# wells-wood-research/timed-design

Measured on AMD Instinct MI355X. Metric: residue_frames_per_sec, higher is better.
Workload: dtype f32

## Files before the change

include/timed_hip.h:

```cpp
#ifndef TIMED_HIP_H
#define TIMED_HIP_H

#include <stddef.h>
#include <stdint.h>

#ifdef __cplusplus
extern "C" {
#endif

#define TH_OK 0
#define TH_EINVAL (-1)
#define TH_EIO (-2)
#define TH_EHIP (-3)
#define TH_EUNSUP (-4)
#define TH_ENOMEM (-5)
#define TH_ECOMM (-6)
#define TH_EBUSY (-7)

#define TH_F32 0
#define TH_F64 1
#define TH_U8 2
#define TH_BOOL 3
#define TH_F16 4

#define TH_LOAD_DEFAULT 0u
#define TH_LOAD_NO_FUSE 1u
#define TH_LOAD_NO_MFMA 2u
#define TH_LOAD_KEEP_ALL 4u

#define TH_PREDICT_DEFAULT 0u
#define TH_PREDICT_LOGITS 1u
#define TH_PREDICT_OUT_DEVICE 2u
#define TH_PREDICT_IN_DEVICE 4u

typedef struct th_model th_model;
typedef struct th_comm th_comm;

int th_version(void);
const char* th_last_error(void);
int th_device_count(int* n_out);
int th_host_cpus(void);
int th_device_info(int device, char* name, size_t name_len, char* arch, size_t arch_len, int* cus);

int th_model_load(const char* pack_path, int device, unsigned flags, th_model** out);
int th_model_load_mem(const void* pack, size_t nbytes, int device, unsigned flags, th_model** out);
void th_model_free(th_model* m);
int th_model_info(const th_model* m, int dims[4], int* n_classes);
int th_model_cost(const th_model* m, double* algo_flops, double* exec_flops, int* n_steps);
int th_model_set_chunk(th_model* m, int frames_per_chunk);

int th_predict(th_model* m, const void* frames, int dtype, int64_t n, float* probs_out, unsigned flags);
int th_predict_async(th_model* m, const void* frames, int dtype, int64_t n, float* probs_out, unsigned flags, int* ticket);
int th_predict_wait(th_model* m, int ticket);
#define TH_SPARSE_MAGIC "THSPF001"
int th_predict_sparse_async(th_model* m, const void* blob, size_t blob_bytes, float* probs_out, unsigned flags, int* ticket);
int th_host_alloc(size_t bytes, void** out);
int th_host_free(void* p);
int th_host_register(void* p, size_t bytes);
int th_host_unregister(void* p);
int th_predict_device(th_model* m, const void* d_frames, int dtype, int64_t n, float* d_probs, unsigned flags);
int th_model_fetch(th_model* m, const char* layer_name, int64_t n, float* out, int64_t out_floats);

int th_model_profile(th_model* m, int enable);
int th_model_step_info(const th_model* m, int i, char* label, size_t label_len, double* ms, int64_t* launches,
                       double* flops_per_frame, double* exec_flops_per_frame, double* bytes_per_frame);
int th_model_step_direct_flops(const th_model* m, int i, double* direct_flops_per_frame);

int th_model_guard_info(const th_model* m, int* state, double* max_dlogit, double* logit_scale, char* note, size_t note_len);

int th_model_knobs(const th_model* m, char* buf, size_t buf_len);

int th_dev_alloc(int device, size_t bytes, void** d_out);
int th_dev_free(int device, void* d);
int th_dev_upload(int device, void* d_dst, const void* h_src, size_t bytes);
int th_dev_download(int device, void* h_dst, const void* d_src, size_t bytes);
int th_dev_sync(int device);
int th_dev_synth_frames(int device, float* d_frames, int64_t n, int side, int channels, int atoms, uint64_t seed);

int th_apply_temp(const double* probs, int64_t n_res, int n_cls, double t, double* out);
int th_apply_temp_on(int device, const double* probs, int64_t n_res, int n_cls, double t, double* out);
#define TH_RNG_HOST 0
#define TH_RNG_PHILOX 1
#define TH_RNG_MT19937 2
#define TH_RNG_MT_WORDS 3
int th_sample(const double* probs, int64_t n_res, int n_cls, int64_t n_samples, double temperature,
              int rng_mode, uint64_t seed, const double* uniforms, int32_t* idx_out);
int th_sample_ex(const double* probs, int64_t n_res, int n_cls, int64_t n_samples, double temperature,
                 int rng_mode, uint64_t seed, uint64_t rng_offset, const double* uniforms, int32_t* idx_out,
                 double* r_out, const char* cat_letters, char* letters_out, double* q_out, int device);

typedef struct th_sampler th_sampler;
int th_sampler_create(int device, th_sampler** out);
void th_sampler_free(th_sampler* s);
#define TH_TEMPER_NONE 0
#define TH_TEMPER_POW 1
#define TH_TEMPER_PREPOWERED 2
int th_sampler_load(th_sampler* s, const double* probs, int64_t n_rows, int n_cls, double temperature, int temper_mode,
                    int cum_dtype, double* q_out);
int th_sampler_draw(th_sampler* s, int64_t n_keys, const int64_t* row_off, int64_t n_samples, int rng_mode, uint64_t seed,
                    uint64_t rng_offset, const double* uniforms, const char* cat_letters, int32_t* idx_out, double* r_out,
                    char* letters_out, double* metrics_out);

int th_sampler_uniform_buffer(th_sampler* s, size_t bytes, void** out);
int th_sampler_run(th_sampler* s, const double* probs, int64_t n_rows, int n_cls, int cum_dtype, int64_t n_keys, const int64_t* row_off,
                   int64_t n_samples, int rng_mode, uint64_t seed, uint64_t rng_offset, const double* uniforms, const char* cat_letters,
                   unsigned want, const void** block_out, int64_t* offsets_out);

int th_mt19937_rand(uint32_t* key, int* pos, int64_t n, double* out);
int th_mt19937_words(uint32_t* key, int* pos, int64_t n, uint32_t* out);

int64_t th_format_csv(const void* data, int dtype, int64_t n, int64_t k, char* out, int64_t cap);
int64_t th_format_csv_device(int device, const float* rows, int64_t n, int64_t k, char* out, int64_t cap);
int th_format_csv_device_release(void);
int th_csv_shape(const char* text, int64_t len, char delim, int64_t* rows_out, int* cols_out, int* width_out);
int th_csv_fill(const char* text, int64_t len, char delim, int64_t rows, int cols, int width, uint32_t* out);
int th_argmax_letters(const void* matrix, int dtype, int64_t n, int64_t k, const char* col_letters, char* letters_out,
                      int32_t* idx_out);

typedef struct th_analysis_totals {
    int64_t confusion[20][20];
    int64_t rank_hist[21];
    int64_t n_labelled, n_nonfinite, n_similar;
} th_analysis_totals;
int th_analyse_probs(int device, const void* matrix, int dtype, int64_t n, int64_t k, const int8_t* col_res, const int8_t* true_res,
                     int8_t* pred_out, int8_t* rank_out, double* entropy_out, th_analysis_totals* totals);

int th_h5_read_chunked(const void* file, int64_t file_len, int64_t base, int64_t n_datasets, const int64_t* btree_addrs,
                       void* const* dests, int rank, const int64_t* shape, const int64_t* chunk, int esz, int n_filters,
                       const int* filter_ids, int nthreads);

int th_h5_read_chunked_as(const void* file, int64_t file_len, int64_t base, int64_t n_datasets, const int64_t* btree_addrs,
                          void* const* dests, int rank, const int64_t* shape, const int64_t* chunk, int esz, int n_filters,
                          const int* filter_ids, int nthreads, int conv);
int th_h5_read_contiguous_as(const void* file, int64_t file_len, int64_t base, int64_t n_datasets, const int64_t* data_addrs,
                             void* const* dests, int64_t count, int esz, int conv);
int th_h5_decode_device(const void* file, int64_t file_len, int64_t base, int64_t n_datasets, const int64_t* btree_addrs, int rank,
                        const int64_t* shape, const int64_t* chunk, int esz, int n_filters, const int* filter_ids, int conv, int device,
                        void* d_out);
int th_dev_trim(int device);
int th_dev_cache_info(int device, uint64_t* cached_bytes, uint64_t* cap_bytes, int* blocks);
int th_h5_release_scratch(int device);
int th_inflate_many(int device, const void* comp, int64_t comp_len, int64_t n, const int64_t* src_off, const int64_t* src_len,
                    const int64_t* dst_off, const int64_t* dst_len, void* out, int64_t out_len, int wrapped, int* status_out);

int th_h5_resolve(const void* file, int64_t file_len, int64_t base, int64_t n, const int64_t* ohdr_addrs, const char* num_attr,
                  double* num_out, int num_len, const char* str_attr, char* str_out, int str_len, int64_t* btree_out,
                  int64_t* geom_out, int* status_out, int nthreads);

int th_h5_group_links(const void* file, int64_t file_len, int64_t base, int64_t btree_addr, int64_t heap_data, int64_t heap_size,
                      char* names, int64_t names_cap, int64_t* addrs, int64_t addrs_cap, int64_t* n_out, int64_t* names_len);

int th_voxelise(int device, const float* atoms_xyz, const int32_t* atom_channel, const float* atom_sigma, int64_t n_atoms,
                const float* frames_rt, int64_t n_res, int voxels_per_side, float frame_edge_length, int n_channels, int gaussian,
                void* out, int out_on_device);

#define TH_COMM_ID_BYTES 128
int th_comm_unique_id(char id[TH_COMM_ID_BYTES]);
int th_comm_init(const char id[TH_COMM_ID_BYTES], int n_ranks, int rank, int device, th_comm** out);
void th_comm_free(th_comm* c);
int th_comm_gather_rows(th_comm* c, const float* d_local, const int64_t* counts, int width, int root,
                        float* d_out);
int th_comm_barrier(th_comm* c);
int th_comm_stats(th_comm* c, int64_t out[5]);

#ifdef __cplusplus
}
#endif
#endif
```

timed-design_amd/csrc/common.h:

```cpp
#pragma once
#include <hip/hip_runtime.h>
#include <stdint.h>
#include <string>
#include <vector>

#include "../../include/timed_hip.h"

enum : int {
    OP_INPUT = 0, OP_CONV3D, OP_DENSE, OP_BN, OP_ACT, OP_MAXPOOL, OP_AVGPOOL, OP_GAP, OP_GMP,
    OP_FLATTEN, OP_CONCAT, OP_ADD, OP_IDENTITY
};
enum : int { ACT_LINEAR = 0, ACT_RELU, ACT_ELU, ACT_SOFTMAX, ACT_SIGMOID, ACT_TANH, ACT_LEAKY };

void th_set_error(const char* fmt, ...);
#define TH_FAIL(code, ...)          \
    do {                            \
        th_set_error(__VA_ARGS__);  \
        return (code);              \
    } while (0)
#define HIP_TRY(expr)                                                                            \
    do {                                                                                         \
        hipError_t _e = (expr);                                                                  \
        if (_e != hipSuccess) {                                                                  \
            th_set_error("%s failed: %s (%s:%d)", #expr, hipGetErrorString(_e), __FILE__, __LINE__); \
            return TH_EHIP;                                                                      \
        }                                                                                        \
    } while (0)

struct ThKnobs {
    int winograd = 1;
    int wino_split = 1;
    int wfused = 1;
    int wf_split = 1;
    int lanes = 1, lane_lag = 1;
    int guard = 1;
    int first_wino = 1;
    int first_split = 1;
    int conv_gl = 1;
    int dense_gemm = 1;
    int first_int = 1;
    int first_zb = 0;
    int first_dbg = 0;
    int no_pool_first = 0;
    int no_tail_fuse = 0;
    int conv_nogeo = 0, n16_nogeo = 0, conv_noxc = 0, conv_notail = 0, conv_nozmajor = 0, conv_nocompact = 0, conv_nopw = 0;
    int conv_bmode = 0;
    int conv_dbg = 0, conv_ldspad = 0, n16_resident = 0;
    int pw_nopipe = 0, pw_noepi = 0, pw_dbg = 0;
    int wf_resident = 0, wf_dbg = 0, wf_noblk = 0;
    long long wino_piece = 0;
    int wino_dbg = 0, wino_var = 3, wino_b3var = 2, wino_nomid = 0;
    std::string nondefault;
};
void th_knobs_read(ThKnobs* k);
inline const ThKnobs& th_knobs_of(const ThKnobs* k) { static const ThKnobs dflt; return k ? *k : dflt; }

hipError_t th_malloc_retry_impl(void** p, size_t bytes);
template <class T> inline hipError_t th_malloc_retry(T** p, size_t bytes) { return th_malloc_retry_impl(reinterpret_cast<void**>(p), bytes); }

int th_usable_cpus();

struct TView {
    float* p = nullptr;
    int D = 1, H = 1, W = 1, C = 0;
    int cs = 0;
    int coff = 0;
    int64_t fs = 0;
    int blk = 0;
    int V() const { return D * H * W; }
};

#define TH_MAX_POST 4
enum : int { POP_ACT = 1, POP_AFFINE = 2 };
struct PostOps {
    int n = 0;
    int type[TH_MAX_POST] = {0, 0, 0, 0};
    int act[TH_MAX_POST] = {0, 0, 0, 0};
    float alpha[TH_MAX_POST] = {0, 0, 0, 0};
    const float* scale[TH_MAX_POST] = {nullptr, nullptr, nullptr, nullptr};
    const float* shift[TH_MAX_POST] = {nullptr, nullptr, nullptr, nullptr};
    int monotone = 0;
};
struct PreOp {
    const float* scale = nullptr;
    const float* shift = nullptr;
    int act = ACT_LINEAR;
    float alpha = 0.f;
};

struct ConvGeom {
    int kd, kh, kw, sd, sh, sw, dd, dh, dw;
    int pz, py, px;
};
int launch_convert_frames(hipStream_t s, const void* src, int dtype, int64_t n, int V, int C, TView dst);
int launch_conv3d_direct(hipStream_t s, int64_t n, TView in, TView out, ConvGeom g, const float* w, const float* bias,
                         PreOp pre, PostOps post);
int launch_pool3d(hipStream_t s, int64_t n, TView in, TView out, ConvGeom g, int is_max);
int launch_eltwise(hipStream_t s, int64_t n, TView in, TView out, PostOps ops);
int launch_global_pool(hipStream_t s, int64_t n, TView in, TView out, int is_max);
int launch_dense(hipStream_t s, int64_t n, TView in, TView out, const float* w, const float* bias, PostOps post);
inline bool conv_gl_wanted(int knob, const ConvGeom& g, int Vo) { return knob == 2 || (knob == 1 && (g.sd > 1 || g.sh > 1 || g.sw > 1 || Vo <= 64)); }
bool conv_gl_ok(int Cin, int Cout, int in_cs, int in_coff, int64_t in_fs);
size_t conv_gl_wpk_floats(const ConvGeom& g, int Cin, int Cout);
double conv_gl_exec_flops(const ConvGeom& g, int Cin, int Cout, int Vo);
std::string conv_gl_label(int Cout);
void conv_gl_pack_weights(const ConvGeom& g, int Cin, int Cout, const float* w, float* dst);
int launch_conv_gl(hipStream_t s, int64_t n, TView in, TView out, ConvGeom g, int Cin, int Cout, const float* wpk, const float* bias, PreOp pre, PostOps post);
bool dense_gemm_ok(int F, int O, int64_t xfs);
int launch_dense_gemm(hipStream_t s, int64_t n, TView in, TView out, const float* w, const float* bias, PostOps post);
int launch_softmax(hipStream_t s, int64_t n, TView in, TView out);
int launch_gap_softmax(hipStream_t s, int64_t n, TView in, TView logits, TView probs);
int launch_tail_dense(hipStream_t s, int64_t n, TView in, PostOps pre, TView pooled, TView logits, TView probs, const float* w,
                      const float* bias, PostOps post, int softmax);
int launch_copy(hipStream_t s, int64_t n, TView in, TView out);
int launch_add(hipStream_t s, int64_t n, TView a, TView b, TView out);
int launch_synth_frames(hipStream_t s, float* d, int64_t n, int side, int channels, int atoms, uint64_t seed);

struct ConvMfmaPlan {
    int cfg = -1;
    int CI = 0, CS = 0;
    int BN = 0;
    int nnb = 0;
    int nchunks = 0;
    int pool = 0;
    int Dc = 0, Hc = 0, Wc = 0;
    int FB = 1, ZB = 0, nzb = 1;
    int Zp = 0, Hp = 0, Wp = 0;
    int rows_pf = 0;
    int bres = 0;
    int ncu = 0;
    size_t lds_bytes = 0;
    size_t tab_off = 0;
    size_t wpk_floats = 0;
    double exec_flops = 0;
    int first_wino = 0;
    double own_flops = 0;
    int geo = 0;
    const ThKnobs* knobs = nullptr;
    std::string label;
};
bool conv_mfma_plan(const TView& in, const TView& out_conv, const ConvGeom& g, int Cin, int Cout, int pool,
                    const ThKnobs& kn, ConvMfmaPlan* plan);
bool conv_mfma_plan_tail(const TView& in, const TView& out_conv, const ConvGeom& g, int Cin, int Cout, int pool,
                         const ConvMfmaPlan& main, const ThKnobs& kn, ConvMfmaPlan* tail, int* cout_main);
void conv_mfma_pack_weights(const ConvMfmaPlan& p, const ConvGeom& g, int Cin, int Cout, const float* w_keras,
                            float* dst);
int launch_conv_mfma(hipStream_t s, int64_t n, const ConvMfmaPlan& p, TView in, TView out, ConvGeom g, int Cin,
                     int Cout, const float* wpk, const float* bias, PreOp pre, PostOps post);

struct ConvWinoPlan {
    int P = 9;
    int Cin = 0, Cout = 0, Coutp = 0, ncb = 0;
    int Cinp = 0;
    size_t wpk_floats = 0;
    int64_t v_fpf = 0, m_fpf = 0;
    double gemm_flops = 0;
    double exec_flops = 0;
    int split = 0;
    int narrow = 0;
    int b3var = 0;
    const ThKnobs* knobs = nullptr;
    std::string label;
};
bool conv_wino_plan(const TView& in, const TView& out_conv, const ConvGeom& g, int Cin, int Cout, int scheme, int split, const ThKnobs& kn,
                    ConvWinoPlan* plan);
void conv_wino_pack_weights(const ConvWinoPlan& p, const float* w_keras, float* dst);
int launch_wino_in(hipStream_t s, int64_t n, const ConvWinoPlan& p, TView in, float* V, PreOp pre);
int launch_wino_gemm(hipStream_t s, int64_t n, const ConvWinoPlan& p, const float* V, float* M, const float* wpk);
int launch_wino_out(hipStream_t s, int64_t n, const ConvWinoPlan& p, const float* M, TView out, const float* bias, PostOps post, bool gap = false);
int launch_wino_mid(hipStream_t s, int64_t n, const ConvWinoPlan& p, const float* M, float* V_next, const float* bias, PostOps post);

struct ConvWfPlan {
    int geo = -1;
    int pool = 0;
    int Cin = 0, Cout = 0, ncb = 0, nchunks = 0;
    size_t wpk_floats = 0, lds_bytes = 0;
    double own_flops = 0;
    double exec_flops = 0;
    int ncu = 0;
    const ThKnobs* knobs = nullptr;
    std::string label;
};
bool conv_wf_plan(const TView& in, const TView& out_conv, const ConvGeom& g, int Cin, int Cout, int pool, const ThKnobs& kn, ConvWfPlan* plan);
bool conv_wf_view_ok(const TView& in);
int conv_wf_pre_kind(const PreOp& pre);
std::string conv_wf_label(const ConvWfPlan& p, const PreOp& pre);
void conv_wf_pack_weights(const ConvWfPlan& p, const float* w_keras, float* dst);
int launch_conv_wf(hipStream_t s, int64_t n, const ConvWfPlan& p, TView in, TView out, const float* wpk, const float* bias, PreOp pre,
                   PostOps post);

struct ConvWfsPlan {
    int geo = -1, pool = 0;
    int Cin = 0, Cout = 0, nkh = 0, ncp = 0;
    size_t wpk_floats = 0, lds_bytes = 0;
    double own_flops = 0, exec_flops = 0;
    int ncu = 0;
    const ThKnobs* knobs = nullptr;
    std::string label;
};
bool conv_wfs_plan(const ConvWfPlan& base, const TView& in, const PreOp& pre, const ThKnobs& kn, ConvWfsPlan* plan);
void conv_wfs_pack_weights(const ConvWfsPlan& p, const float* w_keras, float* dst);
int launch_conv_wfs(hipStream_t s, int64_t n, const ConvWfsPlan& p, TView in, TView out, const float* wpk, const float* bias, PostOps post);

int launch_sparse_expand(hipStream_t s, int64_t n, const uint32_t* bits, const uint64_t* vidx, const float* values, float* out, int E, int W);

std::string conv_first_label(const ConvMfmaPlan& p, int Cin, const PostOps& post);
bool conv_first_plan(int Din, int Hin, int Win, int Cin, const TView& out_conv, const ConvGeom& g, int Cout, int pool,
                     const ThKnobs& kn, ConvMfmaPlan* plan);
void conv_first_pack_weights(int Cin, int Cout, const float* w_keras, float* dst);
void conv_first_w_pack_weights(int Cin, int Cout, const float* w_keras, float* dst);
int launch_conv_first(hipStream_t s, int64_t n, const ConvMfmaPlan& p, const void* frames, int dtype, int Din, int Hin,
                      int Win, int Cin, TView out, ConvGeom g, int Cout, const float* wpk, const float* bias, PostOps post);
bool conv_first_b3_ok(const ConvMfmaPlan& p, int Din, int Hin, int Win, int Cin, int Cout, const ConvGeom& g, const PostOps& post);
size_t conv_first_b3_wpk_floats();
double conv_first_b3_exec_flops();
std::string conv_first_b3_label(int nnb);
void conv_first_b3_pack_weights(int Cin, int Cout, const float* w_keras, float* dst);
int launch_conv_first_b3(hipStream_t s, int64_t n, const ConvMfmaPlan& p, const void* frames, int dtype, int Cin, TView out, int Cout,
                         const float* wpk, const float* bias, PostOps post);

bool conv_first5_ok(int Din, int Hin, int Win, int Cin, int Cout, const ConvGeom& g, int pool, const ThKnobs& kn);
size_t conv_first5_wpk_floats();
double conv_first5_exec_flops();
std::string conv_first5_label();
void conv_first5_pack_weights(int Cin, int Cout, const float* w_keras, float* dst);
int launch_conv_first5(hipStream_t s, int64_t n, const ThKnobs* knobs, int ncu, const void* frames, int dtype, int Cin, TView out, int Cout,
                       const float* wpk, const float* bias, PostOps post);

bool conv_pw_plan(const TView& in, const TView& out_conv, const ConvGeom& g, int Cin, int Cout, int pool, const ThKnobs& kn, ConvMfmaPlan* plan);
void conv_pw_pack_weights(const ConvMfmaPlan& p, int Cin, int Cout, const float* w_keras, float* dst);
std::string conv_pw_label(const ConvMfmaPlan& p, bool out_blk, const PostOps& post);
int launch_conv_pw(hipStream_t s, int64_t n, const ConvMfmaPlan& p, TView in, TView out, int Cin, int Cout, const float* wpk,
                   const float* bias, PreOp pre, PostOps post);

int sampler_run(int device, const double* h_probs, int64_t n_res, int n_cls, int64_t n_samples, double temperature,
                int rng_mode, uint64_t seed, uint64_t rng_offset, const double* h_uniforms, int32_t* h_idx, double* h_r_out,
                const char* cat_letters, char* h_letters, double* h_q_out);
```

timed-design_amd/csrc/conv_wino.hip:

```cpp
#include "common.h"
#include "device_math.h"
#include "wino_tables.h"

#include <algorithm>
#include <cstdlib>
#include <cstring>
#include <thread>
#include <vector>

typedef float f32x16 __attribute__((ext_vector_type(16)));

namespace {

constexpr int kZ = WINO_N;
constexpr int kNF = 64;
constexpr int kKC = 32;
constexpr int kCB = 128;

template <int R, int C>
__device__ __forceinline__ void wino_apply(const float (&T)[R][C], const float (&in)[C], float (&out)[R]) {
#pragma unroll
    for (int r = 0; r < R; ++r) {
        float acc = 0.f;
        bool first = true;
#pragma unroll
        for (int c = 0; c < C; ++c) {
            const float t = T[r][c];
            if (t == 0.f) continue;
            if (first) acc = t == 1.f ? in[c] : (t == -1.f ? -in[c] : t * in[c]);
            else acc = t == 1.f ? acc + in[c] : (t == -1.f ? acc - in[c] : fmaf(t, in[c], acc));
            first = false;
        }
        out[r] = acc;
    }
}

template <int P> struct WinoTab;
template <> struct WinoTab<9> {
    static __device__ __forceinline__ void fwd(const float (&in)[kZ], float (&out)[9]) { wino_apply<9, kZ>(kWinoBT9, in, out); }
    static __device__ __forceinline__ void inv(const float (&in)[9], float (&out)[kZ]) { wino_apply<kZ, 9>(kWinoAT9, in, out); }
};
template <> struct WinoTab<7> {
    static __device__ __forceinline__ void fwd(const float (&in)[kZ], float (&out)[7]) { wino_apply<7, kZ>(kWinoBT7, in, out); }
    static __device__ __forceinline__ void inv(const float (&in)[7], float (&out)[kZ]) { wino_apply<kZ, 7>(kWinoAT7, in, out); }
};

struct WinoInArgs {
    const float* in; int64_t in_fs; int in_cs, in_coff;
    int Cin;
    int Creal;
    PreOp pre;
    float* V; int64_t Ns;
    int64_t n;
};

template <bool PRE, int kP>
__global__ void __launch_bounds__(256) k_wino_in(const WinoInArgs a) {
    constexpr int kPos = kP * kP;
    const unsigned idx = blockIdx.x * 256u + threadIdx.x;
    const unsigned c = idx % (unsigned)a.Cin, f = idx / (unsigned)a.Cin;
    if (f >= (unsigned)a.n) return;
    const unsigned ooff = f * (unsigned)a.Cin + c;
    const int64_t pstride = a.Ns * a.Cin;
    if (c >= (unsigned)a.Creal) {
        for (int z = 0; z < kZ; ++z) {
            float* __restrict__ pos = a.V + (int64_t)z * kPos * pstride;
            for (int q = 0; q < kPos; ++q) (pos + (int64_t)q * pstride)[ooff] = 0.f;
        }
        return;
    }
    const unsigned ioff = f * (unsigned)a.in_fs + c;
    const float* __restrict__ in0 = a.in + a.in_coff;
    const bool affine = PRE && a.pre.scale != nullptr;
    const float sc = affine ? a.pre.scale[c] : 1.f, sh = affine ? a.pre.shift[c] : 0.f;
#pragma unroll 1
    for (int z = 0; z < kZ; ++z) {
        float x[kZ][kZ];
        const float* __restrict__ vox = in0 + (int64_t)z * kZ * kZ * a.in_cs;
#pragma unroll
        for (int i = 0; i < kZ * kZ; ++i) x[i / kZ][i % kZ] = (vox + (int64_t)i * a.in_cs)[ioff];
        if (PRE) {
            float flat[kZ * kZ];
#pragma unroll
            for (int i = 0; i < kZ * kZ; ++i) flat[i] = affine ? fmaf(x[i / kZ][i % kZ], sc, sh) : x[i / kZ][i % kZ];
            th_act_vec<kZ * kZ>(flat, a.pre.act, a.pre.alpha);
#pragma unroll
            for (int i = 0; i < kZ * kZ; ++i) x[i / kZ][i % kZ] = flat[i];
        }
        float t[kP][kZ];
#pragma unroll
        for (int k = 0; k < kZ; ++k) {
            float col[kZ], o[kP];
#pragma unroll
            for (int y = 0; y < kZ; ++y) col[y] = x[y][k];
            WinoTab<kP>::fwd(col, o);
#pragma unroll
            for (int aa = 0; aa < kP; ++aa) t[aa][k] = o[aa];
        }
        float* __restrict__ pos = a.V + (int64_t)z * kPos * pstride;
#pragma unroll
        for (int aa = 0; aa < kP; ++aa) {
            float o[kP];
            WinoTab<kP>::fwd(t[aa], o);
#pragma unroll
            for (int b = 0; b < kP; ++b) (pos + (int64_t)(aa * kP + b) * pstride)[ooff] = o[b];
        }
    }
}

struct WinoOutArgs {
    const float* M; int64_t Ns; int Coutp;
    int Cout;
    const float* bias;
    PostOps post;
    float* out; int64_t out_fs; int out_cs, out_coff;
    int64_t n;
};

template <int kP, bool GAP = false>
__global__ void __launch_bounds__(256) k_wino_out(const WinoOutArgs a) {
    constexpr int kPos = kP * kP;
    const unsigned idx = blockIdx.x * 256u + threadIdx.x;
    const unsigned co = idx % (unsigned)a.Cout, f = idx / (unsigned)a.Cout;
    if (f >= (unsigned)a.n) return;
    const unsigned ioff = f * (unsigned)a.Coutp + co;
    const unsigned ooff = f * (unsigned)a.out_fs + co;
    const int64_t pstride = a.Ns * a.Coutp;
    const float bv = a.bias ? a.bias[co] : 0.f;
    const bool elu_bn = a.post.n == 2 && a.post.type[0] == POP_ACT && a.post.act[0] == ACT_ELU && a.post.type[1] == POP_AFFINE;
    const float ealpha = a.post.alpha[0], esc = elu_bn ? a.post.scale[1][co] : 1.f, esh = elu_bn ? a.post.shift[1][co] : 0.f;
    float* __restrict__ out0 = a.out + a.out_coff;
    float gsum = 0.f;
#pragma unroll 1
    for (int z = 0; z < kZ; ++z) {
        float t[kP][kZ];
        const float* __restrict__ pos = a.M + (int64_t)z * kPos * pstride;
#pragma unroll
        for (int aa = 0; aa < kP; ++aa) {
            float m[kP];
#pragma unroll
            for (int b = 0; b < kP; ++b) m[b] = (pos + (int64_t)(aa * kP + b) * pstride)[ioff];
            WinoTab<kP>::inv(m, t[aa]);
        }
        float y[kZ * kZ];
#pragma unroll
        for (int k = 0; k < kZ; ++k) {
            float col[kP], o[kZ];
#pragma unroll
            for (int aa = 0; aa < kP; ++aa) col[aa] = t[aa][k];
            WinoTab<kP>::inv(col, o);
#pragma unroll
            for (int j = 0; j < kZ; ++j) y[j * kZ + k] = o[j] + bv;
        }
        if (elu_bn) {
#pragma unroll
            for (int k = 0; k < kZ * kZ; ++k) y[k] = fmaf(y[k] > 0.f ? y[k] : ealpha * (__expf(y[k]) - 1.f), esc, esh);
        } else
        for (int i = 0; i < a.post.n; ++i) {
            if (a.post.type[i] == POP_AFFINE) {
                const float sc = a.post.scale[i][co], sh = a.post.shift[i][co];
#pragma unroll
                for (int k = 0; k < kZ * kZ; ++k) y[k] = fmaf(y[k], sc, sh);
            } else {
                th_act_vec<kZ * kZ>(y, a.post.act[i], a.post.alpha[i]);
            }
        }
        if (GAP) {
#pragma unroll
            for (int v = 0; v < kZ * kZ; ++v) gsum += y[v];
            continue;
        }
        float* __restrict__ vox = out0 + (int64_t)z * kZ * kZ * a.out_cs;
#pragma unroll
        for (int v = 0; v < kZ * kZ; ++v) (vox + (int64_t)v * a.out_cs)[ooff] = y[v];
    }
    if (GAP) out0[ooff] = gsum / (float)(kZ * kZ * kZ);
}

struct WinoMidArgs {
    const float* M; int64_t Ns; int Coutp;
    int C;
    const float* bias;
    PostOps post;
    float* V;
    int Cn;
    int64_t n;
};

template <int kP>
__global__ void __launch_bounds__(256) k_wino_mid(const WinoMidArgs a) {
    constexpr int kPos = kP * kP;
    const unsigned idx = blockIdx.x * 256u + threadIdx.x;
    const unsigned c = idx % (unsigned)a.Cn, f = idx / (unsigned)a.Cn;
    if (f >= (unsigned)a.n) return;
    const unsigned ioff = f * (unsigned)a.Coutp + c;
    const unsigned ooff = f * (unsigned)a.Cn + c;
    const int64_t ipstride = a.Ns * a.Coutp, opstride = a.Ns * a.Cn;
    if (c >= (unsigned)a.C) {
        for (int z = 0; z < kZ; ++z) {
            float* __restrict__ opos = a.V + (int64_t)z * kPos * opstride;
            for (int q = 0; q < kPos; ++q) (opos + (int64_t)q * opstride)[ooff] = 0.f;
        }
        return;
    }
    const float bv = a.bias ? a.bias[c] : 0.f;
    const bool elu_bn = a.post.n == 2 && a.post.type[0] == POP_ACT && a.post.act[0] == ACT_ELU && a.post.type[1] == POP_AFFINE;
    const float ealpha = a.post.alpha[0], esc = elu_bn ? a.post.scale[1][c] : 1.f, esh = elu_bn ? a.post.shift[1][c] : 0.f;
#pragma unroll 1
    for (int z = 0; z < kZ; ++z) {
        float t[kP][kZ];
        const float* __restrict__ ipos = a.M + (int64_t)z * kPos * ipstride;
#pragma unroll
        for (int aa = 0; aa < kP; ++aa) {
            float m[kP];
#pragma unroll
            for (int b = 0; b < kP; ++b) m[b] = (ipos + (int64_t)(aa * kP + b) * ipstride)[ioff];
            WinoTab<kP>::inv(m, t[aa]);
        }
        float y[kZ * kZ];
#pragma unroll
        for (int k = 0; k < kZ; ++k) {
            float col[kP], o[kZ];
#pragma unroll
            for (int aa = 0; aa < kP; ++aa) col[aa] = t[aa][k];
            WinoTab<kP>::inv(col, o);
#pragma unroll
            for (int j = 0; j < kZ; ++j) y[j * kZ + k] = o[j] + bv;
        }
        if (elu_bn) {
#pragma unroll
            for (int k = 0; k < kZ * kZ; ++k) y[k] = fmaf(y[k] > 0.f ? y[k] : ealpha * (__expf(y[k]) - 1.f), esc, esh);
        } else
        for (int i = 0; i < a.post.n; ++i) {
            if (a.post.type[i] == POP_AFFINE) {
                const float sc = a.post.scale[i][c], sh = a.post.shift[i][c];
#pragma unroll
                for (int k = 0; k < kZ * kZ; ++k) y[k] = fmaf(y[k], sc, sh);
            } else {
                th_act_vec<kZ * kZ>(y, a.post.act[i], a.post.alpha[i]);
            }
        }
        float u[kP][kZ];
#pragma unroll
        for (int k = 0; k < kZ; ++k) {
            float col[kZ], o[kP];
#pragma unroll
            for (int j = 0; j < kZ; ++j) col[j] = y[j * kZ + k];
            WinoTab<kP>::fwd(col, o);
#pragma unroll
            for (int aa = 0; aa < kP; ++aa) u[aa][k] = o[aa];
        }
        float* __restrict__ opos = a.V + (int64_t)z * kPos * opstride;
#pragma unroll
        for (int aa = 0; aa < kP; ++aa) {
            float o[kP];
            WinoTab<kP>::fwd(u[aa], o);
#pragma unroll
            for (int b = 0; b < kP; ++b) (opos + (int64_t)(aa * kP + b) * opstride)[ooff] = o[b];
        }
    }
}

struct WinoGemmArgs {
    const float* V; const float* U; float* M;
    int64_t Ns;
    int Cin, Coutp;
    int Cout;
    int nfb, ncb;
    int npos;
    unsigned total;
    unsigned per_xcd;
    int dbg;
};

__device__ __forceinline__ constexpr bool wino_tap_ok(int zi, int dz) { return zi - dz + 1 >= 0 && zi - dz + 1 < kZ; }

template <int VAR>
__global__ void __launch_bounds__(256, 2) k_wino_gemm(const WinoGemmArgs a) {
    __shared__ __attribute__((aligned(16))) float lds[kZ * kNF * kKC];
    const unsigned xcd = blockIdx.x & 7u, slot = blockIdx.x >> 3;
    const unsigned L = xcd * a.per_xcd + slot;
    if (slot >= a.per_xcd || L >= a.total) return;
    const unsigned cb = L % (unsigned)a.ncb;
    const unsigned fb = (L / (unsigned)a.ncb) % (unsigned)a.nfb;
    const unsigned p = L / (unsigned)(a.ncb * a.nfb);
    const int tid = threadIdx.x, lane = tid & 63;
    const int wave = __builtin_amdgcn_readfirstlane(tid >> 6);
    const int j = lane & 31, h = lane >> 5;
    const int nchunks = a.Cin / kKC;
    const bool active = (int)(cb * kCB) + wave * 32 < a.Cout;
    const int S = a.Cin / 8;
    const float4* wq = reinterpret_cast<const float4*>(a.U) + ((size_t)((p * a.ncb + cb) * 4 + wave) * S * 3) * 64 + lane;
    const float* vbase = a.V + ((int64_t)p * a.Ns + (int64_t)fb * kNF) * a.Cin;
    const int64_t zstride = (int64_t)a.npos * a.Ns * a.Cin;

    f32x16 acc[kZ][2];
#pragma unroll
    for (int z = 0; z < kZ; ++z)
#pragma unroll
        for (int rt = 0; rt < 2; ++rt)
#pragma unroll
            for (int r = 0; r < 16; ++r) acc[z][rt][r] = 0.f;

    float4 bw[2][3];
#pragma unroll
    for (int dz = 0; dz < 3; ++dz) bw[0][dz] = wq[dz * 64];
    const int r0 = 8 * wave + (lane >> 3);
    const float* gsrc = vbase + (int64_t)r0 * a.Cin + (((lane & 7) ^ (lane >> 3)) << 2);
    const int64_t rstride32 = (int64_t)32 * a.Cin;
    unsigned aoff[kKC / 8];
#pragma unroll
    for (int s = 0; s < kKC / 8; ++s) aoff[s] = (unsigned)(j * kKC + (((2 * s + h) ^ (j & 7)) << 2));
    constexpr int kSlots = kKC / 8;
    static_assert(kSlots % 2 == 0, "the weight register sets alternate per k-slot");

    for (int ch = 0; ch < nchunks; ++ch) {
        __syncthreads();
        if (!(a.dbg & 1))
#pragma unroll
        for (int i = 0; i < 10; ++i)
            __builtin_amdgcn_global_load_lds(gsrc + (i >> 1) * zstride + (i & 1) * rstride32 + ch * kKC,
                                             lds + (size_t)(i * 4 + wave) * 256, 16, 0, 0);
        __syncthreads();
        if (!active) continue;
        float4 af[2][2];
        af[0][0] = *reinterpret_cast<const float4*>(lds + aoff[0]);
        af[0][1] = *reinterpret_cast<const float4*>(lds + aoff[0] + 32 * kKC);
#pragma unroll
        for (int s = 0; s < kSlots; ++s) {
            {
                const int sg = ch * kSlots + s;
                const int nx = sg + 1 < S ? sg + 1 : sg;
                if (a.dbg & 4) {
#pragma unroll
                    for (int dz = 0; dz < 3; ++dz) bw[(s + 1) & 1][dz] = bw[s & 1][dz];
                } else
#pragma unroll
                for (int dz = 0; dz < 3; ++dz) bw[(s + 1) & 1][dz] = wq[(size_t)(nx * 3 + dz) * 64];
            }
#pragma unroll
            for (int zi = 0; zi < kZ; ++zi) {
                const int ph = s * kZ + zi, cur = ph & 1;
                if (ph + 1 < kSlots * kZ) {
                    const int ns = (ph + 1) / kZ, nz = (ph + 1) % kZ;
                    af[cur ^ 1][0] = *reinterpret_cast<const float4*>(lds + aoff[ns] + (nz * kNF) * kKC);
                    af[cur ^ 1][1] = *reinterpret_cast<const float4*>(lds + aoff[ns] + (nz * kNF + 32) * kKC);
                }
                if (VAR == 1) __builtin_amdgcn_sched_barrier(0);
                const float av0[4] = {af[cur][0].x, af[cur][0].y, af[cur][0].z, af[cur][0].w};
                const float av1[4] = {af[cur][1].x, af[cur][1].y, af[cur][1].z, af[cur][1].w};
#pragma unroll
                for (int dz = 0; dz < 3; ++dz) {
                    if (!wino_tap_ok(zi, dz)) continue;
                    const int zo = zi - dz + 1;
                    const float4 b4 = bw[s & 1][dz];
                    const float bv[4] = {b4.x, b4.y, b4.z, b4.w};
#pragma unroll
                    for (int t = 0; t < 4; ++t) {
                        acc[zo][0] = __builtin_amdgcn_mfma_f32_32x32x2f32(av0[t], bv[t], acc[zo][0], 0, 0, 0);
                        acc[zo][1] = __builtin_amdgcn_mfma_f32_32x32x2f32(av1[t], bv[t], acc[zo][1], 0, 0, 0);
                    }
                }
                if (VAR == 1) __builtin_amdgcn_sched_barrier(0);
            }
        }
    }
    if (!active) return;
    float* mbase = a.M + ((int64_t)p * a.Ns + (int64_t)fb * kNF) * a.Coutp + cb * kCB + wave * 32 + j;
    const int64_t mz = (int64_t)a.npos * a.Ns * a.Coutp;
    if (a.dbg & 2) {
        float sum = 0.f;
#pragma unroll
        for (int z = 0; z < kZ; ++z)
#pragma unroll
            for (int rt = 0; rt < 2; ++rt)
#pragma unroll
                for (int r = 0; r < 16; ++r) sum += acc[z][rt][r];
        if (sum == 12345.678f) mbase[0] = sum;
        return;
    }
    if (VAR == 3) {
        __syncthreads();
        float* T = lds + wave * (32 * 36);
        const int rr = lane >> 3, c4 = (lane & 7) * 4;
        float* mb = a.M + ((int64_t)p * a.Ns + (int64_t)fb * kNF) * a.Coutp + cb * kCB + wave * 32 + c4;
#pragma unroll
        for (int z = 0; z < kZ; ++z)
#pragma unroll
            for (int rt = 0; rt < 2; ++rt) {
#pragma unroll
                for (int r = 0; r < 16; ++r) T[((r & 3) + 8 * (r >> 2) + 4 * h) * 36 + j] = acc[z][rt][r];
#pragma unroll
                for (int k = 0; k < 4; ++k) {
                    const int row = rr + 8 * k;
                    *reinterpret_cast<float4*>(mb + z * mz + (int64_t)(rt * 32 + row) * a.Coutp) = *reinterpret_cast<const float4*>(T + row * 36 + c4);
                }
            }
        return;
    }
#pragma unroll
    for (int z = 0; z < kZ; ++z)
#pragma unroll
        for (int rt = 0; rt < 2; ++rt)
#pragma unroll
            for (int r = 0; r < 16; ++r) {
                const int row = rt * 32 + (r & 3) + 8 * (r >> 2) + 4 * h;
                if (VAR == 2) __builtin_nontemporal_store(acc[z][rt][r], mbase + z * mz + (int64_t)row * a.Coutp);
                else mbase[z * mz + (int64_t)row * a.Coutp] = acc[z][rt][r];
            }
}


typedef __bf16 bf16x8 __attribute__((ext_vector_type(8)));
typedef __bf16 bf16x2 __attribute__((ext_vector_type(2)));
typedef float f32x2v __attribute__((ext_vector_type(2)));
typedef unsigned u32x4v __attribute__((ext_vector_type(4)));

__device__ __forceinline__ unsigned wino_pk_bf16(float lo, float hi) {
    return __builtin_bit_cast(unsigned, __builtin_convertvector((f32x2v){lo, hi}, bf16x2));
}
__device__ __forceinline__ float wino_bf16_lo(unsigned w) { return __builtin_bit_cast(float, w << 16); }
__device__ __forceinline__ float wino_bf16_hi(unsigned w) { return __builtin_bit_cast(float, w & 0xffff0000u); }

constexpr int kB3Slab = kZ * kNF * kKC * 2;

__device__ __forceinline__ constexpr int wino_b3_sw16(int R) { return ((R >> 2) & 3) ^ (((R >> 2) & 1) << 1); }

typedef float f32x4 __attribute__((ext_vector_type(4)));

__device__ __forceinline__ void wino_gemm_b3_16(const WinoGemmArgs& a, unsigned char* lds) {
    const unsigned xcd = blockIdx.x & 7u, slot = blockIdx.x >> 3;
    const unsigned L = xcd * a.per_xcd + slot;
    if (slot >= a.per_xcd || L >= a.total) return;
    const unsigned cb = L % (unsigned)a.ncb;
    const unsigned fb = (L / (unsigned)a.ncb) % (unsigned)a.nfb;
    const unsigned p = L / (unsigned)(a.ncb * a.nfb);
    const int tid = threadIdx.x, lane = tid & 63;
    const int wave = __builtin_amdgcn_readfirstlane(tid >> 6);
    const int r16 = lane & 15, g16 = lane >> 4;
    const int nchunks = a.Cin / kKC;
    const bool active = (int)(cb * kCB) + wave * 32 < a.Cout;
    const __amdgpu_buffer_rsrc_t wrsrc = __builtin_amdgcn_make_buffer_rsrc(
        const_cast<float*>(a.U + ((size_t)((p * a.ncb + cb) * 4 + wave) * nchunks * 18) * 256), 0, 0xffffffffu, 0x00020000);
    const unsigned woff = (unsigned)lane * 16u;
    const float* vbase = a.V + ((int64_t)p * a.Ns + (int64_t)fb * kNF) * a.Cin;
    const int64_t zstride = (int64_t)a.npos * a.Ns * a.Cin;

    f32x4 acc[kZ][4][2];
#pragma unroll
    for (int z = 0; z < kZ; ++z)
#pragma unroll
        for (int rt = 0; rt < 4; ++rt)
#pragma unroll
            for (int ct = 0; ct < 2; ++ct) acc[z][rt][ct] = (f32x4){0.f, 0.f, 0.f, 0.f};

    const int r0 = 8 * wave + (lane >> 3), g4 = lane & 7;
    __amdgpu_buffer_rsrc_t vrsrc[kZ];
#pragma unroll
    for (int z = 0; z < kZ; ++z) vrsrc[z] = __builtin_amdgcn_make_buffer_rsrc(const_cast<float*>(vbase + z * zstride), 0, 0xffffffffu, 0x00020000);
    const unsigned goff = (unsigned)(r0 * a.Cin + 4 * g4) * 4u;
    const unsigned rstride32_b = (unsigned)(32 * a.Cin * 4);
    unsigned char* const sdst = lds + r0 * 64 + (((g4 >> 1) ^ wino_b3_sw16(r0)) << 4) + ((g4 & 1) << 3);
    const unsigned char* const aptr = lds + r16 * 64 + ((g16 ^ wino_b3_sw16(r16)) << 4);

    uint4 bw[2][3][3];
    auto load_b = [&](int ch, int ct) {
        if (a.dbg & 4) {
            const unsigned k = woff ^ ((unsigned)(ch * 2 + ct) << 4);
#pragma unroll
            for (int dz = 0; dz < 3; ++dz)
#pragma unroll
                for (int pc = 0; pc < 3; ++pc)
                    bw[ct][dz][pc] = make_uint4(0x3f813f82u ^ (k << (dz + pc)), 0x3e833e84u ^ k, 0x3d853d86u + (k << pc), 0x3c873c88u ^ (k << dz));
            return;
        }
#pragma unroll
        for (int dz = 0; dz < 3; ++dz)
#pragma unroll
            for (int pc = 0; pc < 3; ++pc)
                bw[ct][dz][pc] = __builtin_bit_cast(uint4, __builtin_amdgcn_raw_buffer_load_b128(wrsrc, woff, (((ch * 2 + ct) * 3 + dz) * 3 + pc) * 1024, 0));
    };

    for (int ch = 0; ch < nchunks; ++ch) {
        __syncthreads();
        {
            float4 x[10];
#pragma unroll
            for (int i = 0; i < 10; ++i)
                x[i] = (a.dbg & 1) ? make_float4(1.f, 2.f, 3.f, 4.f) :
                       __builtin_bit_cast(float4, __builtin_amdgcn_raw_buffer_load_b128(vrsrc[i >> 1], goff, (i & 1) * rstride32_b + ch * (kKC * 4), 0));
            __builtin_amdgcn_sched_barrier(0);
#pragma unroll
            for (int i = 0; i < 10; ++i) {
                const unsigned h01 = wino_pk_bf16(x[i].x, x[i].y), h23 = wino_pk_bf16(x[i].z, x[i].w);
                const float rx = x[i].x - wino_bf16_lo(h01), ry = x[i].y - wino_bf16_hi(h01);
                const float rz = x[i].z - wino_bf16_lo(h23), rw = x[i].w - wino_bf16_hi(h23);
                const unsigned m01 = wino_pk_bf16(rx, ry), m23 = wino_pk_bf16(rz, rw);
                const float sx = rx - wino_bf16_lo(m01), sy = ry - wino_bf16_hi(m01);
                const float sz = rz - wino_bf16_lo(m23), sw = rw - wino_bf16_hi(m23);
                const unsigned l01 = wino_pk_bf16(sx, sy), l23 = wino_pk_bf16(sz, sw);
                *reinterpret_cast<uint2*>(sdst + i * 2048) = make_uint2(h01, h23);
                *reinterpret_cast<uint2*>(sdst + i * 2048 + kB3Slab) = make_uint2(m01, m23);
                *reinterpret_cast<uint2*>(sdst + i * 2048 + 2 * kB3Slab) = make_uint2(l01, l23);
            }
        }
        load_b(ch, 0);
        load_b(ch, 1);
        __syncthreads();
        if (!active) continue;
#pragma unroll
        for (int zi = 0; zi < kZ; ++zi)
#pragma unroll
            for (int rt = 0; rt < 4; ++rt) {
                bf16x8 af[3];
#pragma unroll
                for (int pc = 0; pc < 3; ++pc)
                    af[pc] = __builtin_bit_cast(bf16x8, *reinterpret_cast<const uint4*>(aptr + pc * kB3Slab + (zi * kNF + rt * 16) * 64));
#pragma unroll
                for (int dz = 0; dz < 3; ++dz) {
                    if (!wino_tap_ok(zi, dz)) continue;
                    const int zo = zi - dz + 1;
                    constexpr int PA[6] = {2, 0, 1, 1, 0, 0}, PB[6] = {0, 2, 1, 0, 1, 0};
#pragma unroll
                    for (int c = 0; c < 6; ++c)
#pragma unroll
                        for (int ct = 0; ct < 2; ++ct)
                            acc[zo][rt][ct] = __builtin_amdgcn_mfma_f32_16x16x32_bf16(af[PA[c]], __builtin_bit_cast(bf16x8, bw[ct][dz][PB[c]]),
                                                                                     acc[zo][rt][ct], 0, 0, 0);
                }
                __builtin_amdgcn_sched_barrier(0);
            }
    }
    if (!active) return;
    if (a.dbg & 2) {
        float sum = 0.f;
#pragma unroll
        for (int z = 0; z < kZ; ++z)
#pragma unroll
            for (int rt = 0; rt < 4; ++rt)
#pragma unroll
                for (int ct = 0; ct < 2; ++ct)
#pragma unroll
                    for (int r = 0; r < 4; ++r) sum += acc[z][rt][ct][r];
        if (sum == 12345.678f) a.M[0] = sum;
        return;
    }
    __syncthreads();
    float* T = reinterpret_cast<float*>(lds) + wave * (16 * 36);
    const int rr = lane >> 3, c4 = (lane & 7) * 4;
    float* mb = a.M + ((int64_t)p * a.Ns + (int64_t)fb * kNF) * a.Coutp + cb * kCB + wave * 32 + c4;
    const int64_t mz = (int64_t)a.npos * a.Ns * a.Coutp;
#pragma unroll
    for (int z = 0; z < kZ; ++z)
#pragma unroll
        for (int rt = 0; rt < 4; ++rt) {
#pragma unroll
            for (int ct = 0; ct < 2; ++ct)
#pragma unroll
                for (int r = 0; r < 4; ++r) T[(4 * g16 + r) * 36 + ct * 16 + r16] = acc[z][rt][ct][r];
#pragma unroll
            for (int k = 0; k < 2; ++k) {
                const int row = rr + 8 * k;
                *reinterpret_cast<float4*>(mb + z * mz + (int64_t)(rt * 16 + row) * a.Coutp) = *reinterpret_cast<const float4*>(T + row * 36 + c4);
            }
        }
}

template <int VAR>
__global__ void __launch_bounds__(256, 2) k_wino_gemm_b3(const WinoGemmArgs a) {
    __shared__ __attribute__((aligned(16))) unsigned char lds[3 * kB3Slab];
    if constexpr (VAR == 2) {
        wino_gemm_b3_16(a, lds);
        return;
    }
    const unsigned xcd = blockIdx.x & 7u, slot = blockIdx.x >> 3;
    const unsigned L = xcd * a.per_xcd + slot;
    if (slot >= a.per_xcd || L >= a.total) return;
    const unsigned cb = L % (unsigned)a.ncb;
    const unsigned fb = (L / (unsigned)a.ncb) % (unsigned)a.nfb;
    const unsigned p = L / (unsigned)(a.ncb * a.nfb);
    const int tid = threadIdx.x, lane = tid & 63;
    const int wave = __builtin_amdgcn_readfirstlane(tid >> 6);
    const int j = lane & 31, h = lane >> 5;
    const int nchunks = a.Cin / kKC;
    const bool active = (int)(cb * kCB) + wave * 32 < a.Cout;
    const int S = nchunks * 6;
    const uint4* wq = reinterpret_cast<const uint4*>(a.U) + ((size_t)((p * a.ncb + cb) * 4 + wave) * S * 3) * 64 + lane;
    const float* vbase = a.V + ((int64_t)p * a.Ns + (int64_t)fb * kNF) * a.Cin;
    const int64_t zstride = (int64_t)a.npos * a.Ns * a.Cin;

    f32x16 acc[kZ][2];
#pragma unroll
    for (int z = 0; z < kZ; ++z)
#pragma unroll
        for (int rt = 0; rt < 2; ++rt)
#pragma unroll
            for (int r = 0; r < 16; ++r) acc[z][rt][r] = 0.f;

    uint4 bw[2][3];
#pragma unroll
    for (int pc = 0; pc < 3; ++pc) bw[0][pc] = wq[pc * 64];
    const int r0 = 8 * wave + (lane >> 3), g4 = lane & 7;
    __amdgpu_buffer_rsrc_t vrsrc[kZ];
#pragma unroll
    for (int z = 0; z < kZ; ++z) vrsrc[z] = __builtin_amdgcn_make_buffer_rsrc(const_cast<float*>(vbase + z * zstride), 0, 0xffffffffu, 0x00020000);
    const unsigned goff = (unsigned)(r0 * a.Cin + 4 * g4) * 4u;
    const unsigned rstride32_b = (unsigned)(32 * a.Cin * 4);
    unsigned char* const sdst = lds + r0 * 64 + (((g4 >> 1) ^ ((r0 >> 2) & 3)) << 4) + ((g4 & 1) << 3);
    const unsigned char* aptr[2];
#pragma unroll
    for (int ks = 0; ks < 2; ++ks) aptr[ks] = lds + j * 64 + (((2 * ks + h) ^ ((j >> 2) & 3)) << 4);

    for (int ch = 0; ch < nchunks; ++ch) {
        __syncthreads();
        {
            float4 x[10];
#pragma unroll
            for (int i = 0; i < 10; ++i)
                x[i] = (a.dbg & 1) ? make_float4(1.f, 2.f, 3.f, 4.f) :
                       __builtin_bit_cast(float4, __builtin_amdgcn_raw_buffer_load_b128(vrsrc[i >> 1], goff, (i & 1) * rstride32_b + ch * (kKC * 4), 0));
            __builtin_amdgcn_sched_barrier(0);
#pragma unroll
            for (int i = 0; i < 10; ++i) {
                const unsigned h01 = wino_pk_bf16(x[i].x, x[i].y), h23 = wino_pk_bf16(x[i].z, x[i].w);
                const float rx = x[i].x - wino_bf16_lo(h01), ry = x[i].y - wino_bf16_hi(h01);
                const float rz = x[i].z - wino_bf16_lo(h23), rw = x[i].w - wino_bf16_hi(h23);
                const unsigned m01 = wino_pk_bf16(rx, ry), m23 = wino_pk_bf16(rz, rw);
                const float sx = rx - wino_bf16_lo(m01), sy = ry - wino_bf16_hi(m01);
                const float sz = rz - wino_bf16_lo(m23), sw = rw - wino_bf16_hi(m23);
                const unsigned l01 = wino_pk_bf16(sx, sy), l23 = wino_pk_bf16(sz, sw);
                *reinterpret_cast<uint2*>(sdst + i * 2048) = make_uint2(h01, h23);
                *reinterpret_cast<uint2*>(sdst + i * 2048 + kB3Slab) = make_uint2(m01, m23);
                *reinterpret_cast<uint2*>(sdst + i * 2048 + 2 * kB3Slab) = make_uint2(l01, l23);
            }
        }
        __syncthreads();
        if (!active) continue;
#pragma unroll
        for (int st = 0; st < 6; ++st) {
            const int ks = st / 3, dz = st % 3, cur = st & 1;
            {
                const int sg = ch * 6 + st;
                const int nx = sg + 1 < S ? sg + 1 : sg;
                if (a.dbg & 4) {
#pragma unroll
                    for (int pc = 0; pc < 3; ++pc) bw[cur ^ 1][pc] = bw[cur][pc];
                } else
#pragma unroll
                for (int pc = 0; pc < 3; ++pc) bw[cur ^ 1][pc] = wq[(size_t)(nx * 3 + pc) * 64];
            }
            bf16x8 bf[3];
#pragma unroll
            for (int pc = 0; pc < 3; ++pc) bf[pc] = __builtin_bit_cast(bf16x8, bw[cur][pc]);
            const int nzi = 5 - (dz != 1), z0 = dz == 2 ? 1 : 0;
            bf16x8 af[2][2][3];
            auto read_a = [&](int set, int zi) {
#pragma unroll
                for (int rt = 0; rt < 2; ++rt)
#pragma unroll
                    for (int pc = 0; pc < 3; ++pc)
                        af[set][rt][pc] = __builtin_bit_cast(bf16x8, *reinterpret_cast<const uint4*>(aptr[ks] + pc * kB3Slab + (zi * kNF + rt * 32) * 64));
            };
            if (VAR == 1) read_a(0, z0);
#pragma unroll
            for (int k = 0; k < kZ; ++k) {
                if (k >= nzi) continue;
                const int zi = z0 + k, zo = zi - dz + 1;
                const int set = VAR == 1 ? (k & 1) : 0;
                if (VAR == 1) { if (k + 1 < nzi) read_a(set ^ 1, zi + 1); }
                else read_a(0, zi);
                if (VAR == 1) __builtin_amdgcn_sched_barrier(0);
                constexpr int PA[6] = {2, 0, 1, 1, 0, 0}, PB[6] = {0, 2, 1, 0, 1, 0};
#pragma unroll
                for (int c = 0; c < 6; ++c)
#pragma unroll
                    for (int rt = 0; rt < 2; ++rt)
                        acc[zo][rt] = __builtin_amdgcn_mfma_f32_32x32x16_bf16(af[set][rt][PA[c]], bf[PB[c]], acc[zo][rt], 0, 0, 0);
                __builtin_amdgcn_sched_barrier(0);
            }
        }
    }
    if (!active) return;
    if (a.dbg & 2) {
        float sum = 0.f;
#pragma unroll
        for (int z = 0; z < kZ; ++z)
#pragma unroll
            for (int rt = 0; rt < 2; ++rt)
#pragma unroll
                for (int r = 0; r < 16; ++r) sum += acc[z][rt][r];
        if (sum == 12345.678f) a.M[0] = sum;
        return;
    }
    __syncthreads();
    float* T = reinterpret_cast<float*>(lds) + wave * (32 * 36);
    const int rr = lane >> 3, c4 = (lane & 7) * 4;
    float* mb = a.M + ((int64_t)p * a.Ns + (int64_t)fb * kNF) * a.Coutp + cb * kCB + wave * 32 + c4;
    const int64_t mz = (int64_t)a.npos * a.Ns * a.Coutp;
#pragma unroll
    for (int z = 0; z < kZ; ++z)
#pragma unroll
        for (int rt = 0; rt < 2; ++rt) {
#pragma unroll
            for (int r = 0; r < 16; ++r) T[((r & 3) + 8 * (r >> 2) + 4 * h) * 36 + j] = acc[z][rt][r];
#pragma unroll
            for (int k = 0; k < 4; ++k) {
                const int row = rr + 8 * k;
                *reinterpret_cast<float4*>(mb + z * mz + (int64_t)(rt * 32 + row) * a.Coutp) = *reinterpret_cast<const float4*>(T + row * 36 + c4);
            }
        }
}



__global__ void __launch_bounds__(256, 2) k_wino_gemm_n32(const WinoGemmArgs a) {
    __shared__ __attribute__((aligned(16))) float4 tile[4][32 * 8];
    const int tid = threadIdx.x, lane = tid & 63;
    const int wave = __builtin_amdgcn_readfirstlane(tid >> 6);
    const int j = lane & 31, h = lane >> 5;
    const int nfb32 = (int)(a.Ns / 32);
    const int groups = (nfb32 + 3) / 4;
    const unsigned p = blockIdx.x / (unsigned)groups;
    const int fb = (int)(blockIdx.x % (unsigned)groups) * 4 + wave;
    if (fb >= nfb32) return;
    const int nchunks = a.Cin / kKC;
    const uint4* wq = reinterpret_cast<const uint4*>(a.U) + (size_t)p * nchunks * 18 * 64 + lane;
    const float* vbase = a.V + ((int64_t)p * a.Ns + (int64_t)fb * 32) * a.Cin;
    const int64_t zstride = (int64_t)a.npos * a.Ns * a.Cin;
    __amdgpu_buffer_rsrc_t vrsrc[kZ];
#pragma unroll
    for (int z = 0; z < kZ; ++z) vrsrc[z] = __builtin_amdgcn_make_buffer_rsrc(const_cast<float*>(vbase + z * zstride), 0, 0xffffffffu, 0x00020000);
    const int lr = lane >> 3, lg = lane & 7;
    const unsigned goff = (unsigned)(lr * a.Cin + 4 * lg) * 4u;
    const unsigned row8_b = (unsigned)(8 * a.Cin * 4);
    float4* const T = tile[wave];

    f32x16 acc[kZ];
#pragma unroll
    for (int z = 0; z < kZ; ++z)
#pragma unroll
        for (int r = 0; r < 16; ++r) acc[z][r] = 0.f;

    auto load_plane = [&](float4 (&x)[4], int ch, int zi) {
#pragma unroll
        for (int k = 0; k < 4; ++k)
            x[k] = __builtin_bit_cast(float4, __builtin_amdgcn_raw_buffer_load_b128(vrsrc[zi], goff, k * row8_b + ch * (kKC * 4), 0));
    };
    auto transpose = [&](const float4 (&x)[4], float4 (&f)[4]) {
#pragma unroll
        for (int k = 0; k < 4; ++k) { const int r = 8 * k + lr; T[r * 8 + (lg ^ ((r >> 1) & 7))] = x[k]; }
#pragma unroll
        for (int g = 0; g < 4; ++g) f[g] = T[j * 8 + ((4 * h + g) ^ ((j >> 1) & 7))];
    };
    auto split8 = [&](const float4& lo, const float4& hi, bf16x8 (&f)[3]) {
        const float v[8] = {lo.x, lo.y, lo.z, lo.w, hi.x, hi.y, hi.z, hi.w};
        unsigned hw[4], mw[4], lw[4];
#pragma unroll
        for (int q = 0; q < 4; ++q) {
            hw[q] = wino_pk_bf16(v[2 * q], v[2 * q + 1]);
            const float r0 = v[2 * q] - wino_bf16_lo(hw[q]), r1 = v[2 * q + 1] - wino_bf16_hi(hw[q]);
            mw[q] = wino_pk_bf16(r0, r1);
            const float s0 = r0 - wino_bf16_lo(mw[q]), s1 = r1 - wino_bf16_hi(mw[q]);
            lw[q] = wino_pk_bf16(s0, s1);
        }
        f[0] = __builtin_bit_cast(bf16x8, make_uint4(hw[0], hw[1], hw[2], hw[3]));
        f[1] = __builtin_bit_cast(bf16x8, make_uint4(mw[0], mw[1], mw[2], mw[3]));
        f[2] = __builtin_bit_cast(bf16x8, make_uint4(lw[0], lw[1], lw[2], lw[3]));
    };

    float4 xs[3][4];
    auto load_step = [&](float4 (&x)[4], int step_ch, int zi) {
        load_plane(x, step_ch < nchunks ? step_ch : nchunks - 1, zi);
    };
    load_step(xs[0], 0, 0);
    load_step(xs[1], 0, 1);
    for (int ch0 = 0; ch0 < nchunks; ch0 += 3) {
#pragma unroll
        for (int cc = 0; cc < 3; ++cc) {
            const int ch = ch0 + cc;
            if (ch >= nchunks) break;
            uint4 bw[2][3][3];
#pragma unroll
            for (int ks = 0; ks < 2; ++ks)
#pragma unroll
                for (int dz = 0; dz < 3; ++dz)
#pragma unroll
                    for (int pc = 0; pc < 3; ++pc) bw[ks][dz][pc] = wq[(size_t)(((ch * 2 + ks) * 3 + dz) * 3 + pc) * 64];
#pragma unroll
            for (int zi = 0; zi < kZ; ++zi) {
                const int t = cc * kZ + zi;
                float4 fr[4];
                transpose(xs[t % 3], fr);
                {
                    const int t2 = t + 2, c2 = ch0 + t2 / kZ, z2 = t2 % kZ;
                    load_step(xs[t2 % 3], c2, z2);
                }
                bf16x8 af[2][3];
                split8(fr[0], fr[1], af[0]);
                split8(fr[2], fr[3], af[1]);
                constexpr int PA[6] = {2, 0, 1, 1, 0, 0}, PB[6] = {0, 2, 1, 0, 1, 0};
#pragma unroll
                for (int q = 0; q < 6; ++q)
#pragma unroll
                    for (int ks = 0; ks < 2; ++ks)
#pragma unroll
                        for (int dz = 0; dz < 3; ++dz) {
                            if (!wino_tap_ok(zi, dz)) continue;
                            acc[zi - dz + 1] = __builtin_amdgcn_mfma_f32_32x32x16_bf16(af[ks][PA[q]], __builtin_bit_cast(bf16x8, bw[ks][dz][PB[q]]),
                                                                                       acc[zi - dz + 1], 0, 0, 0);
                        }
                __builtin_amdgcn_sched_barrier(0);
            }
        }
    }
    float* mb = a.M + ((int64_t)p * a.Ns + (int64_t)fb * 32) * a.Coutp + j;
    const int64_t mz = (int64_t)a.npos * a.Ns * a.Coutp;
#pragma unroll
    for (int z = 0; z < kZ; ++z)
#pragma unroll
        for (int r = 0; r < 16; ++r) mb[z * mz + (int64_t)((r & 3) + 8 * (r >> 2) + 4 * h) * a.Coutp] = acc[z][r];
}

}

bool conv_wino_plan(const TView& in, const TView& out, const ConvGeom& g, int Cin, int Cout, int scheme, int split, const ThKnobs& kn, ConvWinoPlan* p) {
    if (g.kd != 3 || g.kh != 3 || g.kw != 3 || g.sd != 1 || g.sh != 1 || g.sw != 1 || g.dd != 1 || g.dh != 1 || g.dw != 1) return false;
    if (g.pz != 1 || g.py != 1 || g.px != 1) return false;
    if (in.D != kZ || in.H != kZ || in.W != kZ || out.D != kZ || out.H != kZ || out.W != kZ) return false;
    const bool narrow = split && Cout <= 32 && Cin >= 128;
    if (Cin < kKC || (Cout < 64 && !narrow)) return false;
    if (scheme != 9 && scheme != 7) return false;
    const int kPos = scheme * scheme;
    p->P = scheme;
    p->Cin = Cin; p->Cout = Cout;
    p->Cinp = (Cin + kKC - 1) / kKC * kKC;
    const int Cinp = p->Cinp;
    p->narrow = narrow ? 1 : 0;
    p->Coutp = narrow ? 32 : (Cout + kCB - 1) / kCB * kCB;
    p->ncb = narrow ? 1 : p->Coutp / kCB;
    p->split = split ? 1 : 0;
    p->b3var = split && !narrow ? kn.wino_b3var : 0;
    p->knobs = &kn;
    p->wpk_floats = (size_t)kPos * 3 * Cinp * p->Coutp * (p->split ? 3 : 2) / 2;
    p->v_fpf = (int64_t)kZ * kPos * Cinp;
    p->m_fpf = (int64_t)kZ * kPos * p->Coutp;
    p->gemm_flops = 2.0 * kPos * 13 * Cin * (double)Cout;
    p->exec_flops = 2.0 * kPos * 13 * Cinp * (double)((Cout + 31) / 32 * 32);
    p->label = std::string("conv_wino<") + (scheme == 9 ? "F(3,3)+F(2,3)" : "F(5,3)") + " in-plane, z direct; gemm " + (narrow ? "32f x 32" : "64f x " + std::to_string(kCB)) + "c, K" + std::to_string(Cinp) + (Cinp != Cin ? " (" + std::to_string(Cin) + " real)" : "") +
               (p->split ? "; bf16x3 split operands, 6 products, fp32 accumulate" : "") + ">";
    return true;
}

static inline uint16_t wino_bf16_rne(float f) {
    uint32_t u;
    std::memcpy(&u, &f, 4);
    if ((u & 0x7f800000u) == 0x7f800000u) return (uint16_t)(u >> 16);
    u += 0x7fffu + ((u >> 16) & 1u);
    return (uint16_t)(u >> 16);
}
static inline double wino_bf16_val(uint16_t b) {
    const uint32_t u = (uint32_t)b << 16;
    float f;
    std::memcpy(&f, &u, 4);
    return (double)f;
}
static inline void wino_split3(double x, uint16_t (&pc)[3]) {
    pc[0] = wino_bf16_rne((float)x);
    const double r1 = x - wino_bf16_val(pc[0]);
    pc[1] = wino_bf16_rne((float)r1);
    const double r2 = r1 - wino_bf16_val(pc[1]);
    pc[2] = wino_bf16_rne((float)r2);
}

void conv_wino_pack_weights(const ConvWinoPlan& p, const float* w, float* dst) {
    const int Cin = p.Cin, Cinp = p.Cinp, Cout = p.Cout, S = Cinp / 8, ncb = p.ncb, kP = p.P;
    auto G = [kP](int a, int j) { return kP == 9 ? kWinoG9[a][j] : kWinoG7[a][j]; };
    std::memset(dst, 0, p.wpk_floats * sizeof(float));
    auto work = [&](int ci_lo, int ci_hi) {
        std::vector<double> t((size_t)kP * 3 * Cout), u((size_t)Cout);
        for (int ci = ci_lo; ci < ci_hi; ++ci) {
            const int s = ci / 8, hh = (ci % 8) / 4, tt = ci % 4;
            for (int dz = 0; dz < 3; ++dz) {
                for (int a = 0; a < kP; ++a)
                    for (int k = 0; k < 3; ++k) {
                        double* tr = &t[((size_t)a * 3 + k) * Cout];
                        std::fill(tr, tr + Cout, 0.0);
                        for (int jj = 0; jj < 3; ++jj) {
                            const double g = G(a, jj);
                            if (g == 0.0) continue;
                            const float* wr = w + ((((size_t)dz * 3 + jj) * 3 + k) * Cin + ci) * Cout;
                            for (int co = 0; co < Cout; ++co) tr[co] += g * (double)wr[co];
                        }
                    }
                for (int a = 0; a < kP; ++a)
                    for (int b = 0; b < kP; ++b) {
                        std::fill(u.begin(), u.end(), 0.0);
                        for (int k = 0; k < 3; ++k) {
                            const double g = G(b, k);
                            if (g == 0.0) continue;
                            const double* tr = &t[((size_t)a * 3 + k) * Cout];
                            for (int co = 0; co < Cout; ++co) u[co] += g * tr[co];
                        }
                        const int pos = a * kP + b;
                        if (p.narrow) {
                            uint16_t* d16 = reinterpret_cast<uint16_t*>(dst);
                            const int chunk = ci / kKC, h16 = (ci % kKC) / 16, ks = (ci % 16) / 8, e = ci % 8, nch = Cinp / kKC;
                            for (int co = 0; co < Cout; ++co) {
                                uint16_t pc[3];
                                wino_split3(u[co], pc);
                                const size_t frag = ((size_t)(pos * nch + chunk) * 2 + ks) * 3 + dz;
                                for (int q = 0; q < 3; ++q) d16[((frag * 3 + q) * 64 + (h16 * 32 + co)) * 8 + e] = pc[q];
                            }
                            continue;
                        }
                        if (p.split && p.b3var == 2) {
                            uint16_t* d16 = reinterpret_cast<uint16_t*>(dst);
                            const int chunk = ci / kKC, g8 = (ci % kKC) / 8, e = ci % 8, nch = Cinp / kKC;
                            for (int co = 0; co < Cout; ++co) {
                                const int cb = co / kCB, wv = (co % kCB) / 32, ct = (co % 32) / 16, c = co % 16;
                                uint16_t pc[3];
                                wino_split3(u[co], pc);
                                const size_t frag = ((size_t)(((pos * ncb + cb) * 4 + wv) * nch + chunk) * 2 + ct) * 3 + dz;
                                for (int q = 0; q < 3; ++q) d16[((frag * 3 + q) * 64 + (g8 * 16 + c)) * 8 + e] = pc[q];
                            }
                            continue;
                        }
                        if (p.split) {
                            uint16_t* d16 = reinterpret_cast<uint16_t*>(dst);
                            const int chunk = ci / kKC, ks = (ci % kKC) / 16, h8 = (ci % 16) / 8, e = ci % 8, nsteps = (Cinp / kKC) * 6;
                            for (int co = 0; co < Cout; ++co) {
                                const int cb = co / kCB, wv = (co % kCB) / 32, j = co % 32;
                                uint16_t pc[3];
                                wino_split3(u[co], pc);
                                const size_t step = (size_t)((pos * ncb + cb) * 4 + wv) * nsteps + (size_t)(chunk * 2 + ks) * 3 + dz;
                                for (int q = 0; q < 3; ++q) d16[((step * 3 + q) * 64 + (h8 * 32 + j)) * 8 + e] = pc[q];
                            }
                            continue;
                        }
                        for (int co = 0; co < Cout; ++co) {
                            const int cb = co / kCB, wv = (co % kCB) / 32, j = co % 32;
                            dst[((((size_t)(pos * ncb + cb) * 4 + wv) * S + s) * 3 + dz) * 256 + (hh * 32 + j) * 4 + tt] = (float)u[co];
                        }
                    }
            }
        }
    };
    const int nt = std::max(1, std::min({th_usable_cpus(), 32, Cin / 8}));
    if (nt == 1) { work(0, Cin); return; }
    std::vector<std::thread> th;
    for (int k = 0; k < nt; ++k) th.emplace_back(work, (int)((int64_t)Cin * k / nt), (int)((int64_t)Cin * (k + 1) / nt));
    for (auto& x : th) x.join();
}

static int64_t wino_piece(const ConvWinoPlan& p, int64_t n, int64_t Ns, int64_t fs, int width) {
    const int64_t lim = (1ll << 31) - 1;
    if (Ns * width > lim) return 0;
    const int64_t forced = th_knobs_of(p.knobs).wino_piece;
    const int64_t piece = std::max<int64_t>(1, std::min<int64_t>(n, lim / std::max<int64_t>(fs, 1)));
    return forced > 0 ? std::min(piece, forced) : piece;
}

int launch_wino_in(hipStream_t s, int64_t n, const ConvWinoPlan& p, TView in, float* V, PreOp pre) {
    if (n <= 0) return TH_OK;
    const int64_t Ns = (n + kNF - 1) / kNF * kNF;
    const int64_t piece = wino_piece(p, n, Ns, in.fs, p.Cinp);
    if (!piece) TH_FAIL(TH_EUNSUP, "conv_wino: %lld frames per launch exceed the 32-bit offsets of the transform kernels", (long long)n);
    const bool has_pre = pre.scale || pre.act != ACT_LINEAR;
    for (int64_t f0 = 0; f0 < n; f0 += piece) {
        const int64_t cnt = std::min(piece, n - f0);
        WinoInArgs ia;
        ia.in = in.p + f0 * in.fs; ia.in_fs = in.fs; ia.in_cs = in.cs; ia.in_coff = in.coff; ia.Cin = p.Cinp; ia.Creal = p.Cin; ia.pre = pre;
        ia.V = V + f0 * p.Cinp; ia.Ns = Ns; ia.n = cnt;
        const dim3 grid((unsigned)((cnt * p.Cinp + 255) / 256));
        if (p.P == 9) {
            if (has_pre) hipLaunchKernelGGL((k_wino_in<true, 9>), grid, dim3(256), 0, s, ia);
            else hipLaunchKernelGGL((k_wino_in<false, 9>), grid, dim3(256), 0, s, ia);
        } else {
            if (has_pre) hipLaunchKernelGGL((k_wino_in<true, 7>), grid, dim3(256), 0, s, ia);
            else hipLaunchKernelGGL((k_wino_in<false, 7>), grid, dim3(256), 0, s, ia);
        }
    }
    HIP_TRY(hipGetLastError());
    return TH_OK;
}

int launch_wino_gemm(hipStream_t s, int64_t n, const ConvWinoPlan& p, const float* V, float* M, const float* wpk) {
    if (n <= 0) return TH_OK;
    WinoGemmArgs ga;
    ga.V = V; ga.U = wpk; ga.M = M; ga.Ns = (n + kNF - 1) / kNF * kNF; ga.Cin = p.Cinp; ga.Coutp = p.Coutp;
    ga.Cout = p.Cout;
    ga.nfb = (int)(ga.Ns / kNF); ga.ncb = p.ncb;
    ga.npos = p.P * p.P;
    ga.total = (unsigned)(ga.npos * ga.nfb * ga.ncb);
    ga.per_xcd = (ga.total + 7) / 8;
    const ThKnobs& kn = th_knobs_of(p.knobs);
    ga.dbg = kn.wino_dbg;
    const int var = kn.wino_var;
    if (p.narrow) {
        const int64_t groups = (ga.Ns / 32 + 3) / 4;
        hipLaunchKernelGGL(k_wino_gemm_n32, dim3((unsigned)(ga.npos * groups)), dim3(256), 0, s, ga);
    } else if (p.split) {
        const int bvar = p.b3var;
        if (bvar == 2) hipLaunchKernelGGL(k_wino_gemm_b3<2>, dim3(ga.per_xcd * 8), dim3(256), 0, s, ga);
        else if (bvar == 1) hipLaunchKernelGGL(k_wino_gemm_b3<1>, dim3(ga.per_xcd * 8), dim3(256), 0, s, ga);
        else hipLaunchKernelGGL(k_wino_gemm_b3<0>, dim3(ga.per_xcd * 8), dim3(256), 0, s, ga);
    }
    else if (var == 0) hipLaunchKernelGGL(k_wino_gemm<0>, dim3(ga.per_xcd * 8), dim3(256), 0, s, ga);
    else if (var == 2) hipLaunchKernelGGL(k_wino_gemm<2>, dim3(ga.per_xcd * 8), dim3(256), 0, s, ga);
    else if (var == 3) hipLaunchKernelGGL(k_wino_gemm<3>, dim3(ga.per_xcd * 8), dim3(256), 0, s, ga);
    else hipLaunchKernelGGL(k_wino_gemm<1>, dim3(ga.per_xcd * 8), dim3(256), 0, s, ga);
    HIP_TRY(hipGetLastError());
    return TH_OK;
}

int launch_wino_out(hipStream_t s, int64_t n, const ConvWinoPlan& p, const float* M, TView out, const float* bias, PostOps post, bool gap) {
    if (n <= 0) return TH_OK;
    const int64_t Ns = (n + kNF - 1) / kNF * kNF;
    const int64_t piece = wino_piece(p, n, Ns, out.fs, p.Coutp);
    if (!piece) TH_FAIL(TH_EUNSUP, "conv_wino: %lld frames per launch exceed the 32-bit offsets of the transform kernels", (long long)n);
    for (int64_t f0 = 0; f0 < n; f0 += piece) {
        const int64_t cnt = std::min(piece, n - f0);
        WinoOutArgs oa;
        oa.M = M + f0 * p.Coutp; oa.Ns = Ns; oa.Coutp = p.Coutp; oa.Cout = p.Cout; oa.bias = bias; oa.post = post;
        oa.out = out.p + f0 * out.fs; oa.out_fs = out.fs; oa.out_cs = out.cs; oa.out_coff = out.coff; oa.n = cnt;
        const dim3 grid((unsigned)((cnt * p.Cout + 255) / 256));
        if (gap) {
            if (p.P == 9) hipLaunchKernelGGL((k_wino_out<9, true>), grid, dim3(256), 0, s, oa);
            else hipLaunchKernelGGL((k_wino_out<7, true>), grid, dim3(256), 0, s, oa);
        } else if (p.P == 9) hipLaunchKernelGGL(k_wino_out<9>, grid, dim3(256), 0, s, oa);
        else hipLaunchKernelGGL(k_wino_out<7>, grid, dim3(256), 0, s, oa);
    }
    HIP_TRY(hipGetLastError());
    return TH_OK;
}

int launch_wino_mid(hipStream_t s, int64_t n, const ConvWinoPlan& p, const float* M, float* V_next, const float* bias, PostOps post) {
    if (n <= 0) return TH_OK;
    const int64_t Ns = (n + kNF - 1) / kNF * kNF;
    if (Ns * (int64_t)p.Coutp >= (1ll << 31))
        TH_FAIL(TH_EUNSUP, "conv_wino: %lld frames per launch exceed the 32-bit offsets of the transform kernels", (long long)n);
    const int Cn = (p.Cout + kKC - 1) / kKC * kKC;
    if (Ns * (int64_t)Cn >= (1ll << 31))
        TH_FAIL(TH_EUNSUP, "conv_wino: %lld frames per launch exceed the 32-bit offsets of the transform kernels", (long long)n);
    WinoMidArgs ma;
    ma.M = M; ma.Ns = Ns; ma.Coutp = p.Coutp; ma.C = p.Cout; ma.Cn = Cn; ma.bias = bias; ma.post = post; ma.V = V_next; ma.n = n;
    const dim3 grid((unsigned)((n * (int64_t)Cn + 255) / 256));
    if (p.P == 9) hipLaunchKernelGGL(k_wino_mid<9>, grid, dim3(256), 0, s, ma);
    else hipLaunchKernelGGL(k_wino_mid<7>, grid, dim3(256), 0, s, ma);
    HIP_TRY(hipGetLastError());
    return TH_OK;
}
```

timed-design_amd/csrc/runtime.hip:

```cpp
#include "common.h"

#include <algorithm>
#include <chrono>
#include <cmath>
#include <cstdarg>
#include <cstdio>
#include <cstring>
#include <functional>
#include <map>
#include <memory>
#include <mutex>
#include <set>

#include <dlfcn.h>
#include <sys/stat.h>
#include <unistd.h>

static thread_local char g_err[1024] = "";
void th_set_error(const char* fmt, ...) {
    va_list ap;
    va_start(ap, fmt);
    vsnprintf(g_err, sizeof g_err, fmt, ap);
    va_end(ap);
}

void th_knobs_read(ThKnobs* k) {
    *k = ThKnobs();
    std::string& nd = k->nondefault;
    auto note = [&](const char* name, const char* v) { nd += (nd.empty() ? "" : " "); nd += name; nd += "="; nd += v; };
    auto num = [&](const char* name, int* dst, int lo, int hi) {
        const char* e = getenv(name);
        if (!e) return;
        const int v = std::max(lo, std::min(hi, atoi(e)));
        if (v != *dst) note(name, e);
        *dst = v;
    };
    auto flag = [&](const char* name, int* dst) {
        const char* e = getenv(name);
        if (e && *e && atoi(e) != 0) { *dst = 1; note(name, e); }
    };
    num("TH_WINOGRAD", &k->winograd, 0, 2);
    num("TH_WINO_SPLIT", &k->wino_split, 0, 1);
    num("TH_WFUSED", &k->wfused, 0, 1);
    num("TH_WF_SPLIT", &k->wf_split, 0, 1);
    if (const char* e = getenv("TH_LANES")) { k->lanes = atoi(e) == 2 ? 2 : 1; if (k->lanes != 1) note("TH_LANES", e); }
    num("TH_LANE_LAG", &k->lane_lag, 0, 1 << 20);
    num("TH_GUARD", &k->guard, 0, 2);
    num("TH_FIRST_WINO", &k->first_wino, 0, 1);
    num("TH_FIRST_SPLIT", &k->first_split, 0, 1);
    num("TH_FIRST_INT", &k->first_int, 0, 1);
    num("TH_DENSE_GEMM", &k->dense_gemm, 0, 1);
    num("TH_CONV_GL", &k->conv_gl, 0, 2);
    num("TH_FIRST_ZB", &k->first_zb, 0, 1 << 20);
    num("TH_FIRST_DBG", &k->first_dbg, 0, 1 << 20);
    flag("TH_NO_POOL_FIRST", &k->no_pool_first);
    flag("TH_NO_TAIL_FUSE", &k->no_tail_fuse);
    flag("TH_CONV_NOGEO", &k->conv_nogeo);
    flag("TH_N16_NOGEO", &k->n16_nogeo);
    flag("TH_CONV_NOXC", &k->conv_noxc);
    flag("TH_CONV_NOTAIL", &k->conv_notail);
    flag("TH_CONV_NOZMAJOR", &k->conv_nozmajor);
    flag("TH_CONV_NOCOMPACT", &k->conv_nocompact);
    flag("TH_CONV_NOPW", &k->conv_nopw);
    if (const char* e = getenv("TH_CONV_BMODE")) {
        k->conv_bmode = !std::strcmp(e, "dbuf") ? 1 : !std::strcmp(e, "stream8") ? 2 : !std::strcmp(e, "no16") ? 3 : 0;
        if (k->conv_bmode) note("TH_CONV_BMODE", e);
    }
    num("TH_CONV_DBG", &k->conv_dbg, 0, 1 << 20);
    num("TH_CONV_LDSPAD", &k->conv_ldspad, 0, 160 * 1024);
    num("TH_N16_RESIDENT", &k->n16_resident, 0, 1 << 20);
    flag("TH_PW_NOPIPE", &k->pw_nopipe);
    flag("TH_PW_NOEPI", &k->pw_noepi);
    num("TH_PW_DBG", &k->pw_dbg, 0, 1 << 20);
    num("TH_WF_RESIDENT", &k->wf_resident, 0, 1 << 20);
    num("TH_WF_DBG", &k->wf_dbg, 0, 1 << 20);
    num("TH_WF_NOBLK", &k->wf_noblk, 0, 1);
    if (const char* e = getenv("TH_WINO_PIECE")) { k->wino_piece = std::max(0ll, atoll(e)); if (k->wino_piece) note("TH_WINO_PIECE", e); }
    num("TH_WINO_DBG", &k->wino_dbg, 0, 1 << 20);
    num("TH_WINO_VAR", &k->wino_var, 0, 3);
    num("TH_WINO_B3VAR", &k->wino_b3var, 0, 2);
    num("TH_WINO_NOMID", &k->wino_nomid, 0, 1);
}

namespace {
struct DevCache {
    std::mutex mu;
    struct Blk { void* p; uint64_t stamp; };
    std::multimap<std::pair<int, size_t>, Blk> free_blocks;
    std::map<void*, std::pair<int, size_t>> live;
    std::map<int, size_t> cached_bytes;
    std::map<int, size_t> cap_bytes;
    uint64_t clock = 0;
    static constexpr size_t kCacheBytes = 24ull << 30;
    static constexpr size_t kCacheBlocks = 1024;
};
DevCache g_cache;

size_t cache_cap_locked(int device) {
    auto it = g_cache.cap_bytes.find(device);
    if (it != g_cache.cap_bytes.end()) return it->second;
    size_t cap = DevCache::kCacheBytes, free_b = 0, total_b = 0;
    int cur = -1;
    if (hipGetDevice(&cur) == hipSuccess && (cur == device || hipSetDevice(device) == hipSuccess)) {
        if (hipMemGetInfo(&free_b, &total_b) == hipSuccess && total_b) cap = std::min(cap, total_b / 8);
        if (cur >= 0 && cur != device) (void)hipSetDevice(cur);
    }
    (void)hipGetLastError();
    g_cache.cap_bytes[device] = cap;
    return cap;
}

int cached_malloc(void** out, size_t bytes, int device) {
    if (!bytes) bytes = 4;
    {
        std::lock_guard<std::mutex> lock(g_cache.mu);
        auto it = g_cache.free_blocks.find({device, bytes});
        if (it != g_cache.free_blocks.end()) {
            *out = it->second.p;
            g_cache.free_blocks.erase(it);
            g_cache.cached_bytes[device] -= bytes;
            g_cache.live[*out] = {device, bytes};
            return TH_OK;
        }
    }
    hipError_t e = th_malloc_retry(out, bytes);
    if (e != hipSuccess) {
        (void)hipGetLastError();
        TH_FAIL(e == hipErrorOutOfMemory ? TH_ENOMEM : TH_EHIP, "hipMalloc(%zu) failed: %s", bytes, hipGetErrorString(e));
    }
    std::lock_guard<std::mutex> lock(g_cache.mu);
    g_cache.live[*out] = {device, bytes};
    return TH_OK;
}

void cached_free(void* p) {
    if (!p) return;
    std::vector<void*> evict;
    {
        std::lock_guard<std::mutex> lock(g_cache.mu);
        auto it = g_cache.live.find(p);
        if (it == g_cache.live.end()) { (void)hipFree(p); return; }
        const std::pair<int, size_t> key = it->second;
        g_cache.live.erase(it);
        const size_t cap = cache_cap_locked(key.first);
        if (key.second > cap) evict.push_back(p);
        else {
            g_cache.free_blocks.insert({key, {p, ++g_cache.clock}});
            g_cache.cached_bytes[key.first] += key.second;
            while (g_cache.cached_bytes[key.first] > cap || g_cache.free_blocks.size() > DevCache::kCacheBlocks) {
                auto oldest = g_cache.free_blocks.end();
                for (auto b = g_cache.free_blocks.begin(); b != g_cache.free_blocks.end(); ++b)
                    if ((b->first.first == key.first || g_cache.free_blocks.size() > DevCache::kCacheBlocks) &&
                        (oldest == g_cache.free_blocks.end() || b->second.stamp < oldest->second.stamp))
                        oldest = b;
                if (oldest == g_cache.free_blocks.end()) break;
                evict.push_back(oldest->second.p);
                g_cache.cached_bytes[oldest->first.first] -= oldest->first.second;
                g_cache.free_blocks.erase(oldest);
            }
        }
    }
    for (void* q : evict) (void)hipFree(q);
}
}

hipError_t th_malloc_retry_impl(void** p, size_t bytes) {
    hipError_t e = hipMalloc(p, bytes);
    if (e != hipErrorOutOfMemory) return e;
    (void)hipGetLastError();
    int device = 0;
    if (hipGetDevice(&device) != hipSuccess) return e;
    std::vector<void*> drop;
    {
        std::lock_guard<std::mutex> lock(g_cache.mu);
        for (auto it = g_cache.free_blocks.begin(); it != g_cache.free_blocks.end();) {
            if (it->first.first == device) {
                drop.push_back(it->second.p);
                g_cache.cached_bytes[device] -= it->first.second;
                it = g_cache.free_blocks.erase(it);
            } else ++it;
        }
    }
    if (drop.empty()) return e;
    for (void* q : drop) (void)hipFree(q);
    e = hipMalloc(p, bytes);
    if (e != hipSuccess) (void)hipGetLastError();
    return e;
}

extern "C" int th_dev_trim(int device) {
    std::vector<void*> drop;
    {
        std::lock_guard<std::mutex> lock(g_cache.mu);
        for (auto it = g_cache.free_blocks.begin(); it != g_cache.free_blocks.end();) {
            if (device < 0 || it->first.first == device) {
                drop.push_back(it->second.p);
                g_cache.cached_bytes[it->first.first] -= it->first.second;
                it = g_cache.free_blocks.erase(it);
            } else ++it;
        }
    }
    if (drop.empty()) return TH_OK;
    for (void* p : drop) (void)hipFree(p);
    return TH_OK;
}

extern "C" int th_dev_cache_info(int device, uint64_t* cached_bytes, uint64_t* cap_bytes, int* blocks) {
    std::lock_guard<std::mutex> lock(g_cache.mu);
    uint64_t c = 0;
    int n = 0;
    for (auto& kv : g_cache.free_blocks)
        if (device < 0 || kv.first.first == device) { c += kv.first.second; ++n; }
    if (cached_bytes) *cached_bytes = c;
    if (cap_bytes) *cap_bytes = device >= 0 ? cache_cap_locked(device) : DevCache::kCacheBytes;
    if (blocks) *blocks = n;
    return TH_OK;
}

namespace {

constexpr int kMaxIn = 8, kNIp = 24, kNFp = 8, kNW = 8, kNameBytes = 56;
struct PackNode {
    uint32_t op, n_in;
    int32_t in[kMaxIn];
    int32_t ip[kNIp];
    float fp[kNFp];
    int32_t w[kNW];
    char name[kNameBytes];
};
static_assert(sizeof(PackNode) == 256, "pack node record must be 256 bytes");
struct PackHeader {
    char magic[8];
    uint32_t n_nodes, n_blobs, output_node, reserved;
};

struct Node {
    int op = 0;
    std::vector<int> in;
    int ip[kNIp] = {0};
    float fp[kNFp] = {0};
    int w[kNW] = {-1, -1, -1, -1, -1, -1, -1, -1};
    std::string name;
    int D = 1, H = 1, W = 1, C = 0;
    int rank = 0;
    std::vector<int> consumers;
    int absorbed_by = -1;
    int buf = -1, cs = 0, coff = 0;
    int blk = 0;
    bool materialised = false;
};

struct Buffer {
    int64_t floats_per_frame = 0;
    float* dev = nullptr;
};

struct Step {
    std::string label;
    std::function<int(hipStream_t, int64_t)> run;
    double flops = 0, exec_flops = 0, bytes = 0;
    double direct_flops = -1;
    double ms = 0;
    int64_t launches = 0;
    int out_node = -1;
    bool is_final_softmax = false;
    bool fast = false;
};

inline std::string label_note(const std::string& label, const char* note) {
    const size_t k = label.rfind(" [");
    return k == std::string::npos ? label + note : label.substr(0, k) + note + label.substr(k);
}

inline void keras_same_pad(int n, int k, int s, int d, int* before) {
    const int ke = (k - 1) * d + 1;
    const int out = (n + s - 1) / s;
    int total = (out - 1) * s + ke - n;
    if (total < 0) total = 0;
    *before = total / 2;
}

}

struct th_model {
    int device = 0;
    int ncu = 0;
    unsigned flags = 0;
    hipStream_t stream = nullptr;
    std::vector<Node> nodes;
    std::vector<const float*> blob_host;
    std::vector<size_t> blob_count;
    std::vector<char> pack;
    std::vector<float*> dev_allocs;
    std::vector<Buffer> bufs;
    std::vector<Step> steps;
    int wino_v_buf = -1, wino_m_buf = -1;
    ThKnobs knobs;
    int guard_state = 0;
    double guard_dlogit = 0, guard_scale = 0;
    double guard_ms = 0;
    double guard_ref_load_ms = 0, guard_run_ms = 0;
    std::string guard_note;
    int input_node = -1, output_node = -1, logits_node = -1;
    int in_dims[4] = {0, 0, 0, 0};
    int n_classes = 0;
    int chunk = 1024;
    int chunk_alloc = 0;
    int profiling = 0;
    int dominant_step = -1;
    std::vector<hipEvent_t> ev_pool;
    double algo_flops = 0, exec_flops = 0;
    static constexpr int kRing = 3;
    static constexpr int kTickets = 4;
    hipStream_t copy_stream = nullptr, d2h_stream = nullptr;
    void* d_in_ring[kRing] = {nullptr, nullptr, nullptr};
    size_t in_ring_bytes = 0;
    void* d_sp_ring[kRing] = {nullptr, nullptr, nullptr};
    size_t sp_ring_bytes = 0;
    hipEvent_t ev_h2d[kRing] = {nullptr, nullptr, nullptr};
    hipEvent_t ev_free[kRing] = {nullptr, nullptr, nullptr};
    bool ring_used[kRing] = {false, false, false};
    uint64_t piece_counter = 0;
    std::mutex mu;
    struct Ticket {
        bool busy = false;
        bool waiting = false;
        hipEvent_t computed = nullptr, done = nullptr;
        float* d_out = nullptr;  size_t d_out_floats = 0;
        float* h_out = nullptr;  size_t h_out_floats = 0;
        float* user_out = nullptr;
        size_t floats = 0;
    } tickets[kTickets];
    int64_t last_n = 0;
    const void* cur_in = nullptr;
    int cur_dtype = TH_F32;
    bool need_convert = true;

    int lanes = 1;
    int lane_lag = 1;
    hipStream_t stream2 = nullptr;
    hipEvent_t ev_fork = nullptr, ev_join = nullptr;
    int64_t lane_off = 0;

    TView view(int node) const {
        const Node& nd = nodes[node];
        TView v;
        const Buffer& b = bufs[nd.buf];
        v.p = b.dev + lane_off * b.floats_per_frame;
        v.D = nd.D; v.H = nd.H; v.W = nd.W; v.C = nd.C;
        v.cs = nd.cs; v.coff = nd.coff; v.fs = b.floats_per_frame;
        v.blk = nd.blk;
        return v;
    }
};

namespace {

int upload(th_model* m, const float* h, size_t count, float** out) {
    float* d = nullptr;
    if (int rc = cached_malloc((void**)&d, (count ? count : 1) * sizeof(float), m->device)) return rc;
    m->dev_allocs.push_back(d);
    if (count) HIP_TRY(hipMemcpy(d, h, count * sizeof(float), hipMemcpyHostToDevice));
    *out = d;
    return TH_OK;
}

int parse_pack(th_model* m) {
    const std::vector<char>& p = m->pack;
    if (p.size() < sizeof(PackHeader)) TH_FAIL(TH_EIO, "pack too small (%zu bytes)", p.size());
    PackHeader h;
    std::memcpy(&h, p.data(), sizeof h);
    if (std::memcmp(h.magic, "THPK0001", 8) != 0) TH_FAIL(TH_EIO, "bad pack magic");
    size_t pos = sizeof(PackHeader);
    if (p.size() < pos + (size_t)h.n_nodes * sizeof(PackNode) + (size_t)h.n_blobs * 16) TH_FAIL(TH_EIO, "truncated pack");
    m->nodes.resize(h.n_nodes);
    for (uint32_t i = 0; i < h.n_nodes; ++i) {
        PackNode pn;
        std::memcpy(&pn, p.data() + pos, sizeof pn);
        pos += sizeof pn;
        Node& n = m->nodes[i];
        n.op = (int)pn.op;
        if (pn.n_in > (uint32_t)kMaxIn) TH_FAIL(TH_EIO, "node %u: too many inputs", i);
        for (uint32_t k = 0; k < pn.n_in; ++k) {
            if (pn.in[k] < 0 || pn.in[k] >= (int)i) TH_FAIL(TH_EIO, "node %u: input %d is not topologically earlier", i, pn.in[k]);
            n.in.push_back(pn.in[k]);
        }
        std::memcpy(n.ip, pn.ip, sizeof n.ip);
        std::memcpy(n.fp, pn.fp, sizeof n.fp);
        std::memcpy(n.w, pn.w, sizeof n.w);
        pn.name[kNameBytes - 1] = 0;
        n.name = pn.name;
        n.rank = pn.ip[kNIp - 5];
        const int* shp = &pn.ip[kNIp - 4];
        if (n.rank == 4) { n.D = shp[0]; n.H = shp[1]; n.W = shp[2]; n.C = shp[3]; }
        else if (n.rank == 1) { n.D = n.H = n.W = 1; n.C = shp[0]; }
        else TH_FAIL(TH_EUNSUP, "node %s: output rank %d not supported", n.name.c_str(), n.rank);
        if (n.C <= 0 || n.D <= 0 || n.H <= 0 || n.W <= 0) TH_FAIL(TH_EIO, "node %s: bad shape", n.name.c_str());
    }
    std::vector<std::pair<uint64_t, uint64_t>> table(h.n_blobs);
    for (uint32_t i = 0; i < h.n_blobs; ++i) {
        std::memcpy(&table[i].first, p.data() + pos, 8);
        std::memcpy(&table[i].second, p.data() + pos + 8, 8);
        pos += 16;
    }
    pos = (pos + 15) / 16 * 16;
    const size_t data_floats = (p.size() - pos) / 4;
    for (auto& t : table) {
        if (t.first + t.second > data_floats) TH_FAIL(TH_EIO, "blob outside pack data");
        m->blob_host.push_back(reinterpret_cast<const float*>(p.data() + pos) + t.first);
        m->blob_count.push_back((size_t)t.second);
    }
    if (h.output_node >= h.n_nodes) TH_FAIL(TH_EIO, "bad output node");
    m->output_node = (int)h.output_node;
    for (size_t i = 0; i < m->nodes.size(); ++i) {
        for (int s : m->nodes[i].in) m->nodes[s].consumers.push_back((int)i);
        for (int k = 0; k < kNW; ++k)
            if (m->nodes[i].w[k] >= (int)m->blob_host.size()) TH_FAIL(TH_EIO, "node %zu: blob index out of range", i);
        if (m->nodes[i].op == OP_INPUT) {
            if (m->input_node >= 0) TH_FAIL(TH_EUNSUP, "more than one model input");
            m->input_node = (int)i;
        }
    }
    if (m->input_node < 0) TH_FAIL(TH_EIO, "no input node");
    const Node& in = m->nodes[m->input_node];
    if (in.rank != 4) TH_FAIL(TH_EUNSUP, "input must be rank 4 (D,H,W,C)");
    m->in_dims[0] = in.D; m->in_dims[1] = in.H; m->in_dims[2] = in.W; m->in_dims[3] = in.C;
    const Node& on = m->nodes[m->output_node];
    if (on.rank != 1) TH_FAIL(TH_EUNSUP, "model output must be a vector per frame (got rank %d)", on.rank);
    m->n_classes = on.C;
    return TH_OK;
}

bool is_elementwise(const Node& n) {
    return (n.op == OP_ACT && n.ip[0] != ACT_SOFTMAX) || n.op == OP_BN;
}

int bn_affine(th_model* m, const Node& bn, const float** scale, const float** shift) {
    const int C = bn.ip[0];
    const float eps = bn.fp[0];
    auto blob = [&](int k) -> const float* { return bn.w[k] >= 0 ? m->blob_host[bn.w[k]] : nullptr; };
    const float *g = blob(0), *b = blob(1), *mu = blob(2), *var = blob(3);
    if (!mu || !var) TH_FAIL(TH_EIO, "%s: missing moving statistics", bn.name.c_str());
    for (int k = 0; k < 4; ++k)
        if (bn.w[k] >= 0 && (int)m->blob_count[bn.w[k]] != C) TH_FAIL(TH_EIO, "%s: BN vector length", bn.name.c_str());
    std::vector<float> sc(C), sh(C);
    for (int c = 0; c < C; ++c) {
        const float inv = (g ? g[c] : 1.f) / std::sqrt(var[c] + eps);
        sc[c] = inv;
        sh[c] = (b ? b[c] : 0.f) - mu[c] * inv;
    }
    float *dsc, *dsh;
    int rc;
    if ((rc = upload(m, sc.data(), C, &dsc)) || (rc = upload(m, sh.data(), C, &dsh))) return rc;
    *scale = dsc;
    *shift = dsh;
    return TH_OK;
}

void add_act(PostOps* po, int act, float alpha) {
    const int i = po->n++;
    if (i == 0) po->monotone = 1;
    po->type[i] = POP_ACT;
    po->act[i] = act;
    po->alpha[i] = alpha;
    const bool mono = act == ACT_LINEAR || act == ACT_RELU || act == ACT_SIGMOID || act == ACT_TANH ||
                      ((act == ACT_ELU || act == ACT_LEAKY) && alpha >= 0.f);
    if (!mono) po->monotone = 0;
}

int add_post(th_model* m, PostOps* po, const Node& n) {
    if (po->n >= TH_MAX_POST) return 1;
    if (n.op != OP_BN) { add_act(po, n.ip[0], n.fp[0]); return TH_OK; }
    const int i = po->n;
    if (i == 0) po->monotone = 1;
    po->type[i] = POP_AFFINE;
    if (int rc = bn_affine(m, n, &po->scale[i], &po->shift[i])) return rc;
    const float* g = n.w[0] >= 0 ? m->blob_host[n.w[0]] : nullptr;
    for (int c = 0; g && c < n.ip[0]; ++c) if (!(g[c] >= 0.f)) po->monotone = 0;
    po->n++;
    return TH_OK;
}

PostOps post_from(PostOps po, int c0) {
    for (int k = 0; k < po.n; ++k) {
        if (po.scale[k]) po.scale[k] += c0;
        if (po.shift[k]) po.shift[k] += c0;
    }
    return po;
}

template <class Pack>
int upload_packed(th_model* m, size_t floats, Pack pack, float** out) {
    std::vector<float> h(floats);
    pack(h.data());
    return upload(m, h.data(), h.size(), out);
}

std::vector<float> weight_columns(const float* w, size_t ktaps, int Cout, int c0, int cn) {
    std::vector<float> out(ktaps * cn);
    for (size_t r = 0; r < ktaps; ++r) std::memcpy(&out[r * cn], w + r * Cout + c0, (size_t)cn * sizeof(float));
    return out;
}

TView shape_of(const Node& n) {
    TView v;
    v.D = n.D; v.H = n.H; v.W = n.W; v.C = n.C;
    v.fs = (int64_t)n.D * n.H * n.W * n.C;
    return v;
}

ConvGeom conv_geom(const Node& c, const Node& in) {
    ConvGeom g{};
    g.kd = c.ip[0]; g.kh = c.ip[1]; g.kw = c.ip[2]; g.sd = c.ip[3]; g.sh = c.ip[4]; g.sw = c.ip[5];
    g.dd = c.ip[6]; g.dh = c.ip[7]; g.dw = c.ip[8];
    g.pz = g.py = g.px = 0;
    if (c.ip[9]) {
        keras_same_pad(in.D, g.kd, g.sd, g.dd, &g.pz);
        keras_same_pad(in.H, g.kh, g.sh, g.dh, &g.py);
        keras_same_pad(in.W, g.kw, g.sw, g.dw, &g.px);
    }
    return g;
}

struct ConvFusion {
    int src = -1;
    std::vector<int> pre;
    std::vector<int> post;
    int pool = -1;
    int last = -1;
};

enum class Kern { None, Wino, WfSplit, Wf, First5, First, Pointwise, Gl, Mfma, Direct, DenseGemm, Dense };

struct LayerPlan {
    ConvFusion f;
    ConvGeom g{};
    Kern family = Kern::None;
    ConvMfmaPlan mp;
    bool wf = false;
    ConvWfPlan wfp;
    Kern kind = Kern::None;
    ConvWinoPlan wp;
    ConvWfsPlan sp;
    bool b3 = false;
    bool tailed = false;
    ConvMfmaPlan tp;
    int cout_main = 0;
    PostOps po;
    PreOp pre;
    bool split_softmax = false;
};

bool fast_form(const LayerPlan& L) {
    return L.kind == Kern::Wino || L.kind == Kern::Wf || L.kind == Kern::WfSplit || L.kind == Kern::First5 ||
           (L.kind == Kern::First && (L.mp.first_wino || L.b3));
}

struct Planner {
    th_model* m;
    std::vector<Node>& N;
    const ThKnobs& kn;
    const bool fuse, use_mfma;
    std::map<int, LayerPlan> layers;
    std::vector<char> concat_copy;
    int fused_tail = -1;
    std::set<int> wino_in_done;
    std::set<int> gap_done;
    std::set<int> tail_done;
    explicit Planner(th_model* model)
        : m(model), N(model->nodes), kn(model->knobs), fuse(!(model->flags & (TH_LOAD_NO_FUSE | TH_LOAD_KEEP_ALL))),
          use_mfma(!(model->flags & TH_LOAD_NO_MFMA)), concat_copy(model->nodes.size() * kMaxIn, 0) {}
    int pool_mode(const ConvFusion& f) const { return f.pool < 0 ? 0 : N[f.pool].op == OP_MAXPOOL ? 1 : 2; }
    void add_step(Step s) { m->steps.push_back(std::move(s)); }
    int new_buffer(int64_t floats_per_frame) {
        m->bufs.push_back(Buffer());
        m->bufs.back().floats_per_frame = floats_per_frame;
        return (int)m->bufs.size() - 1;
    }
    Step& add_step(int out_node, std::string label, double bytes, std::function<int(hipStream_t, int64_t)> run) {
        Step s;
        s.out_node = out_node; s.label = std::move(label); s.bytes = bytes; s.run = std::move(run);
        m->steps.push_back(std::move(s));
        return m->steps.back();
    }
};

ConvFusion fuse_chain(const Planner& P, int i) {
    const std::vector<Node>& N = P.N;
    const Node& n = N[i];
    ConvFusion f;
    f.src = n.in[0];
    f.last = i;
    if (!P.fuse) return f;
    if (n.op == OP_CONV3D) {
        int x = f.src;
        std::vector<int> pre;
        if (N[x].absorbed_by < 0 && N[x].op == OP_ACT && N[x].ip[0] != ACT_SOFTMAX && N[x].consumers.size() == 1) {
            pre.push_back(x);
            x = N[x].in[0];
        }
        if (N[x].absorbed_by < 0 && N[x].op == OP_BN && N[x].consumers.size() == 1 && (pre.empty() || N[pre.back()].in[0] == x)) {
            pre.push_back(x);
            x = N[x].in[0];
        }
        if (!pre.empty()) {
            std::reverse(pre.begin(), pre.end());
            f.pre = pre;
            f.src = x;
        }
    }
    int cur = i;
    int npost = (n.op == OP_CONV3D ? n.ip[13] : n.ip[3]) != ACT_LINEAR ? 1 : 0;
    while (N[cur].consumers.size() == 1 && cur != P.m->output_node) {
        const int nx = N[cur].consumers[0];
        if (!is_elementwise(N[nx]) || npost >= TH_MAX_POST) break;
        f.post.push_back(nx);
        ++npost;
        cur = nx;
    }
    f.last = cur;
    if (n.op == OP_CONV3D && N[cur].consumers.size() == 1 && cur != P.m->output_node) {
        const Node& pl = N[N[cur].consumers[0]];
        if ((pl.op == OP_MAXPOOL || pl.op == OP_AVGPOOL) && pl.ip[0] == 2 && pl.ip[1] == 2 && pl.ip[2] == 2 &&
            pl.ip[3] == 2 && pl.ip[4] == 2 && pl.ip[5] == 2 && pl.ip[6] == 0)
            f.pool = N[cur].consumers[0];
    }
    return f;
}

void choose_family(const Planner& P, int i, LayerPlan& L) {
    ConvFusion& f = L.f;
    const Node& n = P.N[i];
    const Node& src = P.N[f.src];
    const ConvGeom& g = L.g;
    const TView iv = shape_of(src), ov = shape_of(n);
    const int pool = P.pool_mode(f);
    const bool stem = P.use_mfma && P.fuse && f.src == P.m->input_node && f.pre.empty();
    ConvMfmaPlan& mp = L.mp;
    Kern& k = L.family;
    if (stem && pool == 1 && conv_first5_ok(src.D, src.H, src.W, src.C, n.C, g, 1, P.kn)) {
        mp = ConvMfmaPlan();
        mp.pool = 1; mp.nnb = 1;
        mp.knobs = &P.kn;
        mp.exec_flops = conv_first5_exec_flops();
        mp.label = conv_first5_label();
        k = Kern::First5;
    }
    if (k == Kern::None && stem && conv_first_plan(src.D, src.H, src.W, src.C, ov, g, n.C, pool, P.kn, &mp)) k = Kern::First;
    if (k == Kern::None && P.use_mfma && g.kd * g.kh * g.kw == 1 && conv_pw_plan(iv, ov, g, src.C, n.C, pool, P.kn, &mp))
        k = Kern::Pointwise;
    if (k == Kern::None && P.use_mfma) {
        if (f.pool >= 0 && conv_mfma_plan(iv, ov, g, src.C, n.C, pool, P.kn, &mp)) k = Kern::Mfma;
        else if (conv_mfma_plan(iv, ov, g, src.C, n.C, 0, P.kn, &mp)) { k = Kern::Mfma; f.pool = -1; }
    }
    if (k == Kern::None) f.pool = -1;
}

void fusion_pass(Planner& P) {
    std::vector<Node>& N = P.N;
    th_model* m = P.m;
    for (int i = 0; i < (int)N.size(); ++i) {
        Node& n = N[i];
        if (n.absorbed_by >= 0 || (n.op != OP_CONV3D && n.op != OP_DENSE)) continue;
        LayerPlan& L = P.layers[i];
        L.f = fuse_chain(P, i);
        if (n.op == OP_CONV3D) {
            L.g = conv_geom(n, N[L.f.src]);
            choose_family(P, i, L);
        }
        ConvFusion& f = L.f;
        if (f.pool >= 0) f.last = f.pool;
        for (int x : f.pre) N[x].absorbed_by = i;
        for (int x : f.post) N[x].absorbed_by = i;
        if (f.pool >= 0) N[f.pool].absorbed_by = i;
        if (f.last != i) n.absorbed_by = i;
    }
    m->need_convert = m->output_node == m->input_node;
    for (int c : N[m->input_node].consumers) {
        const auto it = P.layers.find(c);
        if (it == P.layers.end() || it->second.f.src != m->input_node ||
            (it->second.family != Kern::First && it->second.family != Kern::First5))
            m->need_convert = true;
    }
    for (Node& n : N) n.materialised = n.absorbed_by < 0;
    for (auto& kv : P.layers) N[kv.second.f.last].materialised = true;
}

void storage_pass(Planner& P) {
    std::vector<Node>& N = P.N;
    const int nn = (int)N.size();
    for (int i = nn - 1; i >= 0; --i) {
        Node& n = N[i];
        if (n.op != OP_CONCAT) continue;
        if (n.buf < 0) {
            n.cs = n.C; n.coff = 0;
            n.buf = P.new_buffer((int64_t)n.D * n.H * n.W * n.cs);
        }
        int off = 0;
        for (size_t k = 0; k < n.in.size(); ++k) {
            Node& a = N[n.in[k]];
            const bool can_alias = P.fuse && a.buf < 0 && a.materialised && a.op != OP_INPUT && a.op != OP_FLATTEN &&
                                   a.op != OP_IDENTITY;
            if (can_alias) {
                a.buf = n.buf; a.cs = n.cs; a.coff = n.coff + off;
            } else {
                P.concat_copy[i * kMaxIn + k] = 1;
            }
            off += a.C;
        }
    }
    for (int i = 0; i < nn; ++i) {
        Node& n = N[i];
        if (!n.materialised || n.buf >= 0) continue;
        if ((n.op == OP_FLATTEN || n.op == OP_IDENTITY)) {
            const Node& a = N[n.in[0]];
            if (a.cs == a.C && a.coff == 0) {
                n.buf = a.buf; n.cs = n.C; n.coff = 0;
                if (n.op == OP_IDENTITY) { n.cs = a.cs; }
                continue;
            }
        }
        n.cs = n.C; n.coff = 0;
        if (n.op == OP_INPUT) {
            bool all_conv = !n.consumers.empty();
            for (int c : n.consumers) if (N[c].op != OP_CONV3D) all_conv = false;
            if (all_conv && P.fuse) n.cs = (n.C + 3) / 4 * 4;
        }
        n.buf = P.new_buffer((int64_t)n.D * n.H * n.W * n.cs);
    }
}

void wf_pass(Planner& P) {
    if (!(P.kn.wfused && P.use_mfma && P.fuse)) return;
    for (auto& [i, L] : P.layers) {
        const Node& n = P.N[i];
        if (n.op != OP_CONV3D || n.ip[13] == ACT_SOFTMAX) continue;
        const Node& sn = P.N[L.f.src];
        TView iv = shape_of(sn);
        iv.cs = sn.cs; iv.coff = sn.coff;
        L.wf = conv_wf_view_ok(iv) && conv_wf_plan(iv, shape_of(n), L.g, sn.C, n.C, P.pool_mode(L.f), P.kn, &L.wfp);
    }
}

void blocked_pass(Planner& P) {
    if (P.kn.wf_noblk) return;
    std::vector<Node>& N = P.N;
    for (auto& [i, L] : P.layers) {
        if (!L.wf) continue;
        const ConvFusion& f = L.f;
        const int src = f.src;
        Node& sn = N[src];
        if (src == P.m->input_node || src == P.m->output_node || !sn.materialised || sn.buf < 0) continue;
        if (sn.consumers.size() != 1 || sn.consumers[0] != (f.pre.empty() ? i : f.pre[0])) continue;
        if (sn.cs != sn.C || sn.coff != 0 || sn.C % 4) continue;
        int prod = -1, nprod = 0;
        for (auto& kv : P.layers) if (kv.second.f.last == src) { prod = kv.first; ++nprod; }
        if (nprod != 1) continue;
        const LayerPlan& pp = P.layers.at(prod);
        if (pp.wf) continue;
        if (!((pp.family == Kern::Pointwise && pp.mp.pool == 0) || (pp.family == Kern::First && pp.mp.nnb == 1))) continue;
        bool shared = false;
        for (int k = 0; k < (int)N.size(); ++k) if (k != src && N[k].buf == sn.buf && N[k].materialised) shared = true;
        if (shared) continue;
        sn.blk = 4;
    }
}

int build_epilogue(Planner& P, int i, LayerPlan& L) {
    const Node& n = P.N[i];
    const int own_act = n.op == OP_CONV3D ? n.ip[13] : n.ip[3];
    int rc;
    if (own_act == ACT_SOFTMAX) L.split_softmax = true;
    else if (own_act != ACT_LINEAR) add_act(&L.po, own_act, n.fp[0]);
    for (int x : L.f.post) if ((rc = add_post(P.m, &L.po, P.N[x]))) return rc < 0 ? rc : TH_EUNSUP;
    if (P.kn.no_pool_first) L.po.monotone = 0;
    for (int x : L.f.pre) {
        const Node& pn = P.N[x];
        if (pn.op == OP_BN) { if ((rc = bn_affine(P.m, pn, &L.pre.scale, &L.pre.shift))) return rc; }
        else { L.pre.act = pn.ip[0]; L.pre.alpha = pn.fp[0]; }
    }
    return TH_OK;
}

int choose_kernel(Planner& P, int i, LayerPlan& L) {
    th_model* m = P.m;
    if (int rc = build_epilogue(P, i, L)) return rc;
    const Node& n = P.N[i];
    const Node& sn = P.N[L.f.src];
    if (n.op == OP_DENSE) {
        if (sn.cs != sn.C || sn.coff != 0 || sn.D * sn.H * sn.W != 1) TH_FAIL(TH_EUNSUP, "%s: Dense needs a contiguous vector input", n.name.c_str());
        L.kind = P.kn.dense_gemm && dense_gemm_ok(sn.C, n.C, m->bufs[sn.buf].floats_per_frame) ? Kern::DenseGemm : Kern::Dense;
        return TH_OK;
    }
    const ConvGeom& g = L.g;
    const TView iv = shape_of(sn), ov = shape_of(n);
    const int Cin = sn.C, Cout = n.C;
    if (P.kn.winograd && P.use_mfma && P.fuse && L.f.pool < 0 && !L.split_softmax &&
        conv_wino_plan(iv, ov, g, Cin, Cout, P.kn.winograd == 2 ? 7 : 9, P.kn.wino_split, P.kn, &L.wp))
        L.kind = Kern::Wino;
    else if (L.wf && conv_wfs_plan(L.wfp, m->view(L.f.src), L.pre, P.kn, &L.sp)) L.kind = Kern::WfSplit;
    else if (L.wf) L.kind = Kern::Wf;
    else if (L.family == Kern::First5 || L.family == Kern::First || L.family == Kern::Pointwise) L.kind = L.family;
    else if (conv_gl_wanted(P.kn.conv_gl, g, n.D * n.H * n.W) && L.f.pool < 0 && !sn.blk && !P.N[L.f.last].blk &&
             (L.family == Kern::None || L.mp.bres != 3) &&
             conv_gl_ok(Cin, Cout, sn.cs, sn.coff, (int64_t)m->bufs[sn.buf].floats_per_frame))
        L.kind = Kern::Gl;
    else if (L.family == Kern::Mfma) {
        L.kind = Kern::Mfma;
        L.tailed = conv_mfma_plan_tail(iv, ov, g, Cin, Cout, L.mp.pool, L.mp, P.kn, &L.tp, &L.cout_main);
    } else L.kind = Kern::Direct;
    if (L.kind == Kern::First) L.b3 = conv_first_b3_ok(L.mp, sn.D, sn.H, sn.W, Cin, std::min(Cout, 32), g, L.po);
    L.mp.ncu = L.tp.ncu = L.wfp.ncu = L.sp.ncu = m->ncu;
    return TH_OK;
}

struct ConvArgs {
    th_model* M;
    int i, src, dst, Cin, Cout;
    ConvGeom g;
    const float* hw;
    const float* bias;
    PreOp pre;
    PostOps po;
    TView in() const { return M->view(src); }
    TView out() const { return M->view(dst); }
    const Node& node(int k) const { return M->nodes[k]; }
};

int emit_wino(Planner& P, const ConvArgs& c, const LayerPlan& L, Step st) {
    th_model* M = c.M;
    std::vector<Node>& N = P.N;
    const ConvWinoPlan wp = L.wp;
    float* dw;
    if (int rc = upload_packed(M, wp.wpk_floats, [&](float* d) { conv_wino_pack_weights(wp, c.hw, d); }, &dw)) return rc;
    if (M->wino_v_buf < 0) { M->wino_v_buf = P.new_buffer(0); M->wino_m_buf = P.new_buffer(0); }
    int64_t& v_fpf = M->bufs[M->wino_v_buf].floats_per_frame;
    v_fpf = std::max(v_fpf, wp.v_fpf);
    M->bufs[M->wino_m_buf].floats_per_frame = std::max(M->bufs[M->wino_m_buf].floats_per_frame, wp.m_fpf);
    const Node& sn = N[c.src];
    const double direct = st.flops, act_bytes = st.bytes, in_floats = (double)sn.D * sn.H * sn.W * c.Cin, mf = (double)wp.m_fpf;
    const std::string name = N[c.i].name, pts = std::to_string(wp.P * wp.P);
    auto Vp = [M]() { const Buffer& b = M->bufs[M->wino_v_buf]; return b.dev + M->lane_off * b.floats_per_frame; };
    auto Mp = [M]() { const Buffer& b = M->bufs[M->wino_m_buf]; return b.dev + M->lane_off * b.floats_per_frame; };
    if (!P.wino_in_done.count(c.i))
        P.add_step(st.out_node, name + ": wino_in (25 voxels -> " + pts + " points per plane) [k_wino_in]", 4.0 * (in_floats + (double)wp.v_fpf),
                   [=](hipStream_t s, int64_t cnt) { return launch_wino_in(s, cnt, wp, c.in(), Vp(), c.pre); });
    st.flops = wp.gemm_flops;
    st.direct_flops = direct;
    st.exec_flops = wp.split ? 6.0 * wp.exec_flops : wp.exec_flops;
    st.bytes = 4.0 * ((double)wp.v_fpf + mf);
    st.label = name + ": " + wp.label + (wp.narrow ? " [k_wino_gemm_n32]" : wp.split ? " [k_wino_gemm_b3]" : " [k_wino_gemm]");
    st.run = [=](hipStream_t s, int64_t cnt) { return launch_wino_gemm(s, cnt, wp, Vp(), Mp(), dw); };
    P.add_step(st);
    const int dst = c.dst, Cout = c.Cout;
    if (!P.kn.wino_nomid && dst != M->output_node && N[dst].consumers.size() == 1) {
        const int next = N[dst].consumers[0];
        const auto it = P.layers.find(next);
        const LayerPlan* nl = it == P.layers.end() ? nullptr : &it->second;
        if (nl && nl->kind == Kern::Wino && nl->f.src == dst && nl->f.pre.empty() && nl->wp.Cin == Cout) {
            v_fpf = std::max(v_fpf, nl->wp.v_fpf);
            P.add_step(st.out_node, name + ": wino_mid (" + pts + " points -> bias + epilogue -> " + pts + " points of " + N[next].name + ") [k_wino_mid]",
                       4.0 * (mf / wp.Coutp * Cout + (double)nl->wp.v_fpf),
                       [=](hipStream_t s, int64_t cnt) { return launch_wino_mid(s, cnt, wp, Mp(), Vp(), c.bias, c.po); });
            P.wino_in_done.insert(next);
            N[dst].materialised = false;
            return TH_OK;
        }
    }
    int gp = -1;
    if (!P.kn.no_tail_fuse && dst != M->output_node) {
        int cur = dst;
        while (N[cur].consumers.size() == 1 && N[N[cur].consumers[0]].op == OP_IDENTITY && N[cur].consumers[0] != M->output_node)
            cur = N[cur].consumers[0];
        if (N[cur].consumers.size() == 1 && N[N[cur].consumers[0]].op == OP_GAP && N[N[cur].consumers[0]].materialised &&
            N[N[cur].consumers[0]].absorbed_by < 0) {
            bool single = true;
            for (int k = dst; k != cur; k = N[k].consumers[0]) if (N[k].consumers.size() != 1) single = false;
            if (single) gp = N[cur].consumers[0];
        }
    }
    if (gp >= 0) {
        P.add_step(gp, name + ": wino_out + global_avg_pool (" + pts + " points -> bias + epilogue -> mean of the 125 voxels) [k_wino_out]",
                   4.0 * (mf / wp.Coutp * Cout + Cout),
                   [=](hipStream_t s, int64_t cnt) { return launch_wino_out(s, cnt, wp, Mp(), M->view(gp), c.bias, c.po, true); });
        for (int k = dst; ; k = N[k].consumers[0]) { N[k].materialised = false; if (N[k].consumers[0] == gp) break; }
        P.gap_done.insert(gp);
        return TH_OK;
    }
    P.add_step(st.out_node, name + ": wino_out (" + pts + " points -> 25 voxels per plane, bias + epilogue) [k_wino_out]",
               4.0 * (mf / wp.Coutp * Cout + (act_bytes / 4.0 - in_floats)),
               [=](hipStream_t s, int64_t cnt) { return launch_wino_out(s, cnt, wp, Mp(), c.out(), c.bias, c.po); });
    return TH_OK;
}

std::string conv_label(const ConvArgs& c, const std::string& kernel, bool in_blk, bool out_blk) {
    const std::string l = c.node(c.i).name + ": " + kernel;
    return in_blk ? label_note(l, " (input chunk-blocked)") : out_blk ? label_note(l, " (output chunk-blocked)") : l;
}

int emit_wfs(const ConvArgs& c, const LayerPlan& L, Step& st) {
    const ConvWfsPlan sp = L.sp;
    float* dw;
    if (int rc = upload_packed(c.M, sp.wpk_floats, [&](float* d) { conv_wfs_pack_weights(sp, c.hw, d); }, &dw)) return rc;
    st.direct_flops = st.flops;
    st.flops = sp.own_flops;
    st.exec_flops = sp.exec_flops;
    st.label = conv_label(c, sp.label, c.node(c.src).blk, false);
    st.run = [=](hipStream_t s, int64_t cnt) { return launch_conv_wfs(s, cnt, sp, c.in(), c.out(), dw, c.bias, c.po); };
    return TH_OK;
}

int emit_wf(const ConvArgs& c, const LayerPlan& L, Step& st) {
    const ConvWfPlan fp = L.wfp;
    float* dw;
    if (int rc = upload_packed(c.M, fp.wpk_floats, [&](float* d) { conv_wf_pack_weights(fp, c.hw, d); }, &dw)) return rc;
    st.direct_flops = st.flops;
    st.flops = fp.own_flops;
    st.exec_flops = fp.exec_flops;
    st.label = conv_label(c, conv_wf_label(fp, c.pre), c.node(c.src).blk, false);
    st.run = [=](hipStream_t s, int64_t cnt) { return launch_conv_wf(s, cnt, fp, c.in(), c.out(), dw, c.bias, c.pre, c.po); };
    return TH_OK;
}

int emit_first5(const ConvArgs& c, const LayerPlan& L, Step& st) {
    float* dw;
    if (int rc = upload_packed(c.M, conv_first5_wpk_floats(), [&](float* d) { conv_first5_pack_weights(c.Cin, c.Cout, c.hw, d); }, &dw))
        return rc;
    st.exec_flops = L.mp.exec_flops;
    st.label = conv_label(c, L.mp.label, false, false);
    const ThKnobs* kn = L.mp.knobs;
    st.run = [=](hipStream_t s, int64_t cnt) {
        return launch_conv_first5(s, cnt, kn, c.M->ncu, c.M->cur_in, c.M->cur_dtype, c.Cin, c.out(), c.Cout, dw, c.bias, c.po);
    };
    return TH_OK;
}

int emit_first(const ConvArgs& c, const LayerPlan& L, Step& st) {
    const ConvMfmaPlan mp = L.mp;
    const bool b3 = L.b3;
    if (mp.first_wino) {
        st.direct_flops = st.flops;
        st.flops = mp.own_flops;
    }
    st.exec_flops = b3 ? conv_first_b3_exec_flops() * mp.nnb : mp.exec_flops;
    st.label = conv_label(c, b3 ? conv_first_b3_label(mp.nnb) : conv_first_label(mp, c.Cin, c.po), false, c.node(c.dst).blk);
    if (mp.nnb > 1) st.label = label_note(st.label, (" x" + std::to_string(mp.nnb) + " passes of 32 columns").c_str());
    struct Pass { int c0, cn; float* dw; const float* bias; PostOps po; };
    std::vector<Pass> passes;
    const size_t ktaps = (size_t)c.g.kd * c.g.kh * c.g.kw * c.Cin;
    for (int c0 = 0; c0 < c.Cout; c0 += 32) {
        Pass ps{c0, std::min(32, c.Cout - c0), nullptr, c.bias ? c.bias + c0 : nullptr, post_from(c.po, c0)};
        const std::vector<float> wcol = weight_columns(c.hw, ktaps, c.Cout, c0, ps.cn);
        const int rc = upload_packed(c.M, b3 ? conv_first_b3_wpk_floats() : mp.wpk_floats, [&](float* d) {
            if (b3) conv_first_b3_pack_weights(c.Cin, ps.cn, wcol.data(), d);
            else if (mp.first_wino) conv_first_w_pack_weights(c.Cin, ps.cn, wcol.data(), d);
            else conv_first_pack_weights(c.Cin, ps.cn, wcol.data(), d);
        }, &ps.dw);
        if (rc) return rc;
        passes.push_back(ps);
    }
    const Node& sn = c.node(c.src);
    const int iD = sn.D, iH = sn.H, iW = sn.W;
    st.run = [=](hipStream_t s, int64_t cnt) {
        for (const Pass& ps : passes) {
            TView ov = c.out();
            if (passes.size() > 1) { ov.coff += ps.c0; ov.C = ps.cn; }
            th_model* M = c.M;
            const int r = b3 ? launch_conv_first_b3(s, cnt, mp, M->cur_in, M->cur_dtype, c.Cin, ov, ps.cn, ps.dw, ps.bias, ps.po)
                             : launch_conv_first(s, cnt, mp, M->cur_in, M->cur_dtype, iD, iH, iW, c.Cin, ov, c.g, ps.cn, ps.dw, ps.bias, ps.po);
            if (r) return r;
        }
        return (int)TH_OK;
    };
    return TH_OK;
}

int emit_pointwise(const ConvArgs& c, const LayerPlan& L, Step& st) {
    const ConvMfmaPlan mp = L.mp;
    float* dw;
    if (int rc = upload_packed(c.M, mp.wpk_floats, [&](float* d) { conv_pw_pack_weights(mp, c.Cin, c.Cout, c.hw, d); }, &dw)) return rc;
    const bool blk = c.node(c.dst).blk != 0;
    st.exec_flops = mp.exec_flops;
    st.label = conv_label(c, conv_pw_label(mp, blk, c.po), false, blk);
    st.run = [=](hipStream_t s, int64_t cnt) { return launch_conv_pw(s, cnt, mp, c.in(), c.out(), c.Cin, c.Cout, dw, c.bias, c.pre, c.po); };
    return TH_OK;
}

int emit_gl(const ConvArgs& c, Step& st) {
    float* dw;
    const size_t floats = conv_gl_wpk_floats(c.g, c.Cin, c.Cout);
    if (int rc = upload_packed(c.M, floats, [&](float* d) { conv_gl_pack_weights(c.g, c.Cin, c.Cout, c.hw, d); }, &dw)) return rc;
    const Node& n = c.node(c.i);
    st.exec_flops = conv_gl_exec_flops(c.g, c.Cin, c.Cout, n.D * n.H * n.W);
    st.label = conv_label(c, conv_gl_label(c.Cout), false, false);
    st.run = [=](hipStream_t s, int64_t cnt) { return launch_conv_gl(s, cnt, c.in(), c.out(), c.g, c.Cin, c.Cout, dw, c.bias, c.pre, c.po); };
    return TH_OK;
}

int emit_mfma(const ConvArgs& c, const LayerPlan& L, Step& st) {
    ConvMfmaPlan mp = L.mp;
    float *dw, *dwt;
    int rc;
    if (!L.tailed) {
        if ((rc = upload_packed(c.M, mp.wpk_floats, [&](float* d) { conv_mfma_pack_weights(mp, c.g, c.Cin, c.Cout, c.hw, d); }, &dw))) return rc;
        st.exec_flops = mp.exec_flops;
        st.label = conv_label(c, mp.label, false, false);
        st.run = [=](hipStream_t s, int64_t cnt) { return launch_conv_mfma(s, cnt, mp, c.in(), c.out(), c.g, c.Cin, c.Cout, dw, c.bias, c.pre, c.po); };
        return TH_OK;
    }
    const ConvMfmaPlan tp = L.tp;
    const int cout_main = L.cout_main, cout_tail = c.Cout - cout_main;
    const size_t ktaps = (size_t)c.g.kd * c.g.kh * c.g.kw * c.Cin;
    const std::vector<float> wm = weight_columns(c.hw, ktaps, c.Cout, 0, cout_main), wt = weight_columns(c.hw, ktaps, c.Cout, cout_main, cout_tail);
    mp.nnb -= 1;
    mp.exec_flops *= (double)mp.nnb / (mp.nnb + 1);
    mp.wpk_floats = mp.wpk_floats / (mp.nnb + 1) * mp.nnb;
    if ((rc = upload_packed(c.M, mp.wpk_floats, [&](float* d) { conv_mfma_pack_weights(mp, c.g, c.Cin, cout_main, wm.data(), d); }, &dw)) ||
        (rc = upload_packed(c.M, tp.wpk_floats, [&](float* d) { conv_mfma_pack_weights(tp, c.g, c.Cin, cout_tail, wt.data(), d); }, &dwt)))
        return rc;
    const PostOps pot = post_from(c.po, cout_main);
    const float* bias_t = c.bias ? c.bias + cout_main : nullptr;
    st.exec_flops = mp.exec_flops + tp.exec_flops;
    st.label = conv_label(c, mp.label + " x" + std::to_string(mp.nnb) + " + " + tp.label, false, false);
    st.run = [=](hipStream_t s, int64_t cnt) {
        int r1 = launch_conv_mfma(s, cnt, mp, c.in(), c.out(), c.g, c.Cin, cout_main, dw, c.bias, c.pre, c.po);
        if (r1) return r1;
        TView ot = c.out();
        ot.coff += cout_main;
        return launch_conv_mfma(s, cnt, tp, c.in(), ot, c.g, c.Cin, cout_tail, dwt, bias_t, c.pre, pot);
    };
    return TH_OK;
}

int emit_direct(const ConvArgs& c, Step& st) {
    float* dw;
    if (int rc = upload(c.M, c.hw, (size_t)c.g.kd * c.g.kh * c.g.kw * c.Cin * c.Cout, &dw)) return rc;
    st.exec_flops = st.flops;
    st.label = conv_label(c, "conv3d_direct", false, false);
    st.run = [=](hipStream_t s, int64_t cnt) { return launch_conv3d_direct(s, cnt, c.in(), c.out(), c.g, dw, c.bias, c.pre, c.po); };
    return TH_OK;
}

int emit_dense(const ConvArgs& c, const LayerPlan& L, Step& st) {
    const int F = c.Cin, O = c.Cout;
    if (c.M->blob_count[c.node(c.i).w[0]] != (size_t)F * O) TH_FAIL(TH_EIO, "%s: kernel size mismatch", c.node(c.i).name.c_str());
    float* dw;
    if (int rc = upload(c.M, c.hw, (size_t)F * O, &dw)) return rc;
    st.flops = st.exec_flops = 2.0 * F * O;
    st.bytes = 4.0 * (F + O);
    if (L.kind == Kern::DenseGemm) {
        st.label = conv_label(c, "dense as a batch GEMM, 16 frames x all outputs per workgroup, F in four quarters (16x16x4 fp32 MFMA) [k_dense_gemm]",
                              false, false);
        st.run = [=](hipStream_t s, int64_t cnt) { return launch_dense_gemm(s, cnt, c.in(), c.out(), dw, c.bias, c.po); };
    } else {
        st.label = conv_label(c, "dense", false, false);
        st.run = [=](hipStream_t s, int64_t cnt) { return launch_dense(s, cnt, c.in(), c.out(), dw, c.bias, c.po); };
    }
    return TH_OK;
}

void note_direct_form(const Planner& P, const ConvArgs& c, const LayerPlan& L, Step& st) {
    const ConvGeom& g = c.g;
    const Node& sn = c.node(c.src);
    const bool k333 = g.kd == 3 && g.kh == 3 && g.kw == 3 && g.sd == 1 && g.sh == 1 && g.sw == 1 && g.dd == 1 && g.dh == 1 && g.dw == 1;
    if (!k333 || fast_form(L)) return;
    std::string why;
    const bool same = g.pz == 1 && g.py == 1 && g.px == 1;
    if (!P.use_mfma || !P.fuse) why = "load flags select the direct kernels";
    else if (!same) why = "'valid' padding (the Cook-Toom forms are built for 'same')";
    else if (c.src == P.m->input_node && sn.C <= 8 && c.Cout <= 32) why = P.kn.first_wino ? "odd computed width" : "TH_FIRST_WINO=0";
    else if (sn.D == 5 && sn.H == 5 && sn.W == 5) {
        if (!P.kn.winograd) why = "TH_WINOGRAD=0";
        else if (L.f.pool >= 0) why = "a pooling layer is fused behind it";
        else if (sn.C < 32) why = "Cin < 32";
        else if (c.Cout < 64) why = "Cout < 64 (a 128-column GEMM block would run mostly empty)";
        else why = "softmax fused into the layer";
    } else if (sn.H % 2 == 0 && sn.W % 2 == 0 && sn.D * (sn.H / 2) * (sn.W / 2) <= 250) {
        if (!P.kn.wfused) why = "TH_WFUSED=0";
        else if (sn.C < 16 || sn.C % 4) why = "Cin < 16 or not a multiple of 4";
        else if (!(sn.D == 10 && sn.H == 10 && sn.W == 10)) why = "conv_wf is instantiated for 10^3 volumes only";
        else why = "input view is not 16-byte aligned";
    } else why = "no minimal-filtering kernel for a " + std::to_string(sn.D) + "x" + std::to_string(sn.H) + "x" + std::to_string(sn.W) +
                 " volume (conv_wf: 10^3, conv_wino: 5^3)";
    st.label = label_note(st.label, (" (direct form: " + why + ")").c_str());
}

int emit_layer(Planner& P, int i) {
    th_model* M = P.m;
    const Node& n = P.N[i];
    const LayerPlan& L = P.layers.at(i);
    const Node& sn = P.N[L.f.src];
    const Node& dn = P.N[L.f.last];
    const float* hw = n.w[0] >= 0 ? M->blob_host[n.w[0]] : nullptr;
    if (!hw) TH_FAIL(TH_EIO, "%s: missing kernel", n.name.c_str());
    float* bias = nullptr;
    int rc = TH_OK;
    if ((n.op == OP_CONV3D ? n.ip[12] : n.ip[2]) != 0) {
        if (n.w[1] < 0) TH_FAIL(TH_EIO, "%s: missing bias", n.name.c_str());
        if ((rc = upload(M, M->blob_host[n.w[1]], M->blob_count[n.w[1]], &bias))) return rc;
    }
    const ConvGeom& g = L.g;
    const ConvArgs c{M, i, L.f.src, L.f.last, sn.C, n.C, g, hw, bias, L.pre, L.po};
    Step st;
    st.out_node = c.dst;
    st.fast = fast_form(L);
    if (n.op == OP_CONV3D) {
        if (M->blob_count[n.w[0]] != (size_t)g.kd * g.kh * g.kw * c.Cin * c.Cout) TH_FAIL(TH_EIO, "%s: kernel size mismatch", n.name.c_str());
        st.flops = 2.0 * n.D * n.H * n.W * (double)g.kd * g.kh * g.kw * c.Cin * c.Cout;
        st.bytes = 4.0 * ((double)sn.D * sn.H * sn.W * c.Cin + (double)dn.D * dn.H * dn.W * dn.C);
    }
    switch (L.kind) {
        case Kern::Wino: return emit_wino(P, c, L, st);
        case Kern::WfSplit: rc = emit_wfs(c, L, st); break;
        case Kern::Wf: rc = emit_wf(c, L, st); break;
        case Kern::First5: rc = emit_first5(c, L, st); break;
        case Kern::First: rc = emit_first(c, L, st); break;
        case Kern::Pointwise: rc = emit_pointwise(c, L, st); break;
        case Kern::Gl: rc = emit_gl(c, st); break;
        case Kern::Mfma: rc = emit_mfma(c, L, st); break;
        case Kern::DenseGemm: case Kern::Dense: rc = emit_dense(c, L, st); break;
        default: rc = emit_direct(c, st); break;
    }
    if (rc) return rc;
    if (n.op == OP_CONV3D) note_direct_form(P, c, L, st);
    P.add_step(st);
    if (L.split_softmax) {
        const bool final_softmax = c.dst == M->output_node;
        P.add_step(c.dst, n.name + ": softmax (layer activation)", 0,
                   [=](hipStream_t s, int64_t cnt) { return launch_softmax(s, cnt, c.out(), c.out()); }).is_final_softmax = final_softmax;
        if (final_softmax) M->logits_node = c.dst;
    }
    return TH_OK;
}

int try_dense_tail(Planner& P, int first, Step* st) {
    th_model* M = P.m;
    std::vector<Node>& N = P.N;
    if (!P.fuse || P.kn.no_tail_fuse) return 0;
    std::vector<int> chain;
    int j = first;
    while ((N[j].op == OP_BN || (N[j].op == OP_ACT && N[j].ip[0] != ACT_SOFTMAX)) && (int)chain.size() < TH_MAX_POST) {
        if (N[j].absorbed_by >= 0 || !N[j].materialised || N[j].consumers.size() != 1 || j == M->output_node) return 0;
        chain.push_back(j);
        j = N[j].consumers[0];
    }
    const int gp = j;
    if (N[gp].op != OP_GAP || P.gap_done.count(gp) || N[gp].absorbed_by >= 0 || !N[gp].materialised || N[gp].consumers.size() != 1 ||
        gp == M->output_node || N[gp].C > 2048)
        return 0;
    const int dn = N[gp].consumers[0];
    if (N[dn].op != OP_DENSE || !P.layers.count(dn) || N[dn].C > 512 || N[dn].w[0] < 0) return 0;
    const ConvFusion& f = P.layers.at(dn).f;
    if (f.src != gp || !f.pre.empty() || !f.post.empty() || f.pool >= 0 || f.last != dn || !N[dn].materialised) return 0;
    if (N[dn].ip[3] != ACT_LINEAR || dn == M->output_node || N[dn].consumers.size() != 1) return 0;
    const int sm = N[dn].consumers[0];
    if (!(N[sm].op == OP_ACT && N[sm].ip[0] == ACT_SOFTMAX && sm == M->output_node && N[sm].absorbed_by < 0 && N[sm].materialised)) return 0;
    const int src = N[chain.empty() ? gp : chain[0]].in[0];
    if (N[src].blk || !N[src].materialised || N[src].buf < 0) return 0;
    const Node& gn = N[gp];
    if (gn.cs != gn.C || gn.coff != 0) return 0;
    PostOps pre, post;
    int rc;
    for (int x : chain) if ((rc = add_post(M, &pre, N[x]))) return rc < 0 ? rc : 0;
    const int F = gn.C, O = N[dn].C;
    if (M->blob_count[N[dn].w[0]] != (size_t)F * O) return 0;
    float *dw = nullptr, *dbias = nullptr;
// ... 646 lines not shown
    return TH_OK;
}

int th_model_set_chunk(th_model* m, int frames_per_chunk) {
    if (!m || frames_per_chunk <= 0) TH_FAIL(TH_EINVAL, "bad chunk size");
    m->chunk = frames_per_chunk;
    return TH_OK;
}

int th_predict_device(th_model* m, const void* d_frames, int dtype, int64_t n, float* d_probs, unsigned flags) {
    if (n < 0) TH_FAIL(TH_EINVAL, "negative frame count");
    if (!m || (n > 0 && (!d_frames || !d_probs))) TH_FAIL(TH_EINVAL, "null argument");
    std::lock_guard<std::mutex> lock(m->mu);
    return run_device(m, d_frames, dtype, n, d_probs, flags);
}

static bool host_ptr_is_pinned(const void* p) {
    hipPointerAttribute_t a;
    if (hipPointerGetAttributes(&a, p) != hipSuccess) { (void)hipGetLastError(); return false; }
    return a.type == hipMemoryTypeHost;
}

struct SparseBatch {
    const uint64_t* vidx;
    const uint32_t* bits;
    const float* values;
    int E, W;
};
static int predict_async_locked(th_model* m, const void* frames, int dtype, int64_t n, float* probs_out, unsigned flags, int* ticket,
                                const SparseBatch* sp = nullptr);

int th_predict_async(th_model* m, const void* frames, int dtype, int64_t n, float* probs_out, unsigned flags, int* ticket) {
    if (n < 0) TH_FAIL(TH_EINVAL, "negative frame count");
    if (!m || !ticket || (n > 0 && (!frames || !probs_out))) TH_FAIL(TH_EINVAL, "null argument");
    std::lock_guard<std::mutex> lock(m->mu);
    int rc = predict_async_locked(m, frames, dtype, n, probs_out, flags, ticket);
    if (rc) {
        const std::string keep = th_last_error();
        (void)hipStreamSynchronize(m->copy_stream);
        (void)hipStreamSynchronize(m->stream);
        (void)hipStreamSynchronize(m->d2h_stream);
        (void)hipGetLastError();
        th_set_error("%s", keep.c_str());
    }
    return rc;
}

static int predict_async_locked(th_model* m, const void* frames, int dtype, int64_t n, float* probs_out, unsigned flags, int* ticket,
                                const SparseBatch* sp) {
    const size_t esz = dtype_size(dtype);
    if (!esz) TH_FAIL(TH_EINVAL, "unknown frame dtype %d", dtype);
    HIP_TRY(hipSetDevice(m->device));
    const Node& in = m->nodes[m->input_node];
    const size_t frame_bytes = (size_t)in.D * in.H * in.W * in.C * esz;
    const bool logits = (flags & TH_PREDICT_LOGITS) != 0;
    if (logits && m->logits_node < 0) TH_FAIL(TH_EINVAL, "model does not end in a Softmax: no logits to return");
    const int width = logits ? m->nodes[m->logits_node].C : m->n_classes;
    int ti = -1;
    for (int k = 0; k < th_model::kTickets; ++k) if (!m->tickets[k].busy) { ti = k; break; }
    if (ti < 0) TH_FAIL(TH_EBUSY, "all %d tickets of this model are in flight: call th_predict_wait first", th_model::kTickets);
    th_model::Ticket& t = m->tickets[ti];
    const int64_t piece = std::min<int64_t>(m->chunk, std::max<int64_t>(n, 1));
    const size_t need_in = frame_bytes * (size_t)piece;
    if (!(flags & TH_PREDICT_IN_DEVICE) && m->in_ring_bytes < need_in) {
        HIP_TRY(hipStreamSynchronize(m->copy_stream));
        HIP_TRY(hipStreamSynchronize(m->stream));
        for (int r = 0; r < th_model::kRing; ++r) {
            if (m->d_in_ring[r]) cached_free(m->d_in_ring[r]);
            m->d_in_ring[r] = nullptr;
            m->ring_used[r] = false;
        }
        m->in_ring_bytes = 0;
        for (int r = 0; r < th_model::kRing; ++r)
            if (int rc = cached_malloc(&m->d_in_ring[r], need_in, m->device)) return rc;
        m->in_ring_bytes = need_in;
    }
    const size_t floats = (size_t)n * width;
    const bool out_on_device = (flags & TH_PREDICT_OUT_DEVICE) != 0;
    if (!out_on_device && t.d_out_floats < floats) {
        if (t.d_out) cached_free(t.d_out);
        t.d_out = nullptr; t.d_out_floats = 0;
        if (int rc = cached_malloc((void**)&t.d_out, std::max<size_t>(floats, 1024) * sizeof(float), m->device)) return rc;
        t.d_out_floats = std::max<size_t>(floats, 1024);
    }
    if (!out_on_device && t.h_out_floats < floats) {
        if (t.h_out) HIP_TRY(hipHostFree(t.h_out));
        t.h_out = nullptr; t.h_out_floats = 0;
        HIP_TRY(hipHostMalloc((void**)&t.h_out, std::max<size_t>(floats, 1024) * sizeof(float), hipHostMallocDefault));
        t.h_out_floats = std::max<size_t>(floats, 1024);
    }
    const bool in_device = (flags & TH_PREDICT_IN_DEVICE) != 0;
    const bool pinned = !in_device && n > 0 && host_ptr_is_pinned(sp ? (const void*)sp->values : frames);
    if (in_device && n > 0) {
        int rc = run_device(m, frames, dtype, n, (out_on_device ? probs_out : t.d_out), flags, false);
        if (rc) return rc;
    }
    for (int64_t off = 0; off < n && !in_device; off += piece) {
        const int64_t cnt = std::min<int64_t>(piece, n - off);
        const int r = (int)(m->piece_counter % th_model::kRing);
        if (m->ring_used[r]) {
            if (pinned) HIP_TRY(hipStreamWaitEvent(m->copy_stream, m->ev_free[r], 0));
            else HIP_TRY(hipEventSynchronize(m->ev_free[r]));
        }
        if (sp) {
            const size_t bits_b = (size_t)cnt * sp->W * 4, vidx_b = (size_t)(cnt + 1) * 8;
            const uint64_t v0 = sp->vidx[off], v1 = sp->vidx[off + cnt];
            const size_t val_b = (size_t)(v1 - v0) * 4;
            const size_t o_vidx = (bits_b + 15) / 16 * 16, o_val = (o_vidx + vidx_b + 15) / 16 * 16, need = o_val + val_b + 16;
            if (m->sp_ring_bytes < need) {
                HIP_TRY(hipStreamSynchronize(m->copy_stream));
                HIP_TRY(hipStreamSynchronize(m->stream));
                for (int q = 0; q < th_model::kRing; ++q) {
                    if (m->d_sp_ring[q]) cached_free(m->d_sp_ring[q]);
                    m->d_sp_ring[q] = nullptr;
                }
                m->sp_ring_bytes = 0;
                const size_t cap = need + need / 4;
                for (int q = 0; q < th_model::kRing; ++q)
                    if (int rc = cached_malloc(&m->d_sp_ring[q], cap, m->device)) return rc;
                m->sp_ring_bytes = cap;
            }
            char* const d = (char*)m->d_sp_ring[r];
            HIP_TRY(hipMemcpyAsync(d, sp->bits + (size_t)off * sp->W, bits_b, hipMemcpyHostToDevice, m->copy_stream));
            HIP_TRY(hipMemcpyAsync(d + o_vidx, sp->vidx + off, vidx_b, hipMemcpyHostToDevice, m->copy_stream));
            if (val_b) HIP_TRY(hipMemcpyAsync(d + o_val, sp->values + (v0 - sp->vidx[0]), val_b, hipMemcpyHostToDevice, m->copy_stream));
            HIP_TRY(hipEventRecord(m->ev_h2d[r], m->copy_stream));
            HIP_TRY(hipStreamWaitEvent(m->stream, m->ev_h2d[r], 0));
            int rc = launch_sparse_expand(m->stream, cnt, (const uint32_t*)d, (const uint64_t*)(d + o_vidx), (const float*)(d + o_val),
                                          (float*)m->d_in_ring[r], sp->E, sp->W);
            if (rc) return rc;
        } else {
        HIP_TRY(hipMemcpyAsync(m->d_in_ring[r], (const char*)frames + (size_t)off * frame_bytes, (size_t)cnt * frame_bytes,
                               hipMemcpyHostToDevice, m->copy_stream));
        HIP_TRY(hipEventRecord(m->ev_h2d[r], m->copy_stream));
        HIP_TRY(hipStreamWaitEvent(m->stream, m->ev_h2d[r], 0));
        }
        int rc = run_device(m, m->d_in_ring[r], dtype, cnt, (out_on_device ? probs_out : t.d_out) + (size_t)off * width, flags,
                            false);
        if (rc) return rc;
        HIP_TRY(hipEventRecord(m->ev_free[r], m->stream));
        m->ring_used[r] = true;
        m->piece_counter++;
    }
    HIP_TRY(hipEventRecord(t.computed, m->stream));
    HIP_TRY(hipStreamWaitEvent(m->d2h_stream, t.computed, 0));
    if (floats && !out_on_device)
        HIP_TRY(hipMemcpyAsync(t.h_out, t.d_out, floats * sizeof(float), hipMemcpyDeviceToHost, m->d2h_stream));
    HIP_TRY(hipEventRecord(t.done, m->d2h_stream));
    t.user_out = probs_out;
    t.floats = out_on_device ? 0 : floats;
    t.busy = true;
    *ticket = ti;
    return TH_OK;
}

int th_predict_sparse_async(th_model* m, const void* blob, size_t blob_bytes, float* probs_out, unsigned flags, int* ticket) {
    if (!m || !ticket || !blob) TH_FAIL(TH_EINVAL, "null argument");
    if (flags & TH_PREDICT_IN_DEVICE) TH_FAIL(TH_EINVAL, "a sparse batch is host memory");
    const char* const b = (const char*)blob;
    if ((uintptr_t)blob % 16) TH_FAIL(TH_EINVAL, "sparse batch: the blob is not 16-byte aligned");
    if (blob_bytes < 32 || std::memcmp(b, TH_SPARSE_MAGIC, 8)) TH_FAIL(TH_EINVAL, "not a THSPF001 sparse frame batch");
    uint32_t n32, E, W, esz;
    uint64_t nval;
    std::memcpy(&n32, b + 8, 4); std::memcpy(&E, b + 12, 4); std::memcpy(&W, b + 16, 4); std::memcpy(&esz, b + 20, 4); std::memcpy(&nval, b + 24, 8);
    const Node& in = m->nodes[m->input_node];
    if (esz != 4 || (int64_t)E != (int64_t)in.D * in.H * in.W * in.C)
        TH_FAIL(TH_EINVAL, "sparse batch: %u elements of %u bytes per frame, the model reads %d float32", E, esz, in.D * in.H * in.W * in.C);
    if (W < (E + 31) / 32 || W % 4) TH_FAIL(TH_EINVAL, "sparse batch: %u bitmap words per frame for %u elements", W, E);
    const size_t o_vidx = 32, o_bits = (o_vidx + ((size_t)n32 + 1) * 8 + 15) / 16 * 16, o_val = o_bits + (size_t)n32 * W * 4;
    if (blob_bytes < o_val + nval * 4) TH_FAIL(TH_EINVAL, "sparse batch: %zu bytes, its header describes %zu", blob_bytes, o_val + (size_t)nval * 4);
    SparseBatch sp;
    sp.vidx = (const uint64_t*)(b + o_vidx); sp.bits = (const uint32_t*)(b + o_bits); sp.values = (const float*)(b + o_val);
    sp.E = (int)E; sp.W = (int)W;
    if (n32 && (sp.vidx[n32] - sp.vidx[0] != nval)) TH_FAIL(TH_EINVAL, "sparse batch: the ranks end at %llu, the header says %llu values",
                                                                   (unsigned long long)(sp.vidx[n32] - sp.vidx[0]), (unsigned long long)nval);
    for (uint32_t i = 0; i < n32; ++i)
        if (sp.vidx[i + 1] < sp.vidx[i] || sp.vidx[i + 1] - sp.vidx[i] > E) TH_FAIL(TH_EINVAL, "sparse batch: frame %u has an impossible stored-element count", i);
    if (n32 > 0 && !probs_out) TH_FAIL(TH_EINVAL, "null argument");
    std::lock_guard<std::mutex> lock(m->mu);
    int rc = predict_async_locked(m, blob, TH_F32, n32, probs_out, flags, ticket, &sp);
    if (rc) {
        const std::string keep = th_last_error();
        (void)hipStreamSynchronize(m->copy_stream);
        (void)hipStreamSynchronize(m->stream);
        (void)hipStreamSynchronize(m->d2h_stream);
        (void)hipGetLastError();
        th_set_error("%s", keep.c_str());
    }
    return rc;
}

int th_predict_wait(th_model* m, int ticket) {
    if (!m || ticket < 0 || ticket >= th_model::kTickets) TH_FAIL(TH_EINVAL, "bad ticket");
    th_model::Ticket& t = m->tickets[ticket];
    {
        std::lock_guard<std::mutex> lock(m->mu);
        if (!t.busy) TH_FAIL(TH_EINVAL, "ticket %d is not in flight", ticket);
        if (t.waiting) TH_FAIL(TH_EBUSY, "ticket %d is already being waited on by another thread", ticket);
        t.waiting = true;
    }
    int rc = TH_OK;
    hipError_t e = hipSetDevice(m->device);
    if (e == hipSuccess) e = hipEventSynchronize(t.done);
    if (e != hipSuccess) {
        th_set_error("th_predict_wait: %s", hipGetErrorString(e));
        rc = TH_EHIP;
    } else if (t.floats) {
        std::memcpy(t.user_out, t.h_out, t.floats * sizeof(float));
    }
    std::lock_guard<std::mutex> lock(m->mu);
    t.waiting = false;
    t.busy = false;
    return rc;
}

int th_predict(th_model* m, const void* frames, int dtype, int64_t n, float* probs_out, unsigned flags) {
    int ticket = -1;
    int rc = th_predict_async(m, frames, dtype, n, probs_out, flags, &ticket);
    if (rc) return rc;
    return th_predict_wait(m, ticket);
}

int th_host_alloc(size_t bytes, void** out) {
    if (!out) TH_FAIL(TH_EINVAL, "null argument");
    HIP_TRY(hipHostMalloc(out, bytes ? bytes : 1, hipHostMallocDefault));
    return TH_OK;
}
int th_host_free(void* p) {
    if (p) HIP_TRY(hipHostFree(p));
    return TH_OK;
}
int th_host_register(void* p, size_t bytes) {
    if (!p || !bytes) TH_FAIL(TH_EINVAL, "null argument");
    HIP_TRY(hipHostRegister(p, bytes, hipHostRegisterDefault));
    return TH_OK;
}
int th_host_unregister(void* p) {
    if (!p) TH_FAIL(TH_EINVAL, "null argument");
    HIP_TRY(hipHostUnregister(p));
    return TH_OK;
}

int th_model_fetch(th_model* m, const char* layer_name, int64_t n, float* out, int64_t out_floats) {
    if (!m || !layer_name || !out) TH_FAIL(TH_EINVAL, "null argument");
    HIP_TRY(hipSetDevice(m->device));
    for (size_t i = 0; i < m->nodes.size(); ++i) {
        const Node& nd = m->nodes[i];
        if (nd.name != layer_name) continue;
        if (!nd.materialised || nd.buf < 0 || nd.blk) TH_FAIL(TH_EINVAL, "layer %s is fused away (load with TH_LOAD_KEEP_ALL)", layer_name);
        if (n > m->last_n) TH_FAIL(TH_EINVAL, "only %lld frames in the last chunk", (long long)m->last_n);
        const int64_t per = (int64_t)nd.D * nd.H * nd.W * nd.C;
        if (out_floats < n * per) TH_FAIL(TH_EINVAL, "output buffer too small (%lld < %lld)", (long long)out_floats, (long long)(n * per));
        float* d = nullptr;
        HIP_TRY(th_malloc_retry((void**)&d, (size_t)(n * per) * sizeof(float) + 16));
        TView o;
        o.p = d; o.D = nd.D; o.H = nd.H; o.W = nd.W; o.C = o.cs = nd.C; o.fs = per;
        int rc = launch_copy(m->stream, n, m->view((int)i), o);
        if (!rc) {
            hipError_t e = hipStreamSynchronize(m->stream);
            if (e == hipSuccess) e = hipMemcpy(out, d, (size_t)(n * per) * sizeof(float), hipMemcpyDeviceToHost);
            if (e != hipSuccess) { th_set_error("fetch copy failed: %s", hipGetErrorString(e)); rc = TH_EHIP; }
        }
        (void)hipFree(d);
        return rc;
    }
    TH_FAIL(TH_EINVAL, "no layer named %s", layer_name);
}

int th_model_profile(th_model* m, int enable) {
    if (!m) TH_FAIL(TH_EINVAL, "null model");
    if (enable < 0 || enable > 2) TH_FAIL(TH_EINVAL, "profile mode must be 0, 1 or 2");
    m->profiling = enable;
    m->dominant_step = -1;
    double best = -1;
    bool timed = false;
    for (const Step& s : m->steps) timed = timed || s.launches > 0;
    for (size_t i = 0; i < m->steps.size(); ++i) {
        const double v = timed ? m->steps[i].ms : m->steps[i].flops;
        if (v > best) { best = v; m->dominant_step = (int)i; }
    }
    for (Step& s : m->steps) { s.ms = 0; s.launches = 0; }
    return TH_OK;
}

int th_model_step_info(const th_model* m, int i, char* label, size_t label_len, double* ms, int64_t* launches,
                       double* flops_per_frame, double* exec_flops_per_frame, double* bytes_per_frame) {
    if (!m || i < 0 || i >= (int)m->steps.size()) TH_FAIL(TH_EINVAL, "bad step index");
    const Step& s = m->steps[i];
    if (label && label_len) snprintf(label, label_len, "%s", s.label.c_str());
    if (ms) *ms = s.ms;
    if (launches) *launches = s.launches;
    if (flops_per_frame) *flops_per_frame = s.flops;
    if (exec_flops_per_frame) *exec_flops_per_frame = s.exec_flops;
    if (bytes_per_frame) *bytes_per_frame = s.bytes;
    return TH_OK;
}

int th_model_step_direct_flops(const th_model* m, int i, double* direct_flops_per_frame) {
    if (!m || i < 0 || i >= (int)m->steps.size() || !direct_flops_per_frame) TH_FAIL(TH_EINVAL, "bad step index");
    *direct_flops_per_frame = m->steps[i].direct_flops;
    return TH_OK;
}

int th_model_guard_info(const th_model* m, int* state, double* max_dlogit, double* logit_scale, char* note, size_t note_len) {
    if (!m) TH_FAIL(TH_EINVAL, "null model");
    if (state) *state = m->guard_state;
    if (max_dlogit) *max_dlogit = m->guard_dlogit;
    if (logit_scale) *logit_scale = m->guard_scale;
    if (note && note_len) {
        if (m->guard_state == 0) snprintf(note, note_len, "%s", m->guard_note.c_str());
        else snprintf(note, note_len, "%s%s[%.1f ms: direct plan load %.1f, its run %.1f]", m->guard_note.c_str(), m->guard_note.empty() ? "" : " ",
                      m->guard_ms, m->guard_ref_load_ms, m->guard_run_ms);
    }
    return TH_OK;
}

int th_model_knobs(const th_model* m, char* buf, size_t buf_len) {
    if (!m || !buf || !buf_len) TH_FAIL(TH_EINVAL, "null argument");
    snprintf(buf, buf_len, "%s", m->knobs.nondefault.c_str());
    return TH_OK;
}

int th_dev_alloc(int device, size_t bytes, void** d_out) {
    if (!d_out) TH_FAIL(TH_EINVAL, "null argument");
    HIP_TRY(hipSetDevice(device));
    HIP_TRY(th_malloc_retry(d_out, bytes ? bytes : 1));
    return TH_OK;
}
int th_dev_free(int device, void* d) {
    HIP_TRY(hipSetDevice(device));
    if (d) HIP_TRY(hipFree(d));
    return TH_OK;
}
int th_dev_upload(int device, void* d_dst, const void* h_src, size_t bytes) {
    HIP_TRY(hipSetDevice(device));
    HIP_TRY(hipMemcpy(d_dst, h_src, bytes, hipMemcpyHostToDevice));
    return TH_OK;
}
int th_dev_download(int device, void* h_dst, const void* d_src, size_t bytes) {
    HIP_TRY(hipSetDevice(device));
    HIP_TRY(hipMemcpy(h_dst, d_src, bytes, hipMemcpyDeviceToHost));
    return TH_OK;
}
int th_dev_sync(int device) {
    HIP_TRY(hipSetDevice(device));
    HIP_TRY(hipDeviceSynchronize());
    return TH_OK;
}
int th_dev_synth_frames(int device, float* d_frames, int64_t n, int side, int channels, int atoms, uint64_t seed) {
    if (!d_frames || n < 0 || side <= 0 || channels <= 0 || atoms < 0) TH_FAIL(TH_EINVAL, "bad argument");
    HIP_TRY(hipSetDevice(device));
    int rc = launch_synth_frames(nullptr, d_frames, n, side, channels, atoms, seed);
    if (rc) return rc;
    HIP_TRY(hipDeviceSynchronize());
    return TH_OK;
}

int th_apply_temp(const double* probs, int64_t n_res, int n_cls, double t, double* out) {
    if (!out) TH_FAIL(TH_EINVAL, "null argument");
    return sampler_run(0, probs, n_res, n_cls, 0, t, TH_RNG_PHILOX, 0, 0, nullptr, nullptr, nullptr, nullptr, nullptr, out);
}
int th_apply_temp_on(int device, const double* probs, int64_t n_res, int n_cls, double t, double* out) {
    if (!out) TH_FAIL(TH_EINVAL, "null argument");
    return sampler_run(device, probs, n_res, n_cls, 0, t, TH_RNG_PHILOX, 0, 0, nullptr, nullptr, nullptr, nullptr, nullptr, out);
}
int th_sample(const double* probs, int64_t n_res, int n_cls, int64_t n_samples, double temperature, int rng_mode,
              uint64_t seed, const double* uniforms, int32_t* idx_out) {
    if (!idx_out) TH_FAIL(TH_EINVAL, "null argument");
    return sampler_run(0, probs, n_res, n_cls, n_samples, temperature, rng_mode, seed, 0, uniforms, idx_out, nullptr,
                       nullptr, nullptr, nullptr);
}
int th_sample_ex(const double* probs, int64_t n_res, int n_cls, int64_t n_samples, double temperature, int rng_mode,
                 uint64_t seed, uint64_t rng_offset, const double* uniforms, int32_t* idx_out, double* r_out,
                 const char* cat_letters, char* letters_out, double* q_out, int device) {
    return sampler_run(device, probs, n_res, n_cls, n_samples, temperature, rng_mode, seed, rng_offset, uniforms, idx_out,
                       r_out, cat_letters, letters_out, q_out);
}

}
```

timed-design_amd/timed_hip/_lib.py:

```python
from __future__ import annotations

import ctypes as C
import os

_HERE = os.path.dirname(os.path.abspath(__file__))
LIB_PATH = os.environ.get("TIMED_HIP_LIB", os.path.join(_HERE, "libtimedhip.so"))

TH_OK = 0
TH_EINVAL, TH_EIO, TH_EHIP, TH_EUNSUP, TH_ENOMEM, TH_ECOMM, TH_EBUSY = -1, -2, -3, -4, -5, -6, -7
TH_F32, TH_F64, TH_U8, TH_BOOL, TH_F16 = 0, 1, 2, 3, 4
TH_LOAD_DEFAULT, TH_LOAD_NO_FUSE, TH_LOAD_NO_MFMA, TH_LOAD_KEEP_ALL = 0, 1, 2, 4
TH_PREDICT_DEFAULT, TH_PREDICT_LOGITS, TH_PREDICT_OUT_DEVICE, TH_PREDICT_IN_DEVICE = 0, 1, 2, 4
TH_RNG_HOST, TH_RNG_PHILOX, TH_RNG_MT19937, TH_RNG_MT_WORDS = 0, 1, 2, 3
TH_TEMPER_NONE, TH_TEMPER_POW, TH_TEMPER_PREPOWERED = 0, 1, 2
TH_COMM_ID_BYTES = 128

_vp, _i, _u, _i64, _u64, _d, _sz = C.c_void_p, C.c_int, C.c_uint, C.c_int64, C.c_uint64, C.c_double, C.c_size_t
_pi, _pd, _pi64 = C.POINTER(C.c_int), C.POINTER(C.c_double), C.POINTER(C.c_int64)

PROTOTYPES = {
    "th_version": (_i, []),
    "th_last_error": (C.c_char_p, []),
    "th_device_count": (_i, [_pi]),
    "th_host_cpus": (_i, []),
    "th_device_info": (_i, [_i, C.c_char_p, _sz, C.c_char_p, _sz, _pi]),
    "th_model_load": (_i, [C.c_char_p, _i, _u, C.POINTER(_vp)]),
    "th_model_load_mem": (_i, [_vp, _sz, _i, _u, C.POINTER(_vp)]),
    "th_model_free": (None, [_vp]),
    "th_model_info": (_i, [_vp, C.POINTER(C.c_int * 4), _pi]),
    "th_model_cost": (_i, [_vp, _pd, _pd, _pi]),
    "th_model_set_chunk": (_i, [_vp, _i]),
    "th_predict": (_i, [_vp, _vp, _i, _i64, _vp, _u]),
    "th_predict_device": (_i, [_vp, _vp, _i, _i64, _vp, _u]),
    "th_predict_async": (_i, [_vp, _vp, _i, _i64, _vp, _u, _pi]),
    "th_predict_sparse_async": (_i, [_vp, _vp, _sz, _vp, _u, _pi]),
    "th_predict_wait": (_i, [_vp, _i]),
    "th_host_alloc": (_i, [_sz, C.POINTER(_vp)]),
    "th_host_free": (_i, [_vp]),
    "th_host_register": (_i, [_vp, _sz]),
    "th_host_unregister": (_i, [_vp]),
    "th_model_fetch": (_i, [_vp, C.c_char_p, _i64, _vp, _i64]),
    "th_model_profile": (_i, [_vp, _i]),
    "th_model_step_info": (_i, [_vp, _i, C.c_char_p, _sz, _pd, _pi64, _pd, _pd, _pd]),
    "th_model_knobs": (_i, [_vp, C.c_char_p, _sz]),
    "th_model_step_direct_flops": (_i, [_vp, _i, _pd]),
    "th_model_guard_info": (_i, [_vp, C.POINTER(C.c_int), _pd, _pd, C.c_char_p, _sz]),
    "th_dev_alloc": (_i, [_i, _sz, C.POINTER(_vp)]),
    "th_dev_free": (_i, [_i, _vp]),
    "th_dev_upload": (_i, [_i, _vp, _vp, _sz]),
    "th_dev_download": (_i, [_i, _vp, _vp, _sz]),
    "th_dev_sync": (_i, [_i]),
    "th_dev_synth_frames": (_i, [_i, _vp, _i64, _i, _i, _i, _u64]),
    "th_apply_temp": (_i, [_vp, _i64, _i, _d, _vp]),
    "th_apply_temp_on": (_i, [_i, _vp, _i64, _i, _d, _vp]),
    "th_sampler_create": (_i, [_i, C.POINTER(_vp)]),
    "th_sampler_free": (None, [_vp]),
    "th_sampler_load": (_i, [_vp, _vp, _i64, _i, _d, _i, _i, _vp]),
    "th_sampler_draw": (_i, [_vp, _i64, _pi64, _i64, _i, _u64, _u64, _vp, C.c_char_p, _vp, _vp, _vp, _vp]),
    "th_sampler_uniform_buffer": (_i, [_vp, _sz, C.POINTER(C.c_void_p)]),
    "th_sampler_run": (_i, [_vp, _vp, _i64, _i, _i, _i64, _pi64, _i64, _i, _u64, _u64, _vp, C.c_char_p, C.c_uint, C.POINTER(C.c_void_p), _pi64]),
    "th_sample": (_i, [_vp, _i64, _i, _i64, _d, _i, _u64, _vp, _vp]),
    "th_sample_ex": (_i, [_vp, _i64, _i, _i64, _d, _i, _u64, _u64, _vp, _vp, _vp, C.c_char_p, _vp, _vp, _i]),
    "th_comm_unique_id": (_i, [C.c_char_p]),
    "th_comm_init": (_i, [C.c_char_p, _i, _i, _i, C.POINTER(_vp)]),
    "th_comm_free": (None, [_vp]),
    "th_comm_gather_rows": (_i, [_vp, _vp, _pi64, _i, _i, _vp]),
    "th_comm_barrier": (_i, [_vp]),
    "th_comm_stats": (_i, [_vp, _pi64]),
    "th_voxelise": (_i, [_i, _vp, _vp, _vp, _i64, _vp, _i64, _i, C.c_float, _i, _i, _vp, _i]),
    "th_mt19937_rand": (_i, [_vp, _pi, _i64, _vp]),
    "th_mt19937_words": (_i, [_vp, _pi, _i64, _vp]),
    "th_format_csv": (_i64, [_vp, _i, _i64, _i64, _vp, _i64]),
    "th_format_csv_device": (_i64, [_i, _vp, _i64, _i64, _vp, _i64]),
    "th_format_csv_device_release": (_i, []),
    "th_csv_shape": (_i, [C.c_char_p, _i64, C.c_char, _pi64, _pi, _pi]),
    "th_csv_fill": (_i, [C.c_char_p, _i64, C.c_char, _i64, _i, _i, _vp]),
    "th_argmax_letters": (_i, [_vp, _i, _i64, _i64, C.c_char_p, _vp, _vp]),
    "th_analyse_probs": (_i, [_i, _vp, _i, _i64, _i64, _vp, _vp, _vp, _vp, _vp, _vp]),
    "th_h5_read_chunked": (_i, [_vp, _i64, _i64, _i64, _pi64, C.POINTER(_vp), _i, _pi64, _pi64, _i, _i, _pi, _i]),
    "th_h5_read_chunked_as": (_i, [_vp, _i64, _i64, _i64, _pi64, C.POINTER(_vp), _i, _pi64, _pi64, _i, _i, _pi, _i, _i]),
    "th_h5_read_contiguous_as": (_i, [_vp, _i64, _i64, _i64, _pi64, C.POINTER(_vp), _i64, _i, _i]),
    "th_h5_decode_device": (_i, [_vp, _i64, _i64, _i64, _pi64, _i, _pi64, _pi64, _i, _i, _pi, _i, _i, _vp]),
    "th_h5_release_scratch": (_i, [_i]),
    "th_dev_trim": (_i, [_i]),
    "th_dev_cache_info": (_i, [_i, C.POINTER(C.c_uint64), C.POINTER(C.c_uint64), _pi]),
    "th_inflate_many": (_i, [_i, _vp, _i64, _i64, _pi64, _pi64, _pi64, _pi64, _vp, _i64, _i, _pi]),
    "th_h5_group_links": (_i, [_vp, _i64, _i64, _i64, _i64, _i64, _vp, _i64, _pi64, _i64, _pi64, _pi64]),
    "th_h5_resolve": (_i, [_vp, _i64, _i64, _i64, _pi64, C.c_char_p, _vp, _i, C.c_char_p, _vp, _i, _pi64, _pi64, _pi, _i]),
}

_lib = None


class TimedHipError(RuntimeError):
    def __init__(self, code: int, msg: str):
        super().__init__(f"timed_hip error {code}: {msg}")
        self.code = code


def load() -> C.CDLL:
    global _lib
    if _lib is not None:
        return _lib
    if not os.path.exists(LIB_PATH):
        raise ImportError(
            f"{LIB_PATH} not found: build it with `python __graft_entry__.py` (hipcc --offload-arch=gfx950). "
            "There is no CPU fallback.")
    os.environ.setdefault("HSA_ENABLE_IPC_MODE_LEGACY", "0")
    lib = C.CDLL(LIB_PATH)
    for name, (res, args) in PROTOTYPES.items():
        fn = getattr(lib, name)
        fn.restype = res
        fn.argtypes = args
    _lib = lib
    return lib


def check(rc: int) -> None:
    if rc != TH_OK:
        raise TimedHipError(rc, load().th_last_error().decode(errors="replace"))


def device_count() -> int:
    n = C.c_int(0)
    rc = load().th_device_count(C.byref(n))
    return n.value if rc == TH_OK else 0


def device_info(device: int = 0):
    name = C.create_string_buffer(256)
    arch = C.create_string_buffer(256)
    cus = C.c_int(0)
    check(load().th_device_info(device, name, 256, arch, 256, C.byref(cus)))
    return name.value.decode(), arch.value.decode(), cus.value
```

timed-design_amd/timed_hip/engine.py:

```python
from __future__ import annotations

import ctypes as C
import os
from typing import Dict, List, Optional

import numpy as np

from . import _lib, keras_config, pack

_DTYPES = {
    np.dtype(np.float32): _lib.TH_F32, np.dtype(np.float64): _lib.TH_F64, np.dtype(np.uint8): _lib.TH_U8,
    np.dtype(np.bool_): _lib.TH_BOOL, np.dtype(np.float16): _lib.TH_F16,
}


class HipFrameModel:
    def __init__(self, pack_bytes: bytes, device: int = 0, flags: int = _lib.TH_LOAD_DEFAULT, name: str = "model"):
        self._lib = _lib.load()
        self._h = C.c_void_p()
        self.device = device
        self.name = name
        buf = (C.c_char * len(pack_bytes)).from_buffer_copy(pack_bytes)
        _lib.check(self._lib.th_model_load_mem(buf, len(pack_bytes), device, flags, C.byref(self._h)))
        dims = (C.c_int * 4)()
        ncls = C.c_int()
        _lib.check(self._lib.th_model_info(self._h, C.byref(dims), C.byref(ncls)))
        self.input_shape = tuple(dims)
        self.n_classes = ncls.value
        self.device_name, self.device_arch, self.device_cus = _lib.device_info(device)
        self.chunk = 1024

    @classmethod
    def from_keras(cls, model_config, weights: Dict[str, list], device: int = 0, flags: int = 0, name: str = "model"):
        return cls(pack.keras_to_pack(model_config, weights), device=device, flags=flags, name=name)

    @classmethod
    def load(cls, path, device: int = 0, flags: int = 0):
        path = os.fspath(path)
        stem = os.path.splitext(os.path.basename(path))[0]
        with open(path, "rb") as f:
            head = f.read(8)
        if head == pack.MAGIC:
            with open(path, "rb") as f:
                return cls(f.read(), device=device, flags=flags, name=stem)
        if head == b"\x89HDF\r\n\x1a\n":
            from . import h5model
            cfg, weights = h5model.read_keras_h5(path)
            return cls.from_keras(cfg, weights, device=device, flags=flags, name=stem)
        raise ValueError(f"{path}: neither a THPK0001 pack nor an HDF5 (.h5) Keras model")

    def predict(self, X, batch_size: Optional[int] = None, verbose=0, logits: bool = False, **_ignored) -> np.ndarray:
        if isinstance(X, SparseFrames):
            return self.predict_async(X, logits=logits).result()
        X = np.asarray(X)
        if X.ndim != 5 or tuple(X.shape[1:]) != self.input_shape:
            raise ValueError(f"expected frames of shape (B, {', '.join(map(str, self.input_shape))}), got {X.shape}")
        dt = _DTYPES.get(X.dtype)
        if dt is None:
            X = X.astype(np.float32)
            dt = _lib.TH_F32
        X = np.ascontiguousarray(X)
        n = X.shape[0]
        width = self.logits_width if logits else self.n_classes
        out = np.empty((n, width), dtype=np.float32)
        if n:
            _lib.check(self._lib.th_predict(self._h, X.ctypes.data, dt, n, out.ctypes.data,
                                            _lib.TH_PREDICT_LOGITS if logits else 0))
        return out

    __call__ = predict

    def predict_async(self, X, logits: bool = False) -> "PendingPrediction":
        if isinstance(X, DeviceFrames):
            return self.predict_async_frames_on_device(X, logits=logits)
        if isinstance(X, SparseFrames):
            return self._predict_async_sparse(X, None, logits=logits)
        return self._predict_async_host(X, logits=logits)

    def _predict_async_sparse(self, X: "SparseFrames", d_out, logits: bool = False) -> "PendingPrediction":
        if tuple(X.shape[1:]) != self.input_shape:
            raise ValueError(f"expected frames of shape (B, {', '.join(map(str, self.input_shape))}), got {X.shape}")
        blob = X.blob()
        n = X.shape[0]
        flags = _lib.TH_PREDICT_LOGITS if logits else 0
        out = None
        if d_out is None:
            out = np.empty((n, self.logits_width if logits else self.n_classes), dtype=np.float32)
        else:
            flags |= _lib.TH_PREDICT_OUT_DEVICE
        ticket = C.c_int(-1)
        _lib.check(self._lib.th_predict_sparse_async(self._h, blob.ctypes.data, blob.nbytes,
                                                     C.c_void_p(d_out) if d_out is not None else out.ctypes.data, flags, C.byref(ticket)))
        return PendingPrediction(self, ticket.value, (X, blob), out)

    def _predict_async_host(self, X, logits: bool = False) -> "PendingPrediction":
        X = np.asarray(X)
        if X.ndim != 5 or tuple(X.shape[1:]) != self.input_shape:
            raise ValueError(f"expected frames of shape (B, {', '.join(map(str, self.input_shape))}), got {X.shape}")
        dt = _DTYPES.get(X.dtype)
        if dt is None:
            X = X.astype(np.float32)
            dt = _lib.TH_F32
        X = np.ascontiguousarray(X)
        n = X.shape[0]
        out = np.empty((n, self.logits_width if logits else self.n_classes), dtype=np.float32)
        ticket = C.c_int(-1)
        _lib.check(self._lib.th_predict_async(self._h, X.ctypes.data, dt, n, out.ctypes.data,
                                              _lib.TH_PREDICT_LOGITS if logits else 0, C.byref(ticket)))
        return PendingPrediction(self, ticket.value, X, out)

    def predict_async_device(self, X, d_out: int) -> "PendingPrediction":
        if isinstance(X, SparseFrames):
            return self._predict_async_sparse(X, d_out)
        if isinstance(X, DeviceFrames):
            if tuple(X.shape[1:]) != self.input_shape or X.device != self.device:
                raise ValueError(f"device frames of shape {X.shape} on device {X.device} do not fit this model")
            ticket = C.c_int(-1)
            _lib.check(self._lib.th_predict_async(self._h, C.c_void_p(X.ptr), _DTYPES[np.dtype(X.dtype)], X.shape[0], C.c_void_p(d_out),
                                                  _lib.TH_PREDICT_OUT_DEVICE | _lib.TH_PREDICT_IN_DEVICE, C.byref(ticket)))
            return PendingPrediction(self, ticket.value, X, None)
        X = np.asarray(X)
        if X.ndim != 5 or tuple(X.shape[1:]) != self.input_shape:
            raise ValueError(f"expected frames of shape (B, {', '.join(map(str, self.input_shape))}), got {X.shape}")
        dt = _DTYPES.get(X.dtype)
        if dt is None:
            X = X.astype(np.float32)
            dt = _lib.TH_F32
        X = np.ascontiguousarray(X)
        ticket = C.c_int(-1)
        _lib.check(self._lib.th_predict_async(self._h, X.ctypes.data, dt, X.shape[0], C.c_void_p(d_out),
                                              _lib.TH_PREDICT_OUT_DEVICE, C.byref(ticket)))
        return PendingPrediction(self, ticket.value, X, None)

    def predict_async_frames_on_device(self, frames: "DeviceFrames", logits: bool = False) -> "PendingPrediction":
        if tuple(frames.shape[1:]) != self.input_shape:
            raise ValueError(f"expected frames of shape (B, {', '.join(map(str, self.input_shape))}), got {frames.shape}")
        if frames.device != self.device:
            raise ValueError(f"frames live on device {frames.device}, the model on {self.device}")
        n = frames.shape[0]
        out = np.empty((n, self.logits_width if logits else self.n_classes), dtype=np.float32)
        ticket = C.c_int(-1)
        _lib.check(self._lib.th_predict_async(self._h, C.c_void_p(frames.ptr), _DTYPES[np.dtype(frames.dtype)], n, out.ctypes.data,
                                              _lib.TH_PREDICT_IN_DEVICE | (_lib.TH_PREDICT_LOGITS if logits else 0), C.byref(ticket)))
        return PendingPrediction(self, ticket.value, frames, out)

    @property
    def logits_width(self) -> int:
        return self.n_classes

    def predict_device(self, d_frames: int, n: int, d_probs: int, dtype: int = _lib.TH_F32, logits: bool = False):
        _lib.check(self._lib.th_predict_device(self._h, C.c_void_p(d_frames), dtype, n, C.c_void_p(d_probs),
                                               _lib.TH_PREDICT_LOGITS if logits else 0))

    def set_chunk(self, frames: int):
        _lib.check(self._lib.th_model_set_chunk(self._h, int(frames)))
        self.chunk = int(frames)

    def cost(self):
        a, e, n = C.c_double(), C.c_double(), C.c_int()
        _lib.check(self._lib.th_model_cost(self._h, C.byref(a), C.byref(e), C.byref(n)))
        return dict(algo_flops=a.value, exec_flops=e.value, n_steps=n.value)

    def profile(self, mode=True):
        _lib.check(self._lib.th_model_profile(self._h, int(mode)))

    def steps(self) -> List[dict]:
        out = []
        for i in range(self.cost()["n_steps"]):
            label = C.create_string_buffer(640)
            ms, fl, ef, by = C.c_double(), C.c_double(), C.c_double(), C.c_double()
            ln = C.c_int64()
            _lib.check(self._lib.th_model_step_info(self._h, i, label, 640, C.byref(ms), C.byref(ln), C.byref(fl),
                                                    C.byref(ef), C.byref(by)))
            df = C.c_double()
            _lib.check(self._lib.th_model_step_direct_flops(self._h, i, C.byref(df)))
            out.append(dict(label=label.value.decode(), ms=ms.value, launches=ln.value, flops=fl.value,
                            exec_flops=ef.value, bytes=by.value, direct_flops=df.value if df.value >= 0 else None))
        return out

    def guard(self) -> dict:
        st, d, sc = C.c_int(), C.c_double(), C.c_double()
        note = C.create_string_buffer(512)
        _lib.check(self._lib.th_model_guard_info(self._h, C.byref(st), C.byref(d), C.byref(sc), note, 512))
        return dict(state=st.value, max_dlogit=d.value, logit_scale=sc.value, note=note.value.decode())

    def knobs(self) -> str:
        buf = C.create_string_buffer(1024)
        _lib.check(self._lib.th_model_knobs(self._h, buf, 1024))
        return buf.value.decode()

    def fetch(self, layer_name: str, n: int, shape) -> np.ndarray:
        out = np.empty((n, *shape), dtype=np.float32)
        _lib.check(self._lib.th_model_fetch(self._h, layer_name.encode(), n, out.ctypes.data, out.size))
        return out

    def close(self):
        if getattr(self, "_h", None) and self._h.value:
            self._lib.th_model_free(self._h)
            self._h = C.c_void_p()

    def __del__(self):
        try:
            self.close()
        except Exception:
            pass


class PendingPrediction:

    def __init__(self, model: HipFrameModel, ticket: int, frames: np.ndarray, out: np.ndarray):
        self._model, self._ticket, self._frames, self._out = model, ticket, frames, out

    def result(self) -> np.ndarray:
        if self._ticket is not None:
            t, self._ticket = self._ticket, None
            try:
                _lib.check(self._model._lib.th_predict_wait(self._model._h, t))
            finally:
                self._frames = None
        return self._out

    def __del__(self):
        try:
            if self._ticket is not None and self._model._h:
                self._model._lib.th_predict_wait(self._model._h, self._ticket)
        except Exception:
            pass


class PinnedBuffer:

    def __init__(self, nbytes: int):
        self._lib = _lib.load()
        self.nbytes = int(nbytes)
        p = C.c_void_p()
        _lib.check(self._lib.th_host_alloc(self.nbytes, C.byref(p)))
        self.ptr = p.value
        self._raw = (C.c_char * self.nbytes).from_address(self.ptr)

    def array(self, shape, dtype, offset: int = 0) -> np.ndarray:
        dtype = np.dtype(dtype)
        count = int(np.prod(shape))
        if offset + count * dtype.itemsize > self.nbytes:
            raise ValueError("PinnedBuffer too small for the requested array")
        a = np.frombuffer(self._raw, dtype=dtype, count=count, offset=offset).reshape(shape)
        return a

    def free(self):
        if self.ptr:
            self._raw = None
            self._lib.th_host_free(C.c_void_p(self.ptr))
            self.ptr = 0

    def __del__(self):
        try:
            self.free()
        except Exception:
            pass


SPARSE_MAGIC = b"THSPF001"


def sparse_blob_layout(n: int, words: int, n_values: int):
    o_rank = 32
    o_bits = (o_rank + (n + 1) * 8 + 15) // 16 * 16
    o_val = o_bits + n * words * 4
    return o_rank, o_bits, o_val, o_val + n_values * 4


class SparseFrames:

    def __init__(self, bits, rank, values, frame_shape):
        self.bits, self.rank, self.values = bits, rank, values
        self.frame_shape = tuple(int(d) for d in frame_shape)
        self.shape = (int(bits.shape[0]),) + self.frame_shape
        self.dtype = np.dtype(np.float32)
        self._blob = None

    def __len__(self):
        return self.shape[0]

    @property
    def n_values(self) -> int:
        return int(self.rank[-1] - self.rank[0]) if len(self.rank) else 0

    @property
    def blob_bytes(self) -> int:
        return sparse_blob_layout(self.shape[0], int(self.bits.shape[1]), self.n_values)[3]

    @property
    def dense_bytes(self) -> int:
        return int(np.prod(self.shape)) * 4

    def blob(self, out: Optional[np.ndarray] = None, pool=None, threads: int = 1) -> np.ndarray:
        if out is None and self._blob is not None:
            return self._blob
        n, W, nv = self.shape[0], int(self.bits.shape[1]), self.n_values
        o_rank, o_bits, o_val, total = sparse_blob_layout(n, W, nv)
        buf = np.empty(total + 16, np.uint8) if out is None else out
        if buf.nbytes < total or buf.ctypes.data % 16:
            raise ValueError("sparse blob: the target buffer is too small or not 16-byte aligned")
        buf[:8] = np.frombuffer(SPARSE_MAGIC, np.uint8)
        buf[8:24].view(np.uint32)[:] = (n, int(np.prod(self.frame_shape)), W, 4)
        buf[24:32].view(np.uint64)[0] = nv
        buf[o_rank:o_rank + (n + 1) * 8].view(np.uint64)[:] = self.rank
        dst_bits = buf[o_bits:o_bits + n * W * 4].view(np.uint32).reshape(n, W)
        dst_val = buf[o_val:o_val + nv * 4].view(np.float32)
        src_val = self.values[:nv]
        if pool is not None and threads > 1 and nv > (1 << 20):
            cuts = [nv * i // threads for i in range(threads + 1)]
            jobs = [pool.submit(np.copyto, dst_val[a:b], src_val[a:b]) for a, b in zip(cuts[:-1], cuts[1:]) if b > a]
            jobs.append(pool.submit(np.copyto, dst_bits, self.bits))
            for j in jobs:
                j.result()
        else:
            np.copyto(dst_bits, self.bits)
            np.copyto(dst_val, src_val)
        view = buf[:total]
        if out is None:
            self._blob = view
        return view

    def staged(self, blob: np.ndarray) -> "SparseFrames":
        sf = SparseFrames(self.bits, self.rank, self.values, self.frame_shape)
        sf._blob = blob
        return sf

    def dense(self) -> np.ndarray:
        n, E = self.shape[0], int(np.prod(self.frame_shape))
        mask = np.unpackbits(np.ascontiguousarray(self.bits).view(np.uint8), axis=1, bitorder="little")[:, :E].astype(bool)
        out = np.zeros((n, E), np.float32)
        out[mask] = np.asarray(self.values[:self.n_values])
        return out.reshape(self.shape)

    @classmethod
    def from_dense(cls, frames: np.ndarray) -> "SparseFrames":
        frames = np.ascontiguousarray(frames, dtype=np.float32)
        n = frames.shape[0]
        E = int(np.prod(frames.shape[1:]))
        W = ((E + 31) // 32 + 3) // 4 * 4
        flat = frames.reshape(n, E)
        mask = flat.view(np.uint32) != 0
        padded = np.zeros((n, W * 32), bool)
        padded[:, :E] = mask
        bits = np.packbits(padded, axis=1, bitorder="little").view(np.uint32).reshape(n, W)
        rank = np.concatenate([[0], np.cumsum(mask.sum(1, dtype=np.int64))]).astype(np.uint64)
        return cls(bits, rank, flat[mask], frames.shape[1:])


class BlobRing:

    def __init__(self, slots: int, threads: int = 8):
        import queue
        from concurrent.futures import ThreadPoolExecutor
        self._lib = _lib.load()
        self._arrays = [None] * slots
        self._pinned = [False] * slots
        self._free = queue.SimpleQueue()
        for i in range(slots):
            self._free.put(i)
        self._threads = max(1, int(threads))
        self._pool = ThreadPoolExecutor(max_workers=self._threads, thread_name_prefix="stage_sparse")
        self.enabled = True

    def stage(self, X: SparseFrames):
        if not self.enabled or len(X) == 0:
            return X, None
        need = X.blob_bytes
        slot = self._free.get()
        try:
            a = self._arrays[slot]
            if a is None or a.nbytes < need:
                if a is not None and self._pinned[slot]:
                    self._lib.th_host_unregister(C.c_void_p(a.ctypes.data))
                    self._pinned[slot] = False
                raw = np.empty(need + need // 8 + 4096 + 16, np.uint8)
                off = (-raw.ctypes.data) % 16
                a = self._arrays[slot] = raw[off:]
            blob = X.blob(out=a, pool=self._pool, threads=self._threads)
            if not self._pinned[slot]:
                if self._lib.th_host_register(C.c_void_p(a.ctypes.data), a.nbytes) != 0:
                    self.enabled = False
                    self._free.put(slot)
                    return X, None
                self._pinned[slot] = True
            return X.staged(blob), slot
        except BaseException:
            self._free.put(slot)
            raise

    def release(self, slot) -> None:
        if slot is not None:
            self._free.put(slot)

    def close(self) -> None:
        if self._pool is None:
            return
        self._pool.shutdown(wait=True)
        self._pool = None
        for i, a in enumerate(self._arrays):
            if a is not None and self._pinned[i]:
                self._lib.th_host_unregister(C.c_void_p(a.ctypes.data))
                self._pinned[i] = False
        self._arrays = [None] * len(self._arrays)
        self.enabled = False


class StagingRing:

    def __init__(self, slots: int, rows: int, frame_shape, dtype, threads: int = 8):
        import queue
        from concurrent.futures import ThreadPoolExecutor
        self._lib = _lib.load()
        self._shape = (int(rows),) + tuple(int(d) for d in frame_shape)
        self._dtype = np.dtype(dtype)
        self._arrays = [None] * slots
        self._pinned = [False] * slots
        self._free = queue.SimpleQueue()
        for i in range(slots):
            self._free.put(i)
        self._threads = max(1, int(threads))
        self._pool = ThreadPoolExecutor(max_workers=self._threads, thread_name_prefix="stage_frames")
        self.enabled = True

    def stage(self, rows: np.ndarray):
        n = len(rows)
        if not self.enabled or n == 0 or n > self._shape[0] or rows.dtype != self._dtype or tuple(rows.shape[1:]) != self._shape[1:]:
            return rows, None
        slot = self._free.get()
        try:
            a = self._arrays[slot]
            if a is None:
                a = self._arrays[slot] = np.empty(self._shape, self._dtype)
            dst = a[:n]
            cuts = [n * i // self._threads for i in range(self._threads + 1)]
            jobs = [self._pool.submit(np.copyto, dst[lo:hi], rows[lo:hi]) for lo, hi in zip(cuts[:-1], cuts[1:]) if hi > lo]
            for j in jobs:
                j.result()
            if not self._pinned[slot]:
                if self._lib.th_host_register(C.c_void_p(a.ctypes.data), a.nbytes) != 0:
                    self.enabled = False
                    self._free.put(slot)
                    return rows, None
                self._pinned[slot] = True
            return dst, slot
        except BaseException:
            self._free.put(slot)
            raise

    def release(self, slot) -> None:
        if slot is not None:
            self._free.put(slot)

    def close(self) -> None:
        if self._pool is None:
            return
        self._pool.shutdown(wait=True)
        self._pool = None
        for i, a in enumerate(self._arrays):
            if a is not None and self._pinned[i]:
                self._lib.th_host_unregister(C.c_void_p(a.ctypes.data))
                self._pinned[i] = False
        self._arrays = [None] * len(self._arrays)
        self.enabled = False


def pinned_empty(shape, dtype=np.float32):
    dtype = np.dtype(dtype)
    buf = PinnedBuffer(max(1, int(np.prod(shape)) * dtype.itemsize))
    return buf.array(shape, dtype), buf


class DeviceFrames:

    def __init__(self, buffer: "DeviceBuffer", shape, dtype, on_release=None):
        self.buffer, self.shape, self.dtype = buffer, tuple(int(x) for x in shape), np.dtype(dtype)
        self.ptr, self.device = buffer.ptr, buffer.device
        self._on_release = on_release

# ... 50 lines not shown
```

Baseline: 623,800.

## Fuse Winograd B^T row transform into the split-bf16 GEMM staging

New measurement: 630,500 (median of 4 runs). +1.1%, better.

```diff
diff --git a/include/timed_hip.h b/include/timed_hip.h
--- a/include/timed_hip.h
+++ b/include/timed_hip.h
@@ -65,6 +65,7 @@
 int th_model_step_info(const th_model* m, int i, char* label, size_t label_len, double* ms, int64_t* launches,
                        double* flops_per_frame, double* exec_flops_per_frame, double* bytes_per_frame);
 int th_model_step_direct_flops(const th_model* m, int i, double* direct_flops_per_frame);
+int th_model_step_hbm_bytes(const th_model* m, int i, double* hbm_bytes_per_frame);
 
 int th_model_guard_info(const th_model* m, int* state, double* max_dlogit, double* logit_scale, char* note, size_t note_len);
 
diff --git a/timed-design_amd/csrc/common.h b/timed-design_amd/csrc/common.h
--- a/timed-design_amd/csrc/common.h
+++ b/timed-design_amd/csrc/common.h
@@ -50,6 +50,8 @@
     int wf_resident = 0, wf_dbg = 0, wf_noblk = 0;
     long long wino_piece = 0;
     int wino_dbg = 0, wino_var = 3, wino_b3var = 2, wino_nomid = 0;
+    int wino_tform = 1;
+    int wino_tfg = 0;
     std::string nondefault;
 };
 void th_knobs_read(ThKnobs* k);
@@ -159,6 +161,8 @@
     int split = 0;
     int narrow = 0;
     int b3var = 0;
+    int tform = 0;
+    int64_t vin_fpf = 0;
     const ThKnobs* knobs = nullptr;
     std::string label;
 };
@@ -168,7 +172,7 @@
 int launch_wino_in(hipStream_t s, int64_t n, const ConvWinoPlan& p, TView in, float* V, PreOp pre);
 int launch_wino_gemm(hipStream_t s, int64_t n, const ConvWinoPlan& p, const float* V, float* M, const float* wpk);
 int launch_wino_out(hipStream_t s, int64_t n, const ConvWinoPlan& p, const float* M, TView out, const float* bias, PostOps post, bool gap = false);
-int launch_wino_mid(hipStream_t s, int64_t n, const ConvWinoPlan& p, const float* M, float* V_next, const float* bias, PostOps post);
+int launch_wino_mid(hipStream_t s, int64_t n, const ConvWinoPlan& p, const float* M, float* V_next, const float* bias, PostOps post, bool next_tform);
 
 struct ConvWfPlan {
     int geo = -1;
diff --git a/timed-design_amd/csrc/conv_wino.hip b/timed-design_amd/csrc/conv_wino.hip
--- a/timed-design_amd/csrc/conv_wino.hip
+++ b/timed-design_amd/csrc/conv_wino.hip
@@ -54,9 +54,9 @@
     int64_t n;
 };
 
-template <bool PRE, int kP>
+template <bool PRE, int kP, bool TF = false>
 __global__ void __launch_bounds__(256) k_wino_in(const WinoInArgs a) {
-    constexpr int kPos = kP * kP;
+    constexpr int kPos = TF ? kP * kZ : kP * kP;
     const unsigned idx = blockIdx.x * 256u + threadIdx.x;
     const unsigned c = idx % (unsigned)a.Cin, f = idx / (unsigned)a.Cin;
     if (f >= (unsigned)a.n) return;
@@ -100,6 +100,11 @@
         float* __restrict__ pos = a.V + (int64_t)z * kPos * pstride;
 #pragma unroll
         for (int aa = 0; aa < kP; ++aa) {
+            if (TF) {
+#pragma unroll
+                for (int k = 0; k < kZ; ++k) (pos + (int64_t)(aa * kZ + k) * pstride)[ooff] = t[aa][k];
+                continue;
+            }
             float o[kP];
             WinoTab<kP>::fwd(t[aa], o);
 #pragma unroll
@@ -187,9 +192,9 @@
     int64_t n;
 };
 
-template <int kP>
+template <int kP, bool TF = false>
 __global__ void __launch_bounds__(256) k_wino_mid(const WinoMidArgs a) {
-    constexpr int kPos = kP * kP;
+    constexpr int kPos = kP * kP, kOPos = TF ? kP * kZ : kP * kP;
     const unsigned idx = blockIdx.x * 256u + threadIdx.x;
     const unsigned c = idx % (unsigned)a.Cn, f = idx / (unsigned)a.Cn;
     if (f >= (unsigned)a.n) return;
@@ -198,8 +203,8 @@
     const int64_t ipstride = a.Ns * a.Coutp, opstride = a.Ns * a.Cn;
     if (c >= (unsigned)a.C) {
         for (int z = 0; z < kZ; ++z) {
-            float* __restrict__ opos = a.V + (int64_t)z * kPos * opstride;
-            for (int q = 0; q < kPos; ++q) (opos + (int64_t)q * opstride)[ooff] = 0.f;
+            float* __restrict__ opos = a.V + (int64_t)z * kOPos * opstride;
+            for (int q = 0; q < kOPos; ++q) (opos + (int64_t)q * opstride)[ooff] = 0.f;
         }
         return;
     }
@@ -250,9 +255,14 @@
 #pragma unroll
             for (int aa = 0; aa < kP; ++aa) u[aa][k] = o[aa];
         }
-        float* __restrict__ opos = a.V + (int64_t)z * kPos * opstride;
+        float* __restrict__ opos = a.V + (int64_t)z * kOPos * opstride;
 #pragma unroll
         for (int aa = 0; aa < kP; ++aa) {
+            if (TF) {
+#pragma unroll
+                for (int k = 0; k < kZ; ++k) (opos + (int64_t)(aa * kZ + k) * opstride)[ooff] = u[aa][k];
+                continue;
+            }
             float o[kP];
             WinoTab<kP>::fwd(u[aa], o);
 #pragma unroll
@@ -271,6 +281,7 @@
     unsigned total;
     unsigned per_xcd;
     int dbg;
+    int tfg;
 };
 
 __device__ __forceinline__ constexpr bool wino_tap_ok(int zi, int dz) { return zi - dz + 1 >= 0 && zi - dz + 1 < kZ; }
@@ -428,13 +439,41 @@
 
 typedef float f32x4 __attribute__((ext_vector_type(4)));
 
+struct WinoBT9Rows { int nnz[9]; int col[9][4]; float val[9][4]; };
+constexpr WinoBT9Rows wino_bt9_rows() {
+    WinoBT9Rows r{};
+    for (int b = 0; b < 9; ++b) {
+        int n = 0;
+        for (int k = 0; k < kZ; ++k)
+            if (kWinoBT9[b][k] != 0.f) { r.col[b][n] = k; r.val[b][n] = kWinoBT9[b][k]; ++n; }
+        r.nnz[b] = n;
+        for (; n < 4; ++n) { r.col[b][n] = r.col[b][0]; r.val[b][n] = 0.f; }
+    }
+    return r;
+}
+__device__ constexpr WinoBT9Rows kWinoBT9Rows = wino_bt9_rows();
+
+template <bool TF>
 __device__ __forceinline__ void wino_gemm_b3_16(const WinoGemmArgs& a, unsigned char* lds) {
     const unsigned xcd = blockIdx.x & 7u, slot = blockIdx.x >> 3;
     const unsigned L = xcd * a.per_xcd + slot;
     if (slot >= a.per_xcd || L >= a.total) return;
-    const unsigned cb = L % (unsigned)a.ncb;
-    const unsigned fb = (L / (unsigned)a.ncb) % (unsigned)a.nfb;
-    const unsigned p = L / (unsigned)(a.ncb * a.nfb);
+    unsigned cb, fb, p, pa = 0, pb = 0;
+    if (TF) {
+        const unsigned per_a = 9u * (unsigned)(a.nfb * a.ncb), per_g = 9u * (unsigned)(a.tfg * a.ncb);
+        pa = L / per_a;
+        const unsigned r = L % per_a, g = r / per_g, r2 = r % per_g;
+        const unsigned gsz = min((unsigned)a.tfg, (unsigned)a.nfb - g * (unsigned)a.tfg);
+        pb = r2 / (gsz * (unsigned)a.ncb);
+        const unsigned r3 = r2 % (gsz * (unsigned)a.ncb);
+        fb = g * (unsigned)a.tfg + r3 / (unsigned)a.ncb;
+        cb = r3 % (unsigned)a.ncb;
+        p = pa * 9u + pb;
+    } else {
+        cb = L % (unsigned)a.ncb;
+        fb = (L / (unsigned)a.ncb) % (unsigned)a.nfb;
+        p = L / (unsigned)(a.ncb * a.nfb);
+    }
     const int tid = threadIdx.x, lane = tid & 63;
     const int wave = __builtin_amdgcn_readfirstlane(tid >> 6);
     const int r16 = lane & 15, g16 = lane >> 4;
@@ -443,8 +482,9 @@
     const __amdgpu_buffer_rsrc_t wrsrc = __builtin_amdgcn_make_buffer_rsrc(
         const_cast<float*>(a.U + ((size_t)((p * a.ncb + cb) * 4 + wave) * nchunks * 18) * 256), 0, 0xffffffffu, 0x00020000);
     const unsigned woff = (unsigned)lane * 16u;
-    const float* vbase = a.V + ((int64_t)p * a.Ns + (int64_t)fb * kNF) * a.Cin;
-    const int64_t zstride = (int64_t)a.npos * a.Ns * a.Cin;
+    const float* vbase = a.V + ((int64_t)(TF ? pa * kZ : p) * a.Ns + (int64_t)fb * kNF) * a.Cin;
+    const int64_t zstride = (int64_t)(TF ? 9 * kZ : a.npos) * a.Ns * a.Cin;
+    const unsigned kstride_b = (unsigned)(a.Ns * a.Cin) * 4u;
 
     f32x4 acc[kZ][4][2];
 #pragma unroll
@@ -481,9 +521,65 @@
                 bw[ct][dz][pc] = __builtin_bit_cast(uint4, __builtin_amdgcn_raw_buffer_load_b128(wrsrc, woff, (((ch * 2 + ct) * 3 + dz) * 3 + pc) * 1024, 0));
     };
 
+    const int tn = TF ? kWinoBT9Rows.nnz[pb] : 0;
+    unsigned tk[4]; float tc[4];
+#pragma unroll
+    for (int q = 0; q < 4; ++q) { tk[q] = TF ? (unsigned)kWinoBT9Rows.col[pb][q] * kstride_b : 0u; tc[q] = TF ? kWinoBT9Rows.val[pb][q] : 0.f; }
+    auto load_t = [&](float4 (&y)[5], int q, int i0, int ch) {
+#pragma unroll
+        for (int i = i0; i < i0 + 5; ++i)
+            y[i - i0] = __builtin_bit_cast(float4, __builtin_amdgcn_raw_buffer_load_b128(vrsrc[i >> 1], goff, tk[q] + (i & 1) * rstride32_b + ch * (kKC * 4), 0));
+    };
+    auto fma_t = [](float t, const float4 (&y)[5], float4 (&x)[5]) {
+#pragma unroll
+        for (int i = 0; i < 5; ++i) {
+            x[i].x = fmaf(t, y[i].x, x[i].x); x[i].y = fmaf(t, y[i].y, x[i].y); x[i].z = fmaf(t, y[i].z, x[i].z); x[i].w = fmaf(t, y[i].w, x[i].w);
+        }
+    };
+    auto stage_t = [&](float4 (&x)[5], int i0, int ch) {
+        float4 y[5], z[5];
+        load_t(x, 0, i0, ch);
+        if (tn > 1) load_t(y, 1, i0, ch);
+        if (tn > 2) load_t(z, 2, i0, ch);
+        __builtin_amdgcn_sched_barrier(0);
+#pragma unroll
+        for (int i = 0; i < 5; ++i) {
+            x[i].x = __fmul_rn(tc[0], x[i].x); x[i].y = __fmul_rn(tc[0], x[i].y); x[i].z = __fmul_rn(tc[0], x[i].z); x[i].w = __fmul_rn(tc[0], x[i].w);
+        }
+        if (tn > 1) {
+            fma_t(tc[1], y, x);
+            if (tn > 2) {
+                if (tn > 3) load_t(y, 3, i0, ch);
+                fma_t(tc[2], z, x);
+                if (tn > 3) fma_t(tc[3], y, x);
+            }
+        }
+    };
+    auto split_write = [&](const float4& v, int i) {
+        const unsigned h01 = wino_pk_bf16(v.x, v.y), h23 = wino_pk_bf16(v.z, v.w);
+        const float rx = v.x - wino_bf16_lo(h01), ry = v.y - wino_bf16_hi(h01);
+        const float rz = v.z - wino_bf16_lo(h23), rw = v.w - wino_bf16_hi(h23);
+        const unsigned m01 = wino_pk_bf16(rx, ry), m23 = wino_pk_bf16(rz, rw);
+        const float sx = rx - wino_bf16_lo(m01), sy = ry - wino_bf16_hi(m01);
+        const float sz = rz - wino_bf16_lo(m23), sw = rw - wino_bf16_hi(m23);
+        const unsigned l01 = wino_pk_bf16(sx, sy), l23 = wino_pk_bf16(sz, sw);
+        *reinterpret_cast<uint2*>(sdst + i * 2048) = make_uint2(h01, h23);
+        *reinterpret_cast<uint2*>(sdst + i * 2048 + kB3Slab) = make_uint2(m01, m23);
+        *reinterpret_cast<uint2*>(sdst + i * 2048 + 2 * kB3Slab) = make_uint2(l01, l23);
+    };
+
     for (int ch = 0; ch < nchunks; ++ch) {
         __syncthreads();
-        {
+        if (TF && !(a.dbg & 1)) {
+#pragma unroll
+            for (int hf = 0; hf < 2; ++hf) {
+                float4 x[5];
+                stage_t(x, 5 * hf, ch);
+#pragma unroll
+                for (int i = 0; i < 5; ++i) split_write(x[i], 5 * hf + i);
+                __builtin_amdgcn_sched_barrier(0);
+            }
+        } else {
             float4 x[10];
 #pragma unroll
             for (int i = 0; i < 10; ++i)
@@ -491,18 +587,7 @@
                        __builtin_bit_cast(float4, __builtin_amdgcn_raw_buffer_load_b128(vrsrc[i >> 1], goff, (i & 1) * rstride32_b + ch * (kKC * 4), 0));
             __builtin_amdgcn_sched_barrier(0);
 #pragma unroll
-            for (int i = 0; i < 10; ++i) {
-                const unsigned h01 = wino_pk_bf16(x[i].x, x[i].y), h23 = wino_pk_bf16(x[i].z, x[i].w);
-                const float rx = x[i].x - wino_bf16_lo(h01), ry = x[i].y - wino_bf16_hi(h01);
-                const float rz = x[i].z - wino_bf16_lo(h23), rw = x[i].w - wino_bf16_hi(h23);
-                const unsigned m01 = wino_pk_bf16(rx, ry), m23 = wino_pk_bf16(rz, rw);
-                const float sx = rx - wino_bf16_lo(m01), sy = ry - wino_bf16_hi(m01);
-                const float sz = rz - wino_bf16_lo(m23), sw = rw - wino_bf16_hi(m23);
-                const unsigned l01 = wino_pk_bf16(sx, sy), l23 = wino_pk_bf16(sz, sw);
-                *reinterpret_cast<uint2*>(sdst + i * 2048) = make_uint2(h01, h23);
-                *reinterpret_cast<uint2*>(sdst + i * 2048 + kB3Slab) = make_uint2(m01, m23);
-                *reinterpret_cast<uint2*>(sdst + i * 2048 + 2 * kB3Slab) = make_uint2(l01, l23);
-            }
+            for (int i = 0; i < 10; ++i) split_write(x[i], i);
         }
         load_b(ch, 0);
         load_b(ch, 1);
@@ -569,8 +654,8 @@
 template <int VAR>
 __global__ void __launch_bounds__(256, 2) k_wino_gemm_b3(const WinoGemmArgs a) {
     __shared__ __attribute__((aligned(16))) unsigned char lds[3 * kB3Slab];
-    if constexpr (VAR == 2) {
-        wino_gemm_b3_16(a, lds);
+    if constexpr (VAR == 2 || VAR == 3) {
+        wino_gemm_b3_16<VAR == 3>(a, lds);
         return;
     }
     const unsigned xcd = blockIdx.x & 7u, slot = blockIdx.x >> 3;
@@ -840,9 +925,11 @@
     p->ncb = narrow ? 1 : p->Coutp / kCB;
     p->split = split ? 1 : 0;
     p->b3var = split && !narrow ? kn.wino_b3var : 0;
+    p->tform = kn.wino_tform && scheme == 9 && p->b3var == 2 && p->Cinp <= 128 ? 1 : 0;
     p->knobs = &kn;
     p->wpk_floats = (size_t)kPos * 3 * Cinp * p->Coutp * (p->split ? 3 : 2) / 2;
     p->v_fpf = (int64_t)kZ * kPos * Cinp;
+    p->vin_fpf = p->tform ? (int64_t)kZ * scheme * kZ * Cinp : p->v_fpf;
     p->m_fpf = (int64_t)kZ * kPos * p->Coutp;
     p->gemm_flops = 2.0 * kPos * 13 * Cin * (double)Cout;
     p->exec_flops = 2.0 * kPos * 13 * Cinp * (double)((Cout + 31) / 32 * 32);
@@ -972,7 +1059,10 @@
         ia.in = in.p + f0 * in.fs; ia.in_fs = in.fs; ia.in_cs = in.cs; ia.in_coff = in.coff; ia.Cin = p.Cinp; ia.Creal = p.Cin; ia.pre = pre;
         ia.V = V + f0 * p.Cinp; ia.Ns = Ns; ia.n = cnt;
         const dim3 grid((unsigned)((cnt * p.Cinp + 255) / 256));
-        if (p.P == 9) {
+        if (p.tform) {
+            if (has_pre) hipLaunchKernelGGL((k_wino_in<true, 9, true>), grid, dim3(256), 0, s, ia);
+            else hipLaunchKernelGGL((k_wino_in<false, 9, true>), grid, dim3(256), 0, s, ia);
+        } else if (p.P == 9) {
             if (has_pre) hipLaunchKernelGGL((k_wino_in<true, 9>), grid, dim3(256), 0, s, ia);
             else hipLaunchKernelGGL((k_wino_in<false, 9>), grid, dim3(256), 0, s, ia);
         } else {
@@ -995,13 +1085,17 @@
     ga.per_xcd = (ga.total + 7) / 8;
     const ThKnobs& kn = th_knobs_of(p.knobs);
     ga.dbg = kn.wino_dbg;
+    ga.tfg = std::max(1, std::min(ga.nfb, kn.wino_tfg > 0 ? kn.wino_tfg : 4));
+    if (p.tform && 5 * ga.Ns * (int64_t)ga.Cin * 4 >= (1ll << 32))
+        TH_FAIL(TH_EUNSUP, "conv_wino: %lld frames per launch exceed the 32-bit row offsets of the T-form GEMM", (long long)n);
     const int var = kn.wino_var;
     if (p.narrow) {
         const int64_t groups = (ga.Ns / 32 + 3) / 4;
         hipLaunchKernelGGL(k_wino_gemm_n32, dim3((unsigned)(ga.npos * groups)), dim3(256), 0, s, ga);
     } else if (p.split) {
         const int bvar = p.b3var;
-        if (bvar == 2) hipLaunchKernelGGL(k_wino_gemm_b3<2>, dim3(ga.per_xcd * 8), dim3(256), 0, s, ga);
+        if (bvar == 2 && p.tform) hipLaunchKernelGGL(k_wino_gemm_b3<3>, dim3(ga.per_xcd * 8), dim3(256), 0, s, ga);
+        else if (bvar == 2) hipLaunchKernelGGL(k_wino_gemm_b3<2>, dim3(ga.per_xcd * 8), dim3(256), 0, s, ga);
         else if (bvar == 1) hipLaunchKernelGGL(k_wino_gemm_b3<1>, dim3(ga.per_xcd * 8), dim3(256), 0, s, ga);
         else hipLaunchKernelGGL(k_wino_gemm_b3<0>, dim3(ga.per_xcd * 8), dim3(256), 0, s, ga);
     }
@@ -1034,7 +1128,7 @@
     return TH_OK;
 }
 
-int launch_wino_mid(hipStream_t s, int64_t n, const ConvWinoPlan& p, const float* M, float* V_next, const float* bias, PostOps post) {
+int launch_wino_mid(hipStream_t s, int64_t n, const ConvWinoPlan& p, const float* M, float* V_next, const float* bias, PostOps post, bool next_tform) {
     if (n <= 0) return TH_OK;
     const int64_t Ns = (n + kNF - 1) / kNF * kNF;
     if (Ns * (int64_t)p.Coutp >= (1ll << 31))
@@ -1045,7 +1139,8 @@
     WinoMidArgs ma;
     ma.M = M; ma.Ns = Ns; ma.Coutp = p.Coutp; ma.C = p.Cout; ma.Cn = Cn; ma.bias = bias; ma.post = post; ma.V = V_next; ma.n = n;
     const dim3 grid((unsigned)((n * (int64_t)Cn + 255) / 256));
-    if (p.P == 9) hipLaunchKernelGGL(k_wino_mid<9>, grid, dim3(256), 0, s, ma);
+    if (next_tform) hipLaunchKernelGGL((k_wino_mid<9, true>), grid, dim3(256), 0, s, ma);
+    else if (p.P == 9) hipLaunchKernelGGL(k_wino_mid<9>, grid, dim3(256), 0, s, ma);
     else hipLaunchKernelGGL(k_wino_mid<7>, grid, dim3(256), 0, s, ma);
     HIP_TRY(hipGetLastError());
     return TH_OK;
diff --git a/timed-design_amd/csrc/runtime.hip b/timed-design_amd/csrc/runtime.hip
--- a/timed-design_amd/csrc/runtime.hip
+++ b/timed-design_amd/csrc/runtime.hip
@@ -80,6 +80,8 @@
     num("TH_WINO_VAR", &k->wino_var, 0, 3);
     num("TH_WINO_B3VAR", &k->wino_b3var, 0, 2);
     num("TH_WINO_NOMID", &k->wino_nomid, 0, 1);
+    num("TH_WINO_TFORM", &k->wino_tform, 0, 1);
+    num("TH_WINO_TFG", &k->wino_tfg, 0, 1 << 20);
 }
 
 namespace {
@@ -260,6 +262,7 @@
     std::function<int(hipStream_t, int64_t)> run;
     double flops = 0, exec_flops = 0, bytes = 0;
     double direct_flops = -1;
+    double hbm_bytes = -1;
     double ms = 0;
     int64_t launches = 0;
     int out_node = -1;
@@ -835,16 +838,19 @@
     if (int rc = upload_packed(M, wp.wpk_floats, [&](float* d) { conv_wino_pack_weights(wp, c.hw, d); }, &dw)) return rc;
     if (M->wino_v_buf < 0) { M->wino_v_buf = P.new_buffer(0); M->wino_m_buf = P.new_buffer(0); }
     int64_t& v_fpf = M->bufs[M->wino_v_buf].floats_per_frame;
-    v_fpf = std::max(v_fpf, wp.v_fpf);
+    v_fpf = std::max(v_fpf, wp.vin_fpf);
     M->bufs[M->wino_m_buf].floats_per_frame = std::max(M->bufs[M->wino_m_buf].floats_per_frame, wp.m_fpf);
     const Node& sn = N[c.src];
     const double direct = st.flops, act_bytes = st.bytes, in_floats = (double)sn.D * sn.H * sn.W * c.Cin, mf = (double)wp.m_fpf;
     const std::string name = N[c.i].name, pts = std::to_string(wp.P * wp.P);
     auto Vp = [M]() { const Buffer& b = M->bufs[M->wino_v_buf]; return b.dev + M->lane_off * b.floats_per_frame; };
     auto Mp = [M]() { const Buffer& b = M->bufs[M->wino_m_buf]; return b.dev + M->lane_off * b.floats_per_frame; };
-    if (!P.wino_in_done.count(c.i))
+    auto real_bytes = [&P](const ConvWinoPlan& w, double others) { if (w.tform) P.m->steps.back().hbm_bytes = 4.0 * (others + (double)w.vin_fpf); };
+    if (!P.wino_in_done.count(c.i)) {
         P.add_step(st.out_node, name + ": wino_in (25 voxels -> " + pts + " points per plane) [k_wino_in]", 4.0 * (in_floats + (double)wp.v_fpf),
                    [=](hipStream_t s, int64_t cnt) { return launch_wino_in(s, cnt, wp, c.in(), Vp(), c.pre); });
+        real_bytes(wp, in_floats);
+    }
     st.flops = wp.gemm_flops;
     st.direct_flops = direct;
     st.exec_flops = wp.split ? 6.0 * wp.exec_flops : wp.exec_flops;
@@ -852,16 +858,19 @@
     st.label = name + ": " + wp.label + (wp.narrow ? " [k_wino_gemm_n32]" : wp.split ? " [k_wino_gemm_b3]" : " [k_wino_gemm]");
     st.run = [=](hipStream_t s, int64_t cnt) { return launch_wino_gemm(s, cnt, wp, Vp(), Mp(), dw); };
     P.add_step(st);
+    real_bytes(wp, mf);
     const int dst = c.dst, Cout = c.Cout;
     if (!P.kn.wino_nomid && dst != M->output_node && N[dst].consumers.size() == 1) {
         const int next = N[dst].consumers[0];
         const auto it = P.layers.find(next);
         const LayerPlan* nl = it == P.layers.end() ? nullptr : &it->second;
         if (nl && nl->kind == Kern::Wino && nl->f.src == dst && nl->f.pre.empty() && nl->wp.Cin == Cout) {
-            v_fpf = std::max(v_fpf, nl->wp.v_fpf);
+            v_fpf = std::max(v_fpf, nl->wp.vin_fpf);
+            const bool next_tform = nl->wp.tform != 0;
             P.add_step(st.out_node, name + ": wino_mid (" + pts + " points -> bias + epilogue -> " + pts + " points of " + N[next].name + ") [k_wino_mid]",
                        4.0 * (mf / wp.Coutp * Cout + (double)nl->wp.v_fpf),
-                       [=](hipStream_t s, int64_t cnt) { return launch_wino_mid(s, cnt, wp, Mp(), Vp(), c.bias, c.po); });
+                       [=](hipStream_t s, int64_t cnt) { return launch_wino_mid(s, cnt, wp, Mp(), Vp(), c.bias, c.po, next_tform); });
+            real_bytes(nl->wp, mf / wp.Coutp * Cout);
             P.wino_in_done.insert(next);
             N[dst].materialised = false;
             return TH_OK;
@@ -2114,6 +2123,12 @@
     return TH_OK;
 }
 
+int th_model_step_hbm_bytes(const th_model* m, int i, double* hbm_bytes_per_frame) {
+    if (!m || i < 0 || i >= (int)m->steps.size() || !hbm_bytes_per_frame) TH_FAIL(TH_EINVAL, "bad step index");
+    *hbm_bytes_per_frame = m->steps[i].hbm_bytes;
+    return TH_OK;
+}
+
 int th_model_guard_info(const th_model* m, int* state, double* max_dlogit, double* logit_scale, char* note, size_t note_len) {
     if (!m) TH_FAIL(TH_EINVAL, "null model");
     if (state) *state = m->guard_state;
diff --git a/timed-design_amd/timed_hip/_lib.py b/timed-design_amd/timed_hip/_lib.py
--- a/timed-design_amd/timed_hip/_lib.py
+++ b/timed-design_amd/timed_hip/_lib.py
@@ -44,6 +44,7 @@
     "th_model_step_info": (_i, [_vp, _i, C.c_char_p, _sz, _pd, _pi64, _pd, _pd, _pd]),
     "th_model_knobs": (_i, [_vp, C.c_char_p, _sz]),
     "th_model_step_direct_flops": (_i, [_vp, _i, _pd]),
+    "th_model_step_hbm_bytes": (_i, [_vp, _i, _pd]),
     "th_model_guard_info": (_i, [_vp, C.POINTER(C.c_int), _pd, _pd, C.c_char_p, _sz]),
     "th_dev_alloc": (_i, [_i, _sz, C.POINTER(_vp)]),
     "th_dev_free": (_i, [_i, _vp]),
diff --git a/timed-design_amd/timed_hip/engine.py b/timed-design_amd/timed_hip/engine.py
--- a/timed-design_amd/timed_hip/engine.py
+++ b/timed-design_amd/timed_hip/engine.py
@@ -174,8 +174,11 @@
                                                     C.byref(ef), C.byref(by)))
             df = C.c_double()
             _lib.check(self._lib.th_model_step_direct_flops(self._h, i, C.byref(df)))
+            hb = C.c_double()
+            _lib.check(self._lib.th_model_step_hbm_bytes(self._h, i, C.byref(hb)))
             out.append(dict(label=label.value.decode(), ms=ms.value, launches=ln.value, flops=fl.value,
-                            exec_flops=ef.value, bytes=by.value, direct_flops=df.value if df.value >= 0 else None))
+                            exec_flops=ef.value, bytes=by.value, direct_flops=df.value if df.value >= 0 else None,
+                            hbm_bytes=hb.value if hb.value >= 0 else None))
         return out
 
     def guard(self) -> dict:
```
